# jh-jeong/ContraD

Hardware: AMD Instinct MI355X
Metric: discriminator-step images/sec (ContraD, SimCLR aug) (higher is better)
Workload: dtype f32; 1 GPU; SNDCGAN + ContraD D-step, CIFAR-10 32x32, global batch 512, simclr aug, nonsat loss, Adam(2e-4,(0.5,0.999)), random-init weights; global_batch=512, per_gpu_batch=512, parallelism=dp1, losses_finite=True, launch=hipGraph replay, rccl_ranks=1

## Files before the change

contrad_amd/_lib.py:

```python
import ctypes
import os
import re

_HERE = os.path.dirname(os.path.abspath(__file__))
LIB_PATH = os.environ.get('CONTRAD_HIP_LIB') or os.path.join(_HERE, 'csrc', 'libcontrad_hip.so')
HEADER_PATH = os.path.join(os.path.dirname(_HERE), 'include', 'contrad_hip.h')


class ConvDesc(ctypes.Structure):
    _fields_ = [(n, ctypes.c_int) for n in
                ('N', 'H', 'W', 'C', 'ldx', 'Ho', 'Wo', 'K', 'ldy', 'KH', 'KW', 'stride', 'pad', 'ldw')]


SN_MAX_LAYERS = 24
ADAM_MAX_TENSORS = 64
ADAM_CHUNK = 16384
AUG_NPARAM = 16


class SnLayer(ctypes.Structure):
    _fields_ = [('w', ctypes.c_void_p), ('u', ctypes.c_void_p), ('v', ctypes.c_void_p),
                ('u_snap', ctypes.c_void_p), ('v_snap', ctypes.c_void_p),
                ('wp', ctypes.c_void_p), ('gwp', ctypes.c_void_p), ('gw', ctypes.c_void_p),
                ('K', ctypes.c_int), ('C', ctypes.c_int), ('T', ctypes.c_int), ('ldw', ctypes.c_int),
                ('fixed_scale', ctypes.c_float)]


class SnBatch(ctypes.Structure):
    _fields_ = [('n', ctypes.c_int), ('layers', SnLayer * SN_MAX_LAYERS),
                ('scratch_off', ctypes.c_longlong * SN_MAX_LAYERS)]


class AdamTensor(ctypes.Structure):
    _fields_ = [('p', ctypes.c_void_p), ('g', ctypes.c_void_p), ('m', ctypes.c_void_p), ('v', ctypes.c_void_p),
                ('numel', ctypes.c_longlong)]


class AdamBatch(ctypes.Structure):
    _fields_ = [('n', ctypes.c_int), ('t', AdamTensor * ADAM_MAX_TENSORS),
                ('block_start', ctypes.c_int * (ADAM_MAX_TENSORS + 1))]


MODCONV_MAX_LAYERS = 32


class ModconvLayer(ctypes.Structure):
    _fields_ = [('w', ctypes.c_void_p), ('wp', ctypes.c_void_p), ('wsq', ctypes.c_void_p),
                ('Cout', ctypes.c_int), ('Cin', ctypes.c_int), ('T', ctypes.c_int), ('ldw', ctypes.c_int),
                ('transposed', ctypes.c_int), ('scale', ctypes.c_float)]


class ModconvBatch(ctypes.Structure):
    _fields_ = [('n', ctypes.c_int), ('layers', ModconvLayer * MODCONV_MAX_LAYERS)]


class DemodLayer(ctypes.Structure):
    _fields_ = [('style', ctypes.c_void_p), ('wsq', ctypes.c_void_p), ('out', ctypes.c_void_p),
                ('Cin', ctypes.c_int), ('K', ctypes.c_int)]


class DemodBatch(ctypes.Structure):
    _fields_ = [('n', ctypes.c_int), ('B', ctypes.c_int), ('layers', DemodLayer * MODCONV_MAX_LAYERS)]


_CTYPES = {
    'int': ctypes.c_int,
    'float': ctypes.c_float,
    'double': ctypes.c_double,
    'long long': ctypes.c_longlong,
    'contrad_stream_t': ctypes.c_void_p,
    'void': None,
}


def _map_type(t):
    t = t.strip()
    if t.endswith('*'):
        base = t[:-1].replace('const', '').strip()
        if base == 'contrad_conv_desc':
            return ctypes.POINTER(ConvDesc)
        if base == 'int':
            return ctypes.POINTER(ctypes.c_int)
        return ctypes.c_void_p
    t = t.replace('const', '').strip()
    return _CTYPES[t]


def parse_header(path=HEADER_PATH):
    src = open(path).read()
    src = re.sub(r'/\*.*?\*/', '', src, flags=re.S)
    protos = {}
    for m in re.finditer(r'\b(int|long long|void|double)\s+(contrad_\w+)\s*\(([^)]*)\)\s*;', src):
        ret, name, args = m.group(1), m.group(2), m.group(3).strip()
        argtypes = []
        if args and args != 'void':
            for a in args.split(','):
                a = a.strip()
                mm = re.match(r'(.*?)(\w+)$', a)
                argtypes.append(_map_type(mm.group(1)))
        protos[name] = (_CTYPES[ret], argtypes)
    return protos


class _Lib(object):
    def __init__(self):
        if not os.path.exists(LIB_PATH):
            raise RuntimeError(
                'contrad_amd: %s not found -- run `python -c "import __graft_entry__ as g; g.build()"` '
                '(or python contrad_amd/build.py).  There is no CPU / PyTorch fallback.' % LIB_PATH)
        self._dll = ctypes.CDLL(LIB_PATH)
        self.protos = parse_header()
        for name, (ret, argtypes) in self.protos.items():
            fn = getattr(self._dll, name)
            fn.restype = ret
            fn.argtypes = argtypes
            setattr(self, '_raw_' + name, fn)

    def call(self, name, *args):
        rc = getattr(self, '_raw_' + name)(*args)
        if rc != 0:
            raise RuntimeError('contrad_hip: %s failed with status %d' % (name, rc))

    def raw(self, name):
        return getattr(self, '_raw_' + name)


_lib = None


def lib():
    global _lib
    if _lib is None:
        _lib = _Lib()
    return _lib
```

contrad_amd/csrc/igemm.hip:

```cpp
#include "common.h"
#include <stdlib.h>
#include <string.h>
#include <algorithm>
#include <utility>
#include "../../include/contrad_hip.h"

namespace {

enum { MODE_FWD = 0, MODE_DGRAD = 1, MODE_WGRAD = 2 };
#ifndef IGEMM_BK
#define IGEMM_BK 16
#endif
constexpr int BK = IGEMM_BK;
#ifndef IGEMM_MIN_WAVES
#define IGEMM_MIN_WAVES 4
#endif
constexpr int NTHREADS = 256;

struct IgemmArgs {
  const float* A;
  const float* B;
  float* C;
  const float* bias;
  const float* addend;
// ... 713 lines not shown
  if (d->H < 4 || d->W < 4 || (d->H & (d->H - 1)) || (d->W & (d->W - 1))) return false;
  const int cin = mode == MODE_FWD ? d->C : d->K, cout = mode == MODE_FWD ? d->K : d->C;
  const int ldi = mode == MODE_FWD ? d->ldx : d->ldy, ldo = mode == MODE_FWD ? d->ldy : d->ldx;
  if ((cin & 15) || (cout & 63) || (ldi & 3) || (d->ldw & 3)) return false;
  const int th = std::min(8, d->H / 2), tw = std::min(8, d->W / 2);
  const long long nimg = 64 / (th * tw);
  if (nimg > 16) return false;
  const long long lim = 1ll << 31;
  if (nimg * d->H * d->W * std::max(ldi, ldo) * 4 >= lim) return false;
  if (16ll * cin * cout * 4 >= lim) return false;
  return true;
}

wino::Args wino_args(const contrad_conv_desc* d, int mode) {
  wino::Args a{};
  a.N = d->N; a.H = d->H; a.W = d->W;
  a.Cin = mode == MODE_FWD ? d->C : d->K;
  a.Cout = mode == MODE_FWD ? d->K : d->C;
  a.ldi = mode == MODE_FWD ? d->ldx : d->ldy;
  a.ldo = mode == MODE_FWD ? d->ldy : d->ldx;
  a.TH = std::min(8, d->H / 2); a.TW = std::min(8, d->W / 2);
  a.sh_tw = __builtin_ctz(a.TW); a.sh_thw = __builtin_ctz(a.TH * a.TW);
  a.NIMG = 64 / (a.TH * a.TW);
  a.PH = d->H / (2 * a.TH); a.PW = d->W / (2 * a.TW);
  a.NP = cdiv(d->N, a.NIMG) * a.PH * a.PW;
  a.NKB = a.Cout / 64;
  a.BH = a.PH > 1 ? 2 * a.TH + 2 : d->H; a.r_org = a.PH > 1 ? -1 : 0;
  a.BW = a.PW > 1 ? 2 * a.TW + 2 : d->W; a.c_org = a.PW > 1 ? -1 : 0;
  return a;
}

long long wino_items(const contrad_conv_desc* d, int mode) {
  const wino::Args a = wino_args(d, mode);
  return (long long)a.NP * a.NKB;
}

constexpr int WINO_CUS = 256;
bool wino44_planned(const contrad_conv_desc* d, int mode);

bool wino_planned(const contrad_conv_desc* d, int mode) {
  static const bool enabled = []() { const char* e = contrad_dev_env("CONTRAD_WINO"); return !(e && e[0] == '0'); }();
  if (!enabled || !wino_ok(d, mode)) return false;
  if (wino44_planned(d, mode)) return false;
  const long long items = wino_items(d, mode);
  const long long rounds = cdivll(items, WINO_CUS);
  static const long long min_items = []() { const char* e = contrad_dev_env("CONTRAD_WINO_MIN_ITEMS"); return e ? atoll(e) : 150ll; }();
  if (items < WINO_CUS) return items >= min_items;
  return rounds * WINO_CUS * 10 <= items * 14;
}

long long wino_workspace_bytes(const contrad_conv_desc* d) { return 16ll * d->C * d->K * (long long)sizeof(float); }

int wino_grid(const wino::Args& a) {
  const int l0 = cdiv(a.NP, 8) * a.NKB;
  return 8 * std::min(WINO_CUS / 8, l0);
}


bool wino44_ok(const contrad_conv_desc* d, int mode) {
  if (mode != MODE_FWD && mode != MODE_DGRAD) return false;
  if (d->KH != 3 || d->KW != 3 || d->stride != 1 || d->pad != 1) return false;
  if (d->H < 4 || d->W < 4 || (d->H & (d->H - 1)) || (d->W & (d->W - 1)) || (d->W < 32 ? d->H != d->W : d->H < 16)) return false;
  const int cin = mode == MODE_FWD ? d->C : d->K, cout = mode == MODE_FWD ? d->K : d->C;
  const int ldi = mode == MODE_FWD ? d->ldx : d->ldy, ldo = mode == MODE_FWD ? d->ldy : d->ldx;
  if ((cin & 31) || (cout & 31) || (ldi & 3) || (d->ldw & 3)) return false;
  const long long lim = 1ll << 31;
  const long long nimg = d->W >= 32 ? 1 : d->W == 16 ? 2 : d->W == 8 ? 8 : 32;
  if (nimg * d->H * d->W * std::max(ldi, ldo) * 4 >= lim) return false;
  if (36ll * cin * cout * 4 >= lim) return false;
  return true;
}

static inline bool wino44_round_ok(long long items) {
  static const long long min_items = []() { const char* e = contrad_dev_env("CONTRAD_WINO44_MIN_ITEMS"); return e ? atoll(e) : 230ll; }();
  if (items < WINO_CUS) return items >= min_items;
  return cdivll(items, WINO_CUS) * WINO_CUS * 10 <= items * 14;
}

static inline long long wino44_patches(const contrad_conv_desc* d) {
  const int TW = std::min(8, d->W / 4), TH = std::min(4, d->H / 4);
  return (long long)cdiv(d->N, 32 / (TH * TW)) * (d->H / (4 * TH)) * (d->W / (4 * TW));
}

static inline bool wino44_n32(const contrad_conv_desc* d, int mode) {
  static const bool all = []() { const char* e = contrad_dev_env("CONTRAD_WINO44N_ALL"); return e && e[0] == '1'; }();
  static const bool fill = []() { const char* e = contrad_dev_env("CONTRAD_WINO44N_FILL"); return !(e && e[0] == '0'); }();
  const int cout = mode == MODE_FWD ? d->K : d->C;
  if ((cout & 63) != 0 || d->W == 4 || all) return true;
  const long long items64 = wino44_patches(d) * (cout / 64);
  return fill && !wino44_round_ok(items64) && wino44_round_ok(2 * items64);
}

wino44::Args wino44_args(const contrad_conv_desc* d, int mode) {
  wino44::Args a{};
  a.N = d->N; a.H = d->H; a.W = d->W;
  a.Cin = mode == MODE_FWD ? d->C : d->K;
  a.Cout = mode == MODE_FWD ? d->K : d->C;
  a.ldi = mode == MODE_FWD ? d->ldx : d->ldy;
  a.ldo = mode == MODE_FWD ? d->ldy : d->ldx;
  a.TW = std::min(8, d->W / 4); a.TH = std::min(4, d->H / 4);
  a.sh_tw = __builtin_ctz(a.TW); a.sh_thw = __builtin_ctz(a.TH * a.TW);
  a.NIMG = 32 / (a.TH * a.TW);
  a.PH = d->H / (4 * a.TH); a.PW = d->W / (4 * a.TW);
  a.NP = cdiv(d->N, a.NIMG) * a.PH * a.PW;
  a.n32 = wino44_n32(d, mode) ? 1 : 0;
  a.NKB = a.n32 ? a.Cout / 32 : a.Cout / 64;
  a.BH = 4 * a.TH + 2; a.BW = 4 * a.TW + 2;
  return a;
}

long long wino44_items(const contrad_conv_desc* d, int mode) {
  const wino44::Args a = wino44_args(d, mode);
  return (long long)a.NP * a.NKB;
}

bool wino44_planned(const contrad_conv_desc* d, int mode) {
  static const bool enabled = []() { const char* e = contrad_dev_env("CONTRAD_WINO44"); return !(e && e[0] == '0'); }();
  static const bool enabled2 = []() { const char* e = contrad_dev_env("CONTRAD_WINO"); return !(e && e[0] == '0'); }();
  if (!enabled || !enabled2 || !wino44_ok(d, mode)) return false;
  static const bool enabled_n = []() { const char* e = contrad_dev_env("CONTRAD_WINO44N"); return !(e && e[0] == '0'); }();
  if (!enabled_n && wino44_n32(d, mode)) return false;
  return wino44_round_ok(wino44_items(d, mode));
}

long long wino44_workspace_bytes(const contrad_conv_desc* d) { return 36ll * d->C * d->K * (long long)sizeof(float); }

int wino44_grid(const wino44::Args& a) {
  const int l0 = cdiv(a.NP, 8) * a.NKB;
  return 8 * std::min(WINO_CUS / 8, l0);
}

template <int MODE, int BOXW>
int launch_wino44_inst(const wino44::Args& a, hipStream_t stream) {
  static const hipError_t attr = hipFuncSetAttribute((const void*)wino44::wino44_kernel<MODE, BOXW>, hipFuncAttributeMaxDynamicSharedMemorySize,
                                                     wino44::LDS_DWORDS * 4);
  if (attr != hipSuccess) return (int)attr;
  hipLaunchKernelGGL((wino44::wino44_kernel<MODE, BOXW>), dim3(wino44_grid(a)), dim3(512), wino44::LDS_DWORDS * 4, stream, a);
  CONTRAD_CHECK_LAUNCH();
  return 0;
}

template <int MODE, int BOXW>
int launch_wino44n_inst(const wino44::Args& a, hipStream_t stream) {
  static const hipError_t attr = hipFuncSetAttribute((const void*)wino44n::wino44n_kernel<MODE, BOXW>, hipFuncAttributeMaxDynamicSharedMemorySize,
                                                     wino44::LDS_DWORDS * 4);
  if (attr != hipSuccess) return (int)attr;
  hipLaunchKernelGGL((wino44n::wino44n_kernel<MODE, BOXW>), dim3(wino44_grid(a)), dim3(512), wino44::LDS_DWORDS * 4, stream, a);
  CONTRAD_CHECK_LAUNCH();
  return 0;
}

template <int MODE>
int launch_wino44(const contrad_conv_desc* d, const float* in, const float* wp, const float* bias, const float* ref,
                  float* out, float slope, float gain, float* U, hipStream_t stream) {
  wino44::Args a = wino44_args(d, MODE);
  a.x = in; a.U = U; a.y = out; a.bias = bias; a.ref = ref; a.slope = slope; a.gain = gain;
  const int quads = (a.Cin / 4) * a.Cout;
  hipLaunchKernelGGL(wino44::wino44_filter_kernel<MODE>, dim3(cdiv(quads, 256)), dim3(256), 0, stream, wp, U, d->C, d->K, d->ldw);
  CONTRAD_CHECK_LAUNCH();
  if (a.n32)
    return a.BW == 34 ? launch_wino44n_inst<MODE, 34>(a, stream) : a.BW == 18 ? launch_wino44n_inst<MODE, 18>(a, stream)
           : a.BW == 10 ? launch_wino44n_inst<MODE, 10>(a, stream) : launch_wino44n_inst<MODE, 6>(a, stream);
  return a.BW == 34 ? launch_wino44_inst<MODE, 34>(a, stream) : a.BW == 18 ? launch_wino44_inst<MODE, 18>(a, stream) : launch_wino44_inst<MODE, 10>(a, stream);
}

bool wino22_ok(const contrad_conv_desc* d, int mode) {
  if (mode != MODE_FWD && mode != MODE_DGRAD) return false;
  if (d->KH != 4 || d->KW != 4 || d->stride != 2 || d->pad != 1) return false;
  if ((d->H & 1) || (d->W & 1) || d->Ho * 2 != d->H || d->Wo * 2 != d->W) return false;
  auto grid_ok = [](int g) { return g == 4 || g == 8 || g == 16; };
  if (!grid_ok(d->Ho) || !grid_ok(d->Wo)) return false;
  const int cin = mode == MODE_FWD ? d->C : d->K, cout = mode == MODE_FWD ? d->K : d->C;
  const int ldi = mode == MODE_FWD ? d->ldx : d->ldy;
  if ((cin & (mode == MODE_FWD ? 7 : 15)) || (cout & 63) || (ldi & 3) || (d->ldw & 3)) return false;
  const long long nimg = wino22::TB / ((d->Ho / 2) * (d->Wo / 2));
  const long long lim = 1ll << 31;
  if (nimg * d->H * d->W * std::max(d->ldx, d->ldy) * 4 >= lim) return false;
  if (4ll * 9 * cin * cout * 4 >= lim) return false;
  return true;
}

wino22::Args wino22_args(const contrad_conv_desc* d, int mode) {
  wino22::Args a{};
  const bool dg = mode == MODE_DGRAD;
  a.N = d->N; a.dgrad = dg ? 1 : 0;
  a.Hi = dg ? d->Ho : d->H; a.Wi = dg ? d->Wo : d->W;
  a.Hout = dg ? d->H : d->Ho; a.Wout = dg ? d->W : d->Wo;
  a.Cin = dg ? d->K : d->C; a.Cout = dg ? d->C : d->K;
  a.ldi = dg ? d->ldy : d->ldx; a.ldo = dg ? d->ldx : d->ldy;
  a.GH = d->Ho; a.GW = d->Wo;
  const int tw = a.GW / 2, thw = (a.GH / 2) * tw;
  a.sh_tw = __builtin_ctz(tw); a.sh_thw = __builtin_ctz(thw);
  a.NIMG = wino22::TB / thw;
  a.NTB = cdiv(d->N, a.NIMG);
  a.NKB = a.Cout / 64;
  return a;
}

long long wino22_items(const contrad_conv_desc* d, int mode) {
  const wino22::Args a = wino22_args(d, mode);
  return (long long)a.NTB * a.NKB * (mode == MODE_DGRAD ? 4 : 1);
}

bool wino22_planned(const contrad_conv_desc* d, int mode) {
  static const bool enabled = []() { const char* e = contrad_dev_env("CONTRAD_WINO22"); return !(e && e[0] == '0'); }();
  if (!enabled || !wino22_ok(d, mode)) return false;
  const long long items = wino22_items(d, mode);
  const long long rounds = cdivll(items, WINO_CUS);
  static const long long min_items = []() { const char* e = contrad_dev_env("CONTRAD_WINO22_MIN_ITEMS"); return e ? atoll(e) : 150ll; }();
  if (items < WINO_CUS) return items >= min_items;
  return rounds * WINO_CUS * 100 <= items * 125;
}

long long wino22_workspace_bytes(const contrad_conv_desc* d) { return 4ll * 9 * d->C * d->K * (long long)sizeof(float); }

template <int MODE, int NRAW>
int launch_wino22_inst(const wino22::Args& a, int blocks, hipStream_t stream) {
  static const hipError_t attr = hipFuncSetAttribute((const void*)wino22::wino22_kernel<MODE, NRAW>, hipFuncAttributeMaxDynamicSharedMemorySize,
                                                     wino22::LDS_DWORDS * 4);
  if (attr != hipSuccess) return (int)attr;
  hipLaunchKernelGGL((wino22::wino22_kernel<MODE, NRAW>), dim3(blocks), dim3(512), wino22::LDS_DWORDS * 4, stream, a);
  CONTRAD_CHECK_LAUNCH();
  return 0;
}

template <int MODE>
int launch_wino22(const contrad_conv_desc* d, const float* in, const float* wp, const float* bias, const float* ref,
                  float* out, float slope, float gain, float* U, hipStream_t stream) {
  wino22::Args a = wino22_args(d, MODE);
  a.x = in; a.U = U; a.y = out; a.bias = bias; a.ref = ref; a.slope = slope; a.gain = gain;
  const int quads = 4 * (a.Cin / 4) * a.Cout;
  hipLaunchKernelGGL(wino22::wino22_filter_kernel<MODE>, dim3(cdiv(quads, 256)), dim3(256), 0, stream, wp, U, d->C, d->K, d->ldw);
  CONTRAD_CHECK_LAUNCH();
  const int l0 = cdiv(a.NTB, 8) * a.NKB * (MODE == MODE_DGRAD ? 4 : 1);
  const int blocks = 8 * std::min(WINO_CUS / 8, l0);
  const int items = 2 * a.NIMG * (a.GH + 1) * (a.GW + 1);
  const int nraw = cdiv(items, 256);
  if (nraw <= 5) return launch_wino22_inst<MODE, 5>(a, blocks, stream);
  if (nraw == 6) return launch_wino22_inst<MODE, 6>(a, blocks, stream);
  return launch_wino22_inst<MODE, 7>(a, blocks, stream);
}

bool wino23_ok(const contrad_conv_desc* d, int mode) {
  if (mode != MODE_FWD) return false;
  if (d->KH != 3 || d->KW != 3 || d->stride != 2 || d->pad != 0) return false;
  if (d->H != 2 * d->Ho + 1 || d->W != 2 * d->Wo + 1) return false;
  if (d->Ho < 4 || d->Wo < 4 || (d->Ho & (d->Ho - 1)) || (d->Wo & (d->Wo - 1))) return false;
  if (d->Wo >= 32 ? d->Ho < 16 : d->Ho != d->Wo) return false;
  if ((d->C & 15) || (d->K & 63) || (d->ldx & 3) || (d->ldw & 3)) return false;
  const long long nimg = d->Wo >= 32 ? 1 : 128 / ((d->Ho / 2) * (d->Wo / 2));
  const long long lim = 1ll << 31;
  if (nimg * d->H * d->W * std::max(d->ldx, d->ldy) * 4 >= lim) return false;
  if (4ll * 9 * d->C * d->K * 4 >= lim) return false;
  return true;
}

wino23::Args wino23_args(const contrad_conv_desc* d) {
  wino23::Args a{};
  a.N = d->N; a.Hi = d->H; a.Wi = d->W; a.GH = d->Ho; a.GW = d->Wo;
  a.Cin = d->C; a.Cout = d->K; a.ldi = d->ldx; a.ldo = d->ldy;
  a.TW = d->Wo >= 32 ? 16 : d->Wo / 2; a.TH = d->Wo >= 32 ? 8 : d->Ho / 2;
  a.sh_tw = __builtin_ctz(a.TW); a.sh_thw = __builtin_ctz(a.TH * a.TW);
  a.NIMG = wino23::TB / (a.TH * a.TW);
  a.PH = d->Ho / (2 * a.TH); a.PW = d->Wo / (2 * a.TW);
  a.NP = cdiv(d->N, a.NIMG) * a.PH * a.PW;
  a.NKB = a.Cout / 64;
  return a;
}

bool wino23_planned(const contrad_conv_desc* d, int mode) {
  static const bool enabled = []() { const char* e = contrad_dev_env("CONTRAD_WINO23"); return !(e && e[0] == '0'); }();
  if (!enabled || !wino23_ok(d, mode)) return false;
  const wino23::Args a = wino23_args(d);
  const long long items = (long long)a.NP * a.NKB;
  if (items < WINO_CUS) return items >= 230;
  return cdivll(items, WINO_CUS) * WINO_CUS * 10 <= items * 14;
}

long long wino23_workspace_bytes(const contrad_conv_desc* d) { return 4ll * 9 * d->C * d->K * (long long)sizeof(float); }

int wino23_grid(const wino23::Args& a) { return 8 * std::min(WINO_CUS / 8, cdiv(a.NP, 8) * a.NKB); }

template <int NRAW>
int launch_wino23_inst(const wino23::Args& a, hipStream_t stream) {
  static const hipError_t attr = hipFuncSetAttribute((const void*)wino23::wino23_kernel<NRAW>, hipFuncAttributeMaxDynamicSharedMemorySize,
                                                     wino23::LDS_DWORDS * 4);
  if (attr != hipSuccess) return (int)attr;
  hipLaunchKernelGGL((wino23::wino23_kernel<NRAW>), dim3(wino23_grid(a)), dim3(512), wino23::LDS_DWORDS * 4, stream, a);
  CONTRAD_CHECK_LAUNCH();
  return 0;
}

int launch_wino23(const contrad_conv_desc* d, const float* in, const float* wp, const float* bias, const float* ref,
                  float* out, float slope, float gain, float* U, hipStream_t stream) {
  wino23::Args a = wino23_args(d);
  a.x = in; a.U = U; a.y = out; a.bias = bias; a.ref = ref; a.slope = slope; a.gain = gain;
  const int quads = 4 * (a.Cin / 4) * a.Cout;
  hipLaunchKernelGGL(wino23::wino23_filter_kernel, dim3(cdiv(quads, 256)), dim3(256), 0, stream, wp, U, d->C, d->K, d->ldw);
  CONTRAD_CHECK_LAUNCH();
  const int nraw = cdiv(2 * a.NIMG * (2 * a.TH + 1) * (2 * a.TW + 1), 256);
  if (nraw <= 5) return launch_wino23_inst<5>(a, stream);
  if (nraw == 6) return launch_wino23_inst<6>(a, stream);
  return launch_wino23_inst<7>(a, stream);
}

bool wino22_wgrad_ok(const contrad_conv_desc* d) {
  if (d->KH != 4 || d->KW != 4 || d->stride != 2 || d->pad != 1) return false;
  if (d->Ho * 2 != d->H || d->Wo * 2 != d->W) return false;
  auto grid_ok = [](int g) { return g == 4 || g == 8 || g == 16; };
  if (!grid_ok(d->Ho) || !grid_ok(d->Wo)) return false;
  if ((d->C != 64 && (d->C & 127)) || (d->K & 63) || (d->ldx & 3) || (d->ldy & 3)) return false;
  if (2ll * d->H * d->W * std::max(d->ldx, d->ldy) * 4 >= (1ll << 31)) return false;
  return true;
}

wino22::WArgs wino22_wgrad_args(const contrad_conv_desc* d) {
  wino22::WArgs a{};
  a.N = d->N; a.H = d->H; a.W = d->W; a.C = d->C; a.K = d->K; a.ldx = d->ldx; a.ldy = d->ldy; a.GH = d->Ho; a.GW = d->Wo;
  a.CTW = std::min(4, a.GW / 2);
  a.CTH = std::min(8 / a.CTW, a.GH / 2);
  a.CNIMG = 8 / (a.CTH * a.CTW);
  a.sh_ctw = __builtin_ctz(a.CTW); a.sh_cthw = __builtin_ctz(a.CTH * a.CTW);
  a.QH = a.GH / (2 * a.CTH); a.QW = a.GW / (2 * a.CTW);
  a.Q = cdiv(d->N, a.CNIMG) * a.QH * a.QW;
  a.RBN = 4 * d->C / 128; a.KB = d->K / 64;
  a.CPB = std::min(d->C, 128); a.sh_cpb = __builtin_ctz(a.CPB);
  const int splits = std::max(1, std::min(a.Q, WINO_CUS / (a.RBN * a.KB)));
  a.qps = cdiv(a.Q, splits);
  return a;
}
int wino22_wgrad_splits(const wino22::WArgs& a) { return cdiv(a.Q, a.qps); }

bool wino22_wgrad_planned(const contrad_conv_desc* d) {
  static const bool enabled = []() { const char* e = contrad_dev_env("CONTRAD_WINO22_WGRAD"); return !(e && e[0] == '0'); }();
  static const bool enabled2 = []() { const char* e = contrad_dev_env("CONTRAD_WINO22"); return !(e && e[0] == '0'); }();
  if (!enabled || !enabled2 || !wino22_wgrad_ok(d)) return false;
  const wino22::WArgs a = wino22_wgrad_args(d);
  const long long blocks = (long long)a.RBN * a.KB * wino22_wgrad_splits(a);
  static const int min_qps = []() { const char* e = contrad_dev_env("CONTRAD_WINO_MIN_QPS"); return e ? atoi(e) : 16; }();
  return a.qps >= min_qps && blocks * 10 >= WINO_CUS * 7 && blocks <= WINO_CUS;
}

long long wino22_wgrad_workspace_bytes(const contrad_conv_desc* d) {
  const wino22::WArgs a = wino22_wgrad_args(d);
  return (long long)wino22_wgrad_splits(a) * (16ll * d->C + 1) * d->K * (long long)sizeof(float);
}

bool wino_wgrad_ok(const contrad_conv_desc* d) {
  if (d->KH != 3 || d->KW != 3 || d->stride != 1 || d->pad != 1) return false;
  if (d->H < 4 || d->W < 4 || (d->H & (d->H - 1)) || (d->W & (d->W - 1))) return false;
  if ((d->C & 63) || (d->K & 63) || (d->ldx & 3) || (d->ldy & 3)) return false;
  const long long lim = 1ll << 31;
  if (2ll * d->H * d->W * std::max(d->ldx, d->ldy) * 4 >= lim) return false;
  return true;
}

wino::WArgs wino_wgrad_args(const contrad_conv_desc* d) {
  wino::WArgs a{};
  a.N = d->N; a.H = d->H; a.W = d->W; a.C = d->C; a.K = d->K; a.ldx = d->ldx; a.ldy = d->ldy;
  a.CTW = std::min(4, d->W / 2);
  a.CTH = std::min(8 / a.CTW, d->H / 2);
  a.CNIMG = 8 / (a.CTH * a.CTW);
  a.sh_ctw = __builtin_ctz(a.CTW); a.sh_cthw = __builtin_ctz(a.CTH * a.CTW);
  a.QH = d->H / (2 * a.CTH); a.QW = d->W / (2 * a.CTW);
  a.Q = cdiv(d->N, a.CNIMG) * a.QH * a.QW;
  a.CB = d->C / 64; a.KB = d->K / 64;
  const int splits = std::max(1, std::min(a.Q, WINO_CUS / (a.CB * a.KB)));
  a.qps = cdiv(a.Q, splits);
  a.BH = a.QH > 1 ? 2 * a.CTH + 2 : d->H; a.r_org = a.QH > 1 ? -1 : 0;
  a.BW = a.QW > 1 ? 2 * a.CTW + 2 : d->W; a.c_org = a.QW > 1 ? -1 : 0;
  return a;
}
int wino_wgrad_splits(const wino::WArgs& a) { return cdiv(a.Q, a.qps); }

bool wino_wgrad_planned(const contrad_conv_desc* d) {
  static const bool enabled = []() { const char* e = contrad_dev_env("CONTRAD_WINO_WGRAD"); return !(e && e[0] == '0'); }();
  static const bool enabled2 = []() { const char* e = contrad_dev_env("CONTRAD_WINO"); return !(e && e[0] == '0'); }();
  if (!enabled || !enabled2 || !wino_wgrad_ok(d)) return false;
  const wino::WArgs a = wino_wgrad_args(d);
  const long long blocks = (long long)a.CB * a.KB * wino_wgrad_splits(a);
  static const int min_qps = []() { const char* e = contrad_dev_env("CONTRAD_WINO_MIN_QPS"); return e ? atoi(e) : 16; }();
  return a.qps >= min_qps && blocks * 10 >= WINO_CUS * 7 && blocks <= WINO_CUS;
}

long long wino_wgrad_workspace_bytes(const contrad_conv_desc* d) {
  const wino::WArgs a = wino_wgrad_args(d);
  return (long long)wino_wgrad_splits(a) * (9ll * d->C + 1) * d->K * (long long)sizeof(float);
}

template <int MODE>
int launch_wino(const contrad_conv_desc* d, const float* in, const float* wp, const float* bias, const float* ref,
                float* out, float slope, float gain, float* U, hipStream_t stream) {
  static const hipError_t attr = hipFuncSetAttribute((const void*)wino::wino_kernel<MODE>, hipFuncAttributeMaxDynamicSharedMemorySize,
                                                     wino::LDS_DWORDS * 4);
  if (attr != hipSuccess) return (int)attr;
  wino::Args a = wino_args(d, MODE);
  a.x = in; a.U = U; a.y = out; a.bias = bias; a.ref = ref; a.slope = slope; a.gain = gain;
  const int quads = (a.Cin / 4) * a.Cout;
  hipLaunchKernelGGL(wino::wino_filter_kernel<MODE>, dim3(cdiv(quads, 256)), dim3(256), 0, stream, wp, U, d->C, d->K, d->ldw);
  CONTRAD_CHECK_LAUNCH();
  hipLaunchKernelGGL(wino::wino_kernel<MODE>, dim3(wino_grid(a)), dim3(512), wino::LDS_DWORDS * 4, stream, a);
  CONTRAD_CHECK_LAUNCH();
  return 0;
}

template <int MODE, int BM, int BN, bool BAL>
int launch_lean_inst(const IgemmArgs& a, dim3 grid, hipStream_t stream) {
  static bool attr_set_dev[64] = {};
  constexpr size_t smem = lean_smem_bytes<MODE, BM, BN>();
  int dev_id = 0;
  (void)hipGetDevice(&dev_id);
  bool& attr_set = attr_set_dev[dev_id & 63];
  if (!attr_set) {
    hipError_t e = hipFuncSetAttribute(reinterpret_cast<const void*>(&igemm_lean_kernel<MODE, BM, BN, BAL>),
                                       hipFuncAttributeMaxDynamicSharedMemorySize, (int)smem);
    if (e != hipSuccess) return (int)e;
    attr_set = true;
  }
  IgemmArgs b = a;
  b.ny = (int)grid.y;
  hipLaunchKernelGGL((igemm_lean_kernel<MODE, BM, BN, BAL>), dim3(grid.x * grid.y), dim3(NTHREADS), smem, stream, b);
  CONTRAD_CHECK_LAUNCH();
  return 0;
}

template <int MODE, int BM, int BN>
int launch_lean(const IgemmArgs& a, dim3 grid, hipStream_t stream) {
  if constexpr (MODE == MODE_DGRAD) {
    if (a.cbal > 0) return launch_lean_inst<MODE, BM, BN, true>(a, grid, stream);
  }
  return launch_lean_inst<MODE, BM, BN, false>(a, grid, stream);
}

bool lean_ok(const contrad_conv_desc* d, int mode, long long pps) {
  static const bool enabled = []() { const char* e = contrad_dev_env("CONTRAD_IGEMM_LEAN"); return !(e && e[0] == '0'); }();
  if (!enabled || BK != 16) return false;
  const long long lim = 1ll << 31;
  if (d->KH * d->KW > 32) return false;
  if ((long long)d->KH * d->KW * d->C * d->ldw * 4 >= lim) return false;
  const long long img_x = (long long)d->H * d->W * d->ldx * 4, img_y = (long long)d->Ho * d->Wo * d->ldy * 4;
  if ((long long)d->ldy * 4 * 128 >= (1ll << 30) || (long long)d->K * 4 * 128 >= (1ll << 30)) return false;
  if (mode == MODE_FWD) {
    if ((d->C & 15) || (d->ldx & 3) || (d->K & 3)) return false;
    const long long imgs = 128 / ((long long)d->Ho * d->Wo) + 2;
    return imgs * img_x < lim;
  }
  if (mode == MODE_DGRAD) {
    if ((d->K & 15) || (d->ldy & 3)) return false;
    const long long imgs = 128 / ((long long)cdiv(d->H, d->stride) * cdiv(d->W, d->stride)) + 2;
    return imgs * img_y < lim && imgs * img_x < (1ll << 30);
  }
  if ((d->C & 3) || (d->ldx & 3) || (d->K & 3) || (d->ldy & 3)) return false;
  const long long P = (long long)d->N * d->Ho * d->Wo;
  if (P % 16) return false;
  const int gw = d->Wo < 16 ? d->Wo : 16;
  if (gw <= 0 || 16 % gw || d->Wo % gw) return false;
  const int gh = d->Ho < 16 / gw ? d->Ho : 16 / gw;
  if ((16 / gw) % gh || d->Ho % gh) return false;
  if (d->pad > gh * d->stride || d->pad > gw * d->stride) return false;
  const long long imgs = pps * 16 / ((long long)d->Ho * d->Wo) + 2;
  return imgs * img_x < lim && pps * 16 * d->ldy * 4 < lim;
}

bool vec_ok(const contrad_conv_desc* d, int mode) {
  const bool c4 = (d->C & 3) == 0 && (d->ldx & 3) == 0;
  const bool k4 = (d->K & 3) == 0 && (d->ldy & 3) == 0;
  if (mode == MODE_FWD) return c4 && (d->K & 3) == 0;
  if (mode == MODE_DGRAD) return k4;
  return c4 && k4;
}

struct PlanOverride { int bm, bn, splits; };
PlanOverride g_plan_override = {0, 0, 0};
#if defined(CONTRAD_DEV_SWITCHES)
}
extern "C" void contrad_dev_plan_override(int bm, int bn, int splits) { g_plan_override = PlanOverride{bm, bn, splits}; }
namespace {
#endif

void pick_tile(long long M, int Ncol, bool vec, bool lean, int mult4, int* bm, int* bn) {
  if (!vec) { *bm = 64; *bn = 64; return; }
  if (lean && Ncol <= 32) { *bm = 128; *bn = 32; return; }
  static const int forced = []() { const char* e = contrad_dev_env("CONTRAD_IGEMM_TILE"); return e ? atoi(e) : 0; }();
  if (forced) { *bm = forced / 1000; *bn = forced % 1000; return; }
  if (g_plan_override.bm > 0) { *bm = g_plan_override.bm; *bn = g_plan_override.bn; return; }
  static const int cand[4][2] = {{128, 128}, {64, 128}, {128, 64}, {64, 64}};
  for (int i = (Ncol > 64 ? 0 : 2); i < 4; ++i) {
    *bm = cand[i][0]; *bn = cand[i][1];
    if (cdivll(M, *bm) * cdivll(Ncol, *bn) * mult4 >= 768 * 4) return;
  }
}

template <int MODE>
int dispatch(const IgemmArgs& a, int bm, int bn, bool vec, dim3 grid, hipStream_t s) {
  if (vec && lean_ok(&a.d, MODE, a.ptiles_per_split)) {
    if (bn == 32) return launch_lean<MODE, 128, 32>(a, grid, s);
    if (bm == 128 && bn == 128) return launch_lean<MODE, 128, 128>(a, grid, s);
    if (bm == 128 && bn == 64) return launch_lean<MODE, 128, 64>(a, grid, s);
    if (bm == 64 && bn == 128) return launch_lean<MODE, 64, 128>(a, grid, s);
    return launch_lean<MODE, 64, 64>(a, grid, s);
  }
  if (!vec) return launch<MODE, 64, 64, false>(a, grid, s);
  if (bm == 128 && bn == 128) return launch<MODE, 128, 128, true>(a, grid, s);
  if (bm == 128 && bn == 64) return launch<MODE, 128, 64, true>(a, grid, s);
  if (bm == 64 && bn == 128) return launch<MODE, 64, 128, true>(a, grid, s);
  return launch<MODE, 64, 64, true>(a, grid, s);
}

bool aligned16(const void* a, const void* b, const void* c) {
  return (((uintptr_t)a | (uintptr_t)b | (uintptr_t)c) & 15) == 0;
}

int check_desc(const contrad_conv_desc* d) {
  CONTRAD_ARG(d != nullptr);
  CONTRAD_ARG(d->N > 0 && d->H > 0 && d->W > 0 && d->C > 0 && d->K > 0);
  CONTRAD_ARG(d->KH > 0 && d->KW > 0 && (d->stride == 1 || d->stride == 2) && d->pad >= 0);
  CONTRAD_ARG(d->Ho == (d->H + 2 * d->pad - d->KH) / d->stride + 1);
  CONTRAD_ARG(d->Wo == (d->W + 2 * d->pad - d->KW) / d->stride + 1);
  CONTRAD_ARG(d->ldx >= d->C && d->ldy >= d->K && d->ldw >= d->K);
  CONTRAD_ARG((d->ldw & 3) == 0);
  CONTRAD_ARG((long long)d->N * d->H * d->W * d->ldx < (1ll << 31));
  CONTRAD_ARG((long long)d->N * d->Ho * d->Wo * d->ldy < (1ll << 31));
  CONTRAD_ARG((long long)d->KH * d->KW * d->C * d->ldw < (1ll << 31));
  if ((d->C & 3) == 0) CONTRAD_ARG((d->ldx & 3) == 0);
  if ((d->K & 3) == 0) CONTRAD_ARG((d->ldy & 3) == 0);
  return 0;
}

int wgrad_plan(const contrad_conv_desc* d, int* bm, int* bn, int* tiles_m, int* tiles_n, int* splits,
               int* ptiles_per_split) {
  const int Kg = d->KH * d->KW * d->C;
  const long long P = (long long)d->N * d->Ho * d->Wo;
  *bn = (d->K > 64) ? 128 : 64;
  *bm = (Kg > 64) ? 128 : 64;
  static const int forced = []() { const char* e = contrad_dev_env("CONTRAD_WGRAD_TILE"); return e ? atoi(e) : 0; }();
  if (forced) { *bm = forced / 1000; *bn = forced % 1000; }
  if (g_plan_override.bm > 0) { *bm = g_plan_override.bm; *bn = g_plan_override.bn; }
  static const int target = []() { const char* e = contrad_dev_env("CONTRAD_WGRAD_BLOCKS"); return e ? atoi(e) : 1024; }();
  if (!vec_ok(d, MODE_WGRAD)) { *bm = 64; *bn = 64; }
  *tiles_m = cdiv(Kg, *bm);
  *tiles_n = cdiv(d->K, *bn);
  const long long ptiles = cdivll(P, BK);
  long long want = target / ((long long)(*tiles_m) * (*tiles_n));
  if (g_plan_override.splits > 0) want = g_plan_override.splits;
  if (want < 1) want = 1;
  long long pps = cdivll(ptiles, want);
  if (pps < 4) pps = 4;
  if (pps > ptiles) pps = ptiles;
  *ptiles_per_split = (int)pps;
  *splits = (int)cdivll(ptiles, pps);
  if (d->K <= 32 && *bm == 128 && vec_ok(d, MODE_WGRAD) && lean_ok(d, MODE_WGRAD, pps)) *bn = 32;
  return 0;
}
// ... 566 lines not shown
                       d->ldx, d->ldw, bias, slope, gain, y, d->ldy, addend);
    CONTRAD_CHECK_LAUNCH();
    return 0;
  }
  const bool vec = vec_ok(d, MODE_FWD);
  const FwdPlan p = fwd_plan(d);
  a.tiles_m = p.pixmajor == 1 ? cdiv(d->N, p.bm) * d->Ho * d->Wo : cdiv(a.M, p.bm);
  a.tiles_n = cdiv(a.Ncol, p.bn);
  a.pixmajor = p.pixmajor == 1;
  if (p.pixmajor == 2) fill_border_classes(d, MODE_FWD, p.bm, &a);
  if (p.pixmajor == 1) {
    int taps[256];
    for (int ho = 0; ho < d->Ho; ++ho)
      for (int wo = 0; wo < d->Wo; ++wo) {
        int vh = 0, vw = 0;
        for (int kh = 0; kh < d->KH; ++kh) vh += (unsigned)(ho * d->stride - d->pad + kh) < (unsigned)d->H;
        for (int kw = 0; kw < d->KW; ++kw) vw += (unsigned)(wo * d->stride - d->pad + kw) < (unsigned)d->W;
        taps[ho * d->Wo + wo] = vh * vw;
      }
    pixel_order(taps, d->Ho * d->Wo, a.px_order);
    unsigned char full[256];
    if (pixel_order_full(taps, d->Ho * d->Wo, cdiv(d->N, p.bm), a.tiles_n, full, 8)) {
      memcpy(a.px_order, full, sizeof(full));
      a.px_full = 1;
    }
  }
  a.ptiles_per_split = p.tps;
  if (p.splits > 1) {
    CONTRAD_ARG(workspace && workspace_bytes >= contrad_conv2d_fwd_workspace_bytes(d));
    a.C = workspace;
  }
  rc = dispatch<MODE_FWD>(a, p.bm, p.bn, vec, dim3(a.tiles_m * a.tiles_n, p.splits), (hipStream_t)stream);
  if (rc || p.splits <= 1) return rc;
  const long long total = M * d->K;
  int blocks = (int)((total + 255) / 256);
  if (blocks > 2048) blocks = 2048;
  hipLaunchKernelGGL(fwd_reduce_kernel, dim3(blocks), dim3(256), 0, (hipStream_t)stream, workspace, p.splits, M,
                     d->K, bias, slope, gain, y, d->ldy, addend);
  CONTRAD_CHECK_LAUNCH();
  return 0;
}

extern "C" int contrad_conv2d_fwd(const contrad_conv_desc* d, const float* x, const float* wp,
                                  const float* bias, float* y, float slope, float gain, float* workspace,
                                  long long workspace_bytes, contrad_stream_t stream) {
  return contrad_conv2d_fwd_add(d, x, wp, bias, nullptr, y, slope, gain, workspace, workspace_bytes, stream);
}

extern "C" long long contrad_conv2d_dgrad_workspace_bytes(const contrad_conv_desc* d) {
  if (check_desc(d)) return -22;
  if (wino44_planned(d, MODE_DGRAD)) return wino44_workspace_bytes(d);
  if (wino_planned(d, MODE_DGRAD)) return wino_workspace_bytes(d);
  if (wino22_planned(d, MODE_DGRAD)) return wino22_workspace_bytes(d);
  const FwdPlan p = dgrad_plan(d, true);
  if (p.splits <= 1) return 0;
  return (long long)p.splits * d->N * d->H * d->W * d->ldx * (long long)sizeof(float);
}

extern "C" int contrad_conv2d_dgrad_ws(const contrad_conv_desc* d, const float* gy, const float* wp,
                                       float* dx, const float* act_ref, float slope, float gain,
                                       float* workspace, long long workspace_bytes, contrad_stream_t stream) {
  int rc = check_desc(d);
  if (rc) return rc;
  CONTRAD_ARG(gy && wp && dx);
  if (vec_ok(d, MODE_DGRAD)) CONTRAD_ARG(aligned16(gy, wp, dx) && aligned16(act_ref, nullptr, nullptr));
  if (wino44_planned(d, MODE_DGRAD) && workspace && workspace_bytes >= wino44_workspace_bytes(d)) {
    CONTRAD_ARG(aligned16(gy, wp, workspace));
    return launch_wino44<MODE_DGRAD>(d, gy, wp, nullptr, act_ref, dx, slope, gain, workspace, (hipStream_t)stream);
  }
  if (wino_planned(d, MODE_DGRAD) && workspace && workspace_bytes >= wino_workspace_bytes(d)) {
    CONTRAD_ARG(aligned16(gy, wp, workspace));
    return launch_wino<MODE_DGRAD>(d, gy, wp, nullptr, act_ref, dx, slope, gain, workspace, (hipStream_t)stream);
  }
  if (wino22_planned(d, MODE_DGRAD) && workspace && workspace_bytes >= wino22_workspace_bytes(d)) {
    CONTRAD_ARG(aligned16(gy, wp, workspace));
    return launch_wino22<MODE_DGRAD>(d, gy, wp, nullptr, act_ref, dx, slope, gain, workspace, (hipStream_t)stream);
  }
  if (conv_c32_ok(d))
    return launch_conv_c32<MODE_DGRAD>(d, gy, wp, dx, nullptr, nullptr, act_ref, slope, gain, (hipStream_t)stream);
  IgemmArgs a{};
  a.A = gy; a.B = wp; a.C = dx; a.act_ref = act_ref; a.d = *d; a.slope = slope; a.gain = gain;
  a.st_nt = st_nt_for((long long)d->N * d->H * d->W, d->ldx);
  const int s = d->stride;
  const long long Mc = (long long)d->N * cdiv(d->H, s) * cdiv(d->W, s);
  CONTRAD_ARG(Mc < (1ll << 31));
  const bool vec = vec_ok(d, MODE_DGRAD);
  const FwdPlan pl = dgrad_plan(d, workspace != nullptr);
  const int bm = pl.bm, bn = pl.bn;
  a.pixmajor = pl.pixmajor == 1;
  a.px_pixels = cdiv(d->H, s) * cdiv(d->W, s);
  a.tiles_m = pl.pixmajor == 1 ? cdiv(d->N, bm) * a.px_pixels : cdiv((int)Mc, bm);
  if (pl.pixmajor == 2) fill_border_classes(d, MODE_DGRAD, bm, &a);
  if (pl.pixmajor == 1) {
    int taps[256];
    for (int i = 0; i < a.px_pixels; ++i) taps[i] = 1;
    if (s == 1)
      for (int h = 0; h < d->H; ++h)
        for (int w = 0; w < d->W; ++w) {
          int vh = 0, vw = 0;
          for (int kh = 0; kh < d->KH; ++kh) vh += (unsigned)(h + d->pad - kh) < (unsigned)d->Ho;
          for (int kw = 0; kw < d->KW; ++kw) vw += (unsigned)(w + d->pad - kw) < (unsigned)d->Wo;
          taps[h * d->W + w] = vh * vw;
        }
    pixel_order(taps, a.px_pixels, a.px_order);
    unsigned char full[256];
    if (s == 1 && pixel_order_full(taps, a.px_pixels, cdiv(d->N, bm), cdiv(d->C, bn), full, 8)) {
      memcpy(a.px_order, full, sizeof(full));
      a.px_full = 1;
    } else if (s == 2 && dgrad_strided_full_ok(d, bm, bn)) {
      int t0[256];
      const int npix = dgrad_strided_class0_taps(d, t0);
      pixel_order_full(t0, npix, cdiv(d->N, bm), cdiv(d->C, bn), full, 2);
      memcpy(a.px_order, full, sizeof(full));
      a.px_full = 2;
    }
  }
  a.tiles_n = cdiv(d->C, bn);
  if (pl.splits > 1) {
    CONTRAD_ARG(workspace_bytes >= contrad_conv2d_dgrad_workspace_bytes(d));
    a.dsplits = pl.splits;
    a.ptiles_per_split = pl.tps;
    a.slab_elems = (long long)d->N * d->H * d->W * d->ldx;
    CONTRAD_ARG(a.slab_elems * 4 < (1ll << 40));
    a.C = workspace; a.act_ref = nullptr;
    rc = dispatch<MODE_DGRAD>(a, bm, bn, vec, dim3(a.tiles_m * a.tiles_n, pl.splits), (hipStream_t)stream);
    if (rc) return rc;
    const long long rows = (long long)d->N * d->H * d->W;
    long long blocks = (rows * (d->C / 4) + 255) / 256;
    if (blocks > 4096) blocks = 4096;
    hipLaunchKernelGGL(dgrad_reduce_kernel, dim3((unsigned)blocks), dim3(256), 0, (hipStream_t)stream, workspace,
                       pl.splits, a.slab_elems, rows, d->C, d->ldx, act_ref, slope, gain, dx);
    CONTRAD_CHECK_LAUNCH();
    return 0;
  }
  a.cgroup = (s > 1) ? dgrad_cgroup(a.tiles_m, a.tiles_n) : 0;
  if (a.px_full == 2) a.cgroup = a.tiles_m;
  if (pl.balanced && vec && lean_ok(d, MODE_DGRAD, 0) && !a.pixmajor && a.nwin == 0) {
    const long long blocks = dgrad_balance(d, a.tiles_m, &a);
    if (blocks > 0) {
      a.cgroup = 0;
      return dispatch<MODE_DGRAD>(a, bm, bn, vec, dim3((unsigned)(blocks * a.tiles_n), 1), (hipStream_t)stream);
    }
  }
  const int tm_pad = a.cgroup > 0 ? cdiv(a.tiles_m, a.cgroup) * a.cgroup : a.tiles_m;
  return dispatch<MODE_DGRAD>(a, bm, bn, vec, dim3(tm_pad * a.tiles_n, s * s), (hipStream_t)stream);
}

extern "C" int contrad_conv2d_dgrad(const contrad_conv_desc* d, const float* gy, const float* wp,
                                    float* dx, const float* act_ref, float slope, float gain,
                                    contrad_stream_t stream) {
  return contrad_conv2d_dgrad_ws(d, gy, wp, dx, act_ref, slope, gain, nullptr, 0, stream);
}

extern "C" int contrad_conv2d_wino_ok(const contrad_conv_desc* d, int mode) {
  if (check_desc(d)) return -22;
  if (mode == MODE_WGRAD) return (wino_wgrad_ok(d) || wino22_wgrad_ok(d)) ? 1 : 0;
  return (wino_ok(d, mode) || wino22_ok(d, mode) || wino23_ok(d, mode)) ? 1 : 0;
}

extern "C" long long contrad_conv2d_wino_workspace_bytes(const contrad_conv_desc* d, int mode) {
  if (check_desc(d) || mode < 0 || mode > 2) return -22;
  if (mode == MODE_WGRAD) return wino_wgrad_ok(d) ? wino_wgrad_workspace_bytes(d) : wino22_wgrad_ok(d) ? wino22_wgrad_workspace_bytes(d) : -22;
  if (wino22_ok(d, mode)) return wino22_workspace_bytes(d);
  if (wino23_ok(d, mode)) return wino23_workspace_bytes(d);
  return wino_ok(d, mode) ? wino_workspace_bytes(d) : -22;
}

extern "C" int contrad_conv2d_wino_wgrad(const contrad_conv_desc* d, const float* x, const float* gy, float* dwp,
                                         float* dbias, float* workspace, long long workspace_bytes,
                                         contrad_stream_t stream) {
  int rc = check_desc(d);
  if (rc) return rc;
  CONTRAD_ARG(x && gy && dwp && workspace && aligned16(x, gy, workspace));
  if (wino22_wgrad_ok(d)) {
    CONTRAD_ARG(workspace_bytes >= wino22_wgrad_workspace_bytes(d));
    return launch_wino22_wgrad(d, x, gy, dwp, dbias, workspace, (hipStream_t)stream);
  }
  CONTRAD_ARG(wino_wgrad_ok(d) && workspace_bytes >= wino_wgrad_workspace_bytes(d));
  return launch_wino_wgrad(d, x, gy, dwp, dbias, workspace, (hipStream_t)stream);
}

extern "C" int contrad_conv2d_wino(const contrad_conv_desc* d, int mode, const float* in, const float* wp,
                                   const float* bias, const float* ref, float* out, float slope, float gain,
                                   float* workspace, long long workspace_bytes, contrad_stream_t stream) {
  int rc = check_desc(d);
  if (rc) return rc;
  CONTRAD_ARG(in && wp && out && workspace && (mode == MODE_FWD || mode == MODE_DGRAD));
  CONTRAD_ARG(aligned16(in, wp, workspace));
  if (wino22_ok(d, mode)) {
    CONTRAD_ARG(workspace_bytes >= wino22_workspace_bytes(d) && (mode == MODE_FWD || bias == nullptr));
    if (mode == MODE_FWD) return launch_wino22<MODE_FWD>(d, in, wp, bias, ref, out, slope, gain, workspace, (hipStream_t)stream);
    return launch_wino22<MODE_DGRAD>(d, in, wp, nullptr, ref, out, slope, gain, workspace, (hipStream_t)stream);
  }
  if (wino23_ok(d, mode)) {
    CONTRAD_ARG(workspace_bytes >= wino23_workspace_bytes(d));
    return launch_wino23(d, in, wp, bias, ref, out, slope, gain, workspace, (hipStream_t)stream);
  }
  CONTRAD_ARG(wino_ok(d, mode) && workspace_bytes >= wino_workspace_bytes(d));
  if (mode == MODE_FWD) return launch_wino<MODE_FWD>(d, in, wp, bias, ref, out, slope, gain, workspace, (hipStream_t)stream);
  CONTRAD_ARG(bias == nullptr);
  return launch_wino<MODE_DGRAD>(d, in, wp, nullptr, ref, out, slope, gain, workspace, (hipStream_t)stream);
}

extern "C" int contrad_conv2d_wino44_ok(const contrad_conv_desc* d, int mode) {
  if (check_desc(d)) return -22;
  return wino44_ok(d, mode) ? 1 : 0;
}

extern "C" long long contrad_conv2d_wino44_workspace_bytes(const contrad_conv_desc* d) {
  if (check_desc(d)) return -22;
  if (!wino44_ok(d, MODE_FWD) && !wino44_ok(d, MODE_DGRAD)) return -22;
  return wino44_workspace_bytes(d);
}

extern "C" int contrad_conv2d_wino44(const contrad_conv_desc* d, int mode, const float* in, const float* wp,
                                     const float* bias, const float* ref, float* out, float slope, float gain,
                                     float* workspace, long long workspace_bytes, contrad_stream_t stream) {
  int rc = check_desc(d);
  if (rc) return rc;
  CONTRAD_ARG(in && wp && out && workspace && (mode == MODE_FWD || mode == MODE_DGRAD));
  CONTRAD_ARG(aligned16(in, wp, workspace) && aligned16(ref, nullptr, nullptr));
  CONTRAD_ARG(wino44_ok(d, mode) && workspace_bytes >= wino44_workspace_bytes(d));
  if (mode == MODE_FWD) return launch_wino44<MODE_FWD>(d, in, wp, bias, ref, out, slope, gain, workspace, (hipStream_t)stream);
  CONTRAD_ARG(bias == nullptr);
  return launch_wino44<MODE_DGRAD>(d, in, wp, nullptr, ref, out, slope, gain, workspace, (hipStream_t)stream);
}

extern "C" int contrad_conv2d_tile(const contrad_conv_desc* d, int mode, int* bm, int* bn) {
  int rc = check_desc(d);
  if (rc) return rc;
  CONTRAD_ARG(bm && bn && mode >= 0 && mode <= 2);
  if (mode == MODE_FWD) {
    const FwdPlan p = fwd_plan(d);
    *bm = p.bm; *bn = p.bn;
  } else if (mode == MODE_DGRAD) {
    const FwdPlan p = dgrad_plan(d, true);
    *bm = p.bm; *bn = p.bn;
  } else {
    int tm, tn, sp, pps;
    wgrad_plan(d, bm, bn, &tm, &tn, &sp, &pps);
  }
  return 0;
}

extern "C" int contrad_conv2d_path(const contrad_conv_desc* d, int mode) {
  if (check_desc(d) || mode < 0 || mode > 2) return -22;
  if (mode == MODE_FWD && fwd_k1_ok(d)) return 5;
  if (mode != MODE_WGRAD && wino44_planned(d, mode)) return wino44_n32(d, mode) ? 11 : 9;
  if (mode != MODE_WGRAD && wino_planned(d, mode)) return 7;
  if (mode != MODE_WGRAD && wino22_planned(d, mode)) return 8;
  if (wino23_planned(d, mode)) return 10;
  if (mode == MODE_WGRAD && wino_wgrad_planned(d)) return 7;
  if (mode == MODE_WGRAD && wino22_wgrad_planned(d)) return 8;
  if (mode != MODE_WGRAD && conv_c32_ok(d)) return 6;
  if (!vec_ok(d, mode)) return 0;
  if (mode == MODE_WGRAD && wgrad_c32_ok(d)) return 4;
  long long pps = 0;
  if (mode == MODE_WGRAD) {
    int bm, bn, tm, tn, sp, p;
    wgrad_plan(d, &bm, &bn, &tm, &tn, &sp, &p);
    pps = p;
  }
  if (!lean_ok(d, mode, pps)) return 1;
  if (mode == MODE_FWD && fwd_plan(d).pixmajor) return 3;
  if (mode == MODE_DGRAD && dgrad_plan(d, true).pixmajor) return 3;
  if (mode == MODE_WGRAD) {
    int bm, bn, tm, tn, sp, p;
    wgrad_plan(d, &bm, &bn, &tm, &tn, &sp, &p);
    if (wgrad_pixmajor_ok(d, bm, p)) return 3;
  }
  return 2;
}

extern "C" double contrad_conv2d_executed_fraction(const contrad_conv_desc* d, int mode) {
  if (check_desc(d) || mode < 0 || mode > 2) return -22.0;
  if (contrad_conv2d_path(d, mode) == 9 || contrad_conv2d_path(d, mode) == 11) return 0.25;
  if (contrad_conv2d_path(d, mode) == 7) return 4.0 / 9.0;
  if (contrad_conv2d_path(d, mode) == 8) return 9.0 / 16.0;
  if (contrad_conv2d_path(d, mode) == 10) return 25.0 / 36.0;
  if (contrad_conv2d_path(d, mode) != 3) return 1.0;
  return mode == MODE_DGRAD ? dgrad_valid_tap_fraction(d) : fwd_valid_tap_fraction(d);
}

extern "C" long long contrad_conv2d_grid_blocks(const contrad_conv_desc* d, int mode, int with_workspace) {
  if (check_desc(d) || mode < 0 || mode > 2) return -22;
  if (mode != MODE_WGRAD && with_workspace && wino44_planned(d, mode)) return wino44_grid(wino44_args(d, mode));
  if (mode != MODE_WGRAD && with_workspace && wino_planned(d, mode)) return wino_grid(wino_args(d, mode));
  if (with_workspace && wino23_planned(d, mode)) return wino23_grid(wino23_args(d));
  if (mode != MODE_WGRAD && with_workspace && wino22_planned(d, mode)) {
    const wino22::Args a = wino22_args(d, mode);
    return 8 * std::min(WINO_CUS / 8, cdiv(a.NTB, 8) * a.NKB * (mode == MODE_DGRAD ? 4 : 1));
  }
  if (mode == MODE_FWD) {
    const FwdPlan p = fwd_plan(d);
    const long long M = (long long)d->N * d->Ho * d->Wo;
    if (fwd_k1_ok(d)) return cdivll(M, 4);
    if (conv_c32_ok(d)) return conv_c32_blocks(d);
    if (p.pixmajor == 1) return (long long)cdiv(d->N, p.bm) * d->Ho * d->Wo * cdiv(d->K, p.bn);
    if (p.pixmajor == 2) return (long long)border_class_tiles(d, MODE_FWD, p.bm) * cdiv(d->K, p.bn);
    return cdivll(M, p.bm) * cdiv(d->K, p.bn) * (with_workspace ? p.splits : 1);
  }
  if (mode == MODE_DGRAD) {
    if (conv_c32_ok(d)) return conv_c32_blocks(d);
    const int s = d->stride;
    const long long Mc = (long long)d->N * cdiv(d->H, s) * cdiv(d->W, s);
    const FwdPlan p = dgrad_plan(d, with_workspace != 0);
// ... 127 lines not shown
```

contrad_amd/csrc/wino.h:

```cpp
#pragma once

namespace wino {

constexpr int KQS = 264;
constexpr int PL = 528;
constexpr int V_SZ = 16 * PL;
constexpr int BUF = 2 * V_SZ;
constexpr int RAW_PX = 324;
constexpr int RAW_SZ = (RAW_PX + 1) * 8;
constexpr int RAW0 = 2 * BUF;
constexpr int LDS_DWORDS = 2 * BUF + 2 * RAW_SZ;
constexpr unsigned OOB = 0x80000000u;

struct Args {
  const float* x;
  const float* U;
  float* y;
  const float* bias;
  const float* ref;
  float slope, gain;
  int N, H, W, Cin, Cout, ldi, ldo;
  int TH, TW;
  int sh_tw, sh_thw;
  int NIMG;
// ... 181 lines not shown
    for (int i = 0; i < 4; ++i) row_stage_store(0, i);
  }
  __syncthreads();

#ifndef WINO_EARLY_BARRIER
#define WINO_EARLY_BARRIER 1
#endif
  float4 fa[2], fb[2];
  fa[0] = *reinterpret_cast<const float4*>(smem + rdA);
  fb[0] = *reinterpret_cast<const float4*>(smem + rdB);
  auto chunk = [&](auto par) {
    constexpr int P = decltype(par)::value;
    constexpr int cur = P * BUF, nxt = BUF - cur;
#if !WINO_EARLY_BARRIER
    fa[0] = *reinterpret_cast<const float4*>(smem + cur + rdA);
    fb[0] = *reinterpret_cast<const float4*>(smem + cur + rdB);
#endif
#pragma unroll
    for (int xi = 0; xi < 8; ++xi) {
      if (xi + 1 < 8) {
        fa[(xi + 1) & 1] = *reinterpret_cast<const float4*>(smem + cur + rdA + (xi + 1) * PL);
        fb[(xi + 1) & 1] = *reinterpret_cast<const float4*>(smem + cur + rdB + (xi + 1) * PL);
      }
      if constexpr (ROLE == 0) {
        if (xi == 0) read_raw(1 - P);
        if (xi == 1) { col_stage(0); col_stage(1); }
        if (xi == 2) { col_stage(2); col_stage(3); }
        if (xi >= 3 && xi < 7) row_stage_store(nxt, xi - 3);
      } else {
        if (xi == 0) { store_raw(P, 0); store_raw(P, 1); store_raw(P, 2); }
        if (xi == 1) load_raw3();
        if (xi >= 2 && xi < 6) { store_u(nxt, 2 * (xi - 2)); store_u(nxt, 2 * (xi - 2) + 1); }
        if (xi >= 3 && xi < 7) { load_u(2 * (xi - 3)); load_u(2 * (xi - 3) + 1); }
        if (xi == 6) step_u();
      }
#if WINO_EARLY_BARRIER
      if (xi == 7) {
        __syncthreads();
        fa[0] = *reinterpret_cast<const float4*>(smem + nxt + rdA);
        fb[0] = *reinterpret_cast<const float4*>(smem + nxt + rdB);
      }
#endif
      __builtin_amdgcn_sched_barrier(0);
      const float* a = (const float*)&fa[xi & 1];
      const float* b = (const float*)&fb[xi & 1];
#pragma unroll
      for (int j = 0; j < 4; ++j) acc[xi] = __builtin_amdgcn_mfma_f32_32x32x2f32(a[j], b[j], acc[xi], 0, 0, 0);
      __builtin_amdgcn_sched_barrier(0);
    }
#if !WINO_EARLY_BARRIER
    __syncthreads();
#endif
  };

  float4* xch = reinterpret_cast<float4*>(smem + BUF) + (wave * 16) * 64 + lane;
  const float g1 = p.gain, g0 = p.gain * p.slope;

  for (; w_cur < L; w_cur += nslots) {
    for (int t = 0; t < NCH; t += 2) {
      chunk(std::integral_constant<int, 0>{});
      chunk(std::integral_constant<int, 1>{});
    }
    auto part = [&](int r) -> float4 {
      float s0[2], s1[2];
#pragma unroll
      for (int a = 0; a < 2; ++a) {
        const float m0 = acc[a * 4 + 0][r], m1 = acc[a * 4 + 1][r], m2 = acc[a * 4 + 2][r], m3 = acc[a * 4 + 3][r];
        s0[a] = m0 + m1 + m2;
        s1[a] = m1 - m2 - m3;
      }
      return ROLE == 0 ? make_float4(s0[0] + s0[1], s1[0] + s1[1], s0[1], s1[1])
                       : make_float4(s0[0], s1[0], -s0[0] - s0[1], -s1[0] - s1[1]);
    };
    if constexpr (ROLE == 1) {
#pragma unroll
      for (int r = 0; r < 16; ++r) xch[r * 64] = part(r);
      __syncthreads();
    } else {
      const Item it = decode(w_cur);
      const int cout = it.kb * 64 + wn * 32 + l31;
      float* ybase = p.y + (size_t)it.n_first * p.H * p.W * p.ldo;
      const __amdgpu_buffer_rsrc_t rsY = rsrc(ybase, true);
      const __amdgpu_buffer_rsrc_t rsR = rsrc(p.ref ? p.ref + (size_t)it.n_first * p.H * p.W * p.ldo : ybase, p.ref != nullptr);
      const unsigned dcol = (unsigned)p.ldo * 4u, drow = (unsigned)(p.W * p.ldo) * 4u;
      auto bit_off = [&](int b) -> unsigned {
        return b < p.sh_tw ? (unsigned)((2 << b) * p.ldo * 4)
               : b < p.sh_thw ? (unsigned)((2 << (b - p.sh_tw)) * p.W * p.ldo * 4)
                              : (unsigned)((1 << (b - p.sh_thw)) * p.H * p.W * p.ldo * 4);
      };
      const unsigned lane_off = (lhi ? bit_off(2) : 0u) + (wm ? bit_off(5) : 0u) + (unsigned)((wn * 32 + l31) * 4);
      const int lane_img = (wm * 32 + 4 * lhi) >> p.sh_thw;
      const unsigned item_off = (unsigned)(((it.ph * 2 * p.TH * p.W + it.pw * 2 * p.TW) * p.ldo + it.kb * 64) * 4);
      const int img_lim = p.N - it.n_first - lane_img;
      const unsigned base_off = lane_off + item_off;
      auto row_off = [&](int r) -> unsigned {
        const int rbits = (r & 3) + 8 * (r >> 2);
        const unsigned u = ((r & 1) ? bit_off(0) : 0u) + ((r & 2) ? bit_off(1) : 0u) + ((r & 4) ? bit_off(3) : 0u) + ((r & 8) ? bit_off(4) : 0u);
        return ((rbits >> p.sh_thw) < img_lim) ? base_off + u : OOB;
      };
      float rv[16][4];
#ifndef WINO_NO_REF
      if (p.ref) {
#pragma unroll
        for (int r = 0; r < 16; ++r) {
          const unsigned o = row_off(r);
          rv[r][0] = __builtin_bit_cast(float, __builtin_amdgcn_raw_buffer_load_b32(rsR, (int)o, 0, 0));
          rv[r][1] = __builtin_bit_cast(float, __builtin_amdgcn_raw_buffer_load_b32(rsR, (int)(o + dcol), 0, 0));
          rv[r][2] = __builtin_bit_cast(float, __builtin_amdgcn_raw_buffer_load_b32(rsR, (int)(o + drow), 0, 0));
          rv[r][3] = __builtin_bit_cast(float, __builtin_amdgcn_raw_buffer_load_b32(rsR, (int)(o + drow + dcol), 0, 0));
        }
      }
#else
      for (int r = 0; r < 16; ++r) for (int e = 0; e < 4; ++e) rv[r][e] = 1.f;
#endif
      const float bj = (MODE == MODE_FWD && p.bias) ? p.bias[cout] : 0.f;
      __syncthreads();
#pragma unroll
      for (int r = 0; r < 16; ++r) {
        __builtin_amdgcn_sched_barrier(0);
        const float4 mine = part(r), oth = xch[r * 64];
        float v[4] = {mine.x + oth.x, mine.y + oth.y, mine.z + oth.z, mine.w + oth.w};
#pragma unroll
        for (int e = 0; e < 4; ++e) {
          if constexpr (MODE == MODE_DGRAD) {
            if (p.ref) v[e] *= (rv[r][e] > 0.f) ? g1 : g0;
          } else {
            v[e] += bj;
            v[e] *= (v[e] > 0.f) ? g1 : g0;
            if (p.ref) v[e] += rv[r][e];
          }
        }
        const unsigned o = row_off(r);
        __builtin_amdgcn_raw_buffer_store_b32(__builtin_bit_cast(unsigned, v[0]), rsY, (int)o, 0, 0);
        __builtin_amdgcn_raw_buffer_store_b32(__builtin_bit_cast(unsigned, v[1]), rsY, (int)(o + dcol), 0, 0);
        __builtin_amdgcn_raw_buffer_store_b32(__builtin_bit_cast(unsigned, v[2]), rsY, (int)(o + drow), 0, 0);
        __builtin_amdgcn_raw_buffer_store_b32(__builtin_bit_cast(unsigned, v[3]), rsY, (int)(o + drow + dcol), 0, 0);
      }
    }
#pragma unroll
    for (int i = 0; i < 8; ++i)
#pragma unroll
      for (int r = 0; r < 16; ++r) acc[i][r] = 0.f;
    __syncthreads();
  }
}

template <int MODE>
__global__ __launch_bounds__(512, 2) void wino_kernel(const Args p) {
  extern __shared__ __attribute__((aligned(16))) float smem[];
  if (threadIdx.x < 256) body<MODE, 0>(p, smem); else body<MODE, 1>(p, smem);
}

template <int MODE>
__global__ __launch_bounds__(256) void wino_filter_kernel(const float* __restrict__ wp, float* __restrict__ U, int C, int K, int ldw) {
  const int cin = (MODE == MODE_FWD) ? C : K, cout = (MODE == MODE_FWD) ? K : C;
  const int idx = blockIdx.x * 256 + threadIdx.x;
  if (idx >= (cin >> 2) * cout) return;
  const int o = idx % cout, q4 = idx / cout;
  float g[9][4];
  if constexpr (MODE == MODE_FWD) {
#pragma unroll
    for (int t = 0; t < 9; ++t)
#pragma unroll
      for (int j = 0; j < 4; ++j) g[t][j] = wp[(size_t)(t * C + 4 * q4 + j) * ldw + o];
  } else {
#pragma unroll
    for (int t = 0; t < 9; ++t) {
      const float4 v = *reinterpret_cast<const float4*>(wp + (size_t)((8 - t) * C + o) * ldw + 4 * q4);
      g[t][0] = v.x; g[t][1] = v.y; g[t][2] = v.z; g[t][3] = v.w;
    }
  }
  const int nch = cin >> 3;
  float4* Uo = reinterpret_cast<float4*>(U);
#pragma unroll
  for (int a = 0; a < 4; ++a) {
    float t[3][4];
#pragma unroll
    for (int j = 0; j < 3; ++j)
#pragma unroll
      for (int e = 0; e < 4; ++e) {
        const float g0 = g[0 * 3 + j][e], g1 = g[1 * 3 + j][e], g2 = g[2 * 3 + j][e];
        t[j][e] = a == 0 ? g0 : a == 1 ? 0.5f * (g0 + g1 + g2) : a == 2 ? 0.5f * (g0 - g1 + g2) : g2;
      }
#pragma unroll
    for (int b = 0; b < 4; ++b) {
      float u[4];
#pragma unroll
      for (int e = 0; e < 4; ++e) {
        const float v = b == 0 ? t[0][e] : b == 1 ? 0.5f * (t[0][e] + t[1][e] + t[2][e]) : b == 2 ? 0.5f * (t[0][e] - t[1][e] + t[2][e]) : -t[2][e];
        u[e] = v;
      }
      const int xi = a * 4 + b;
      Uo[((size_t)(xi * nch + (q4 >> 1)) * 2 + (q4 & 1)) * cout + o] = make_float4(u[0], u[1], u[2], u[3]);
    }
  }
}


constexpr int W_PLANE = 512;
constexpr int W_VSZ = 16 * W_PLANE;
constexpr int W_STAGE = 2 * W_VSZ;
constexpr int W_RAWPX = 60;
constexpr int W_RAWSZ = W_RAWPX * 64;
constexpr int W_RAW0 = 2 * W_STAGE;
constexpr int W_ZERO = W_RAW0 + 2 * W_RAWSZ;
constexpr int W_LDS_DWORDS = W_ZERO + 64;

struct WArgs {
  const float* x;
  const float* gy;
  float* ws;
  float* bias_ws;
  int N, H, W, C, K, ldx, ldy;
  int CTH, CTW, sh_ctw, sh_cthw, CNIMG;
  int QH, QW;
  int Q, qps;
  int BH, BW, r_org, c_org;
  int CB, KB;
};

template <int ROLE>
__device__ __forceinline__ void wbody(const WArgs& p, float* smem) {
  const int tid = threadIdx.x & 255, lane = tid & 63, wave = tid >> 6;
  const int l31 = lane & 31, lhi = lane >> 5;
  const int wm = wave >> 1, wn = wave & 1;
  const int per = p.CB * p.KB;
  const int lin = xcd_remap(blockIdx.x, gridDim.x);
  const int split = lin / per, rem = lin - split * per;
  const int cb = rem / p.KB, kb = rem - cb * p.KB;
  const int q_begin = split * p.qps, q_end = min(p.Q, q_begin + p.qps);
  const int T = max(0, q_end - q_begin);
  const int qpi = p.QH * p.QW;

  struct Stream { int q, ng, cy, cx; };
  auto stream_at = [&](int q) -> Stream {
    Stream s; s.q = q; s.ng = q / qpi;
    const int r = q - s.ng * qpi;
    s.cy = r / p.QW; s.cx = r - s.cy * p.QW;
    return s;
  };
  auto step = [&](Stream& s) { ++s.q; if (++s.cx == p.QW) { s.cx = 0; if (++s.cy == p.QH) { s.cy = 0; ++s.ng; } } };

  int xfix[4], xr[4], xc[4], ximg[4], wrRaw[4];
  const int npx = p.CNIMG * p.BH * p.BW;
  const int gq = tid & 15, hsel = (tid >> 4) & 1, gt = tid >> 5;
  int gfix = 0, gimg = 0;
  const int wrG = W_VSZ + (hsel * 8) * W_PLANE + gt * 64 + gq * 4;
  if constexpr (ROLE == 1) {
#pragma unroll
    for (int i = 0; i < 4; ++i) {
      const int item = (tid + 256 * i) % (npx * 16), px = item >> 4, cq = item & 15;
      const int bhw = p.BH * p.BW;
      ximg[i] = px / bhw;
      const int r2 = px - ximg[i] * bhw;
      xr[i] = r2 / p.BW + p.r_org; xc[i] = r2 - (r2 / p.BW) * p.BW + p.c_org;
      xfix[i] = ((ximg[i] * p.H + xr[i]) * p.W + xc[i]) * p.ldx * 4 + (cb * 64 + cq * 4) * 4;
      wrRaw[i] = px * 64 + ((cq ^ ((px & 1) * 8)) * 4);
    }
    gimg = gt >> p.sh_cthw;
    const int ty = (gt >> p.sh_ctw) & (p.CTH - 1), tx = gt & (p.CTW - 1);
    gfix = ((gimg * p.H + 2 * ty) * p.W + 2 * tx) * p.ldy * 4 + (kb * 64 + gq * 4) * 4;
  }
  Stream sx = stream_at(q_begin), sg = stream_at(q_begin);
  float4 rraw[4], rg[4];
  float4 colacc = make_float4(0.f, 0.f, 0.f, 0.f);
  const bool do_bias = p.bias_ws != nullptr && cb == 0;

  auto load_raw = [&]() {
    const bool on = sx.q < q_end;
    const float* base = p.x + (size_t)sx.ng * p.CNIMG * p.H * p.W * p.ldx;
    const __amdgpu_buffer_rsrc_t rs = rsrc(base, on);
    const int oy = sx.cy * 2 * p.CTH, ox = sx.cx * 2 * p.CTW;
    const int soff = (oy * p.W + ox) * p.ldx * 4;
    const int nleft = p.N - sx.ng * p.CNIMG;
#pragma unroll
    for (int i = 0; i < 4; ++i) {
      const bool ok = (unsigned)(oy + xr[i]) < (unsigned)p.H && (unsigned)(ox + xc[i]) < (unsigned)p.W && ximg[i] < nleft;
      rraw[i] = bload4(rs, ok ? (unsigned)(xfix[i] + soff) : OOB, 0);
    }
    step(sx);
  };
  auto store_raw = [&](int stage) {
#pragma unroll
    for (int i = 0; i < 4; ++i)
      *reinterpret_cast<float4*>(smem + W_RAW0 + stage * W_RAWSZ + wrRaw[i]) = rraw[i];
  };
  auto load_gy = [&]() {
    const bool on = sg.q < q_end && sg.ng * p.CNIMG + gimg < p.N;
    const float* base = p.gy + (size_t)sg.ng * p.CNIMG * p.H * p.W * p.ldy;
    const __amdgpu_buffer_rsrc_t rs = rsrc(base, sg.q < q_end);
    const unsigned v = on ? (unsigned)(gfix + ((sg.cy * 2 * p.CTH * p.W + sg.cx * 2 * p.CTW) * p.ldy) * 4) : OOB;
    const unsigned dc = (unsigned)p.ldy * 4u, dr = (unsigned)(p.W * p.ldy) * 4u;
    rg[0] = bload4(rs, v, 0); rg[1] = bload4(rs, v + dc, 0);
    rg[2] = bload4(rs, v + dr, 0); rg[3] = bload4(rs, v + dr + dc, 0);
    step(sg);
  };
  const float hs = hsel ? 1.f : 0.f;
  auto gy_stage_store = [&](int bufoff) {
    float u0[2][4], u1[2][4];
#pragma unroll
    for (int q = 0; q < 2; ++q)
#pragma unroll
      for (int e = 0; e < 4; ++e) {
        const float g0 = ((const float*)&rg[q])[e], g1 = ((const float*)&rg[2 + q])[e];
        u0[q][e] = __builtin_fmaf(-hs, g1, g0);
        u1[q][e] = __builtin_fmaf(1.f - hs, g0, g1);
      }
#pragma unroll
    for (int al = 0; al < 2; ++al) {
      const float (*u)[4] = al ? u1 : u0;
      float4 o0, o1, o2, o3;
#pragma unroll
      for (int e = 0; e < 4; ++e) {
        ((float*)&o0)[e] = u[0][e]; ((float*)&o1)[e] = u[0][e] + u[1][e];
        ((float*)&o2)[e] = u[0][e] - u[1][e]; ((float*)&o3)[e] = u[1][e];
      }
      float* dst = smem + bufoff + wrG + al * 4 * W_PLANE;
      *reinterpret_cast<float4*>(dst) = o0;
      *reinterpret_cast<float4*>(dst + W_PLANE) = o1;
      *reinterpret_cast<float4*>(dst + 2 * W_PLANE) = o2;
      *reinterpret_cast<float4*>(dst + 3 * W_PLANE) = o3;
      if (al == 1 && do_bias) {
        asm volatile("" ::: "memory");
        colacc.x += o1.x; colacc.y += o1.y; colacc.z += o1.z; colacc.w += o1.w;
      }
    }
  };

  const int half = tid & 1, cq = (tid >> 1) & 15, tile = tid >> 5;
  const float sgn = half ? -1.f : 1.f;
  const int wsw = (cq ^ (half ? 4 : 0)) * 4;
  const int wrV0 = (half ? 3 : 0) * W_PLANE + tile * 64 + wsw;
  const int wrV1 = (half ? 2 : 1) * W_PLANE + tile * 64 + wsw;
  int rdRawA[4], rdRawB[4];
  if constexpr (ROLE == 0) {
    const int img = tile >> p.sh_cthw, ty = (tile >> p.sh_ctw) & (p.CTH - 1), tx = tile & (p.CTW - 1);
    const int cA = 2 * tx - 1 + (half ? 2 : 1) - p.c_org, cB = 2 * tx - 1 + (half ? 3 : 0) - p.c_org;
#pragma unroll
    for (int i = 0; i < 4; ++i) {
      const int r = 2 * ty - 1 + i - p.r_org;
      const bool rok = (unsigned)r < (unsigned)p.BH;
      const int pa = (img * p.BH + r) * p.BW + cA, pb = (img * p.BH + r) * p.BW + cB;
      rdRawA[i] = (rok && (unsigned)cA < (unsigned)p.BW) ? pa * 64 + ((cq ^ ((pa & 1) * 8)) * 4) : -1;
      rdRawB[i] = (rok && (unsigned)cB < (unsigned)p.BW) ? pb * 64 + ((cq ^ ((pb & 1) * 8)) * 4) : -1;
    }
  }
  float4 rxA[4], rxB[4];
  float tA[4][4], tB[4][4];
// ... 163 lines not shown
```

contrad_amd/csrc/wino22.h:

```cpp
#pragma once

namespace wino22 {

constexpr int TB = 128;
constexpr int VKQ = TB * 4;
constexpr int VPL = 2 * VKQ;
constexpr int V_SZ = 9 * VPL;
constexpr int UKQ = 64 * 4, UPL = 2 * UKQ;
constexpr int U_SZ = 9 * UPL;
constexpr int BUF = V_SZ + U_SZ;
constexpr int RAW_PX = 800;
constexpr int RAW_SZ = RAW_PX * 8;
constexpr int RAW0 = 2 * BUF;
constexpr int LDS_DWORDS = 2 * BUF + 2 * RAW_SZ;
constexpr unsigned OOB = 0x80000000u;
constexpr int NU = 5;

struct Args {
  const float* x;
  const float* U;
  float* y;
  const float* bias;
  const float* ref;
  float slope, gain;
// ... 158 lines not shown
  for (int i = 0; i < 9; ++i)
#pragma unroll
    for (int r = 0; r < 16; ++r) acc[i][r] = 0.f;

  if constexpr (ROLE == 1) {
    w_raw = w_cur; raw_item(w_raw);
    load_raw();
    store_raw(0);
    load_raw();
  } else {
    w_u = w_cur; u_item(w_u);
    load_u();
    store_u(0);
    load_u();
  }
  __syncthreads();
  if constexpr (ROLE == 0) {
    read_raw(0);
    row_ops();
#pragma unroll
    for (int r = 0; r < 3; ++r) col_ops_store(0, r);
  } else {
    store_raw(1);
    load_raw();
  }
  __syncthreads();

  auto chunk = [&](auto par, auto last_c) {
    constexpr int P = decltype(par)::value;
    constexpr bool last = decltype(last_c)::value;
    constexpr int cur = P * BUF, nxt = BUF - cur;
    float4 fa[2], fb[2];
    fa[0] = *reinterpret_cast<const float4*>(smem + cur + rdA);
    fb[0] = *reinterpret_cast<const float4*>(smem + cur + rdB);
#pragma unroll
    for (int xi = 0; xi < 9; ++xi) {
      if (xi + 1 < 9) {
        fa[(xi + 1) & 1] = *reinterpret_cast<const float4*>(smem + cur + rdA + (xi + 1) * VPL);
        fb[(xi + 1) & 1] = *reinterpret_cast<const float4*>(smem + cur + rdB + (xi + 1) * UPL);
      }
      if constexpr (ROLE == 0) {
#ifndef W22_ABL_NO_TR
        if (xi == 0) read_raw(1 - P);
        if (xi == 2) row_ops();
        if (xi >= 3 && xi < 6) col_ops_store(nxt, xi - 3);
#endif
#ifndef W22_ABL_NO_U
        if (xi == 6) store_u(nxt);
        if (xi == 7 && !last) load_u();
#endif
      } else {
#ifndef W22_ABL_NO_RAW
        if (xi == 0) store_raw(P);
        if (xi == 1 && !last) load_raw();
#endif
      }
      __builtin_amdgcn_sched_barrier(0);
      const float* a = (const float*)&fa[xi & 1];
      const float* b = (const float*)&fb[xi & 1];
#pragma unroll
      for (int j = 0; j < 4; ++j) acc[xi] = __builtin_amdgcn_mfma_f32_32x32x2f32(a[j], b[j], acc[xi], 0, 0, 0);
      __builtin_amdgcn_sched_barrier(0);
    }
    __syncthreads();
  };

  const float g1 = p.gain, g0 = p.gain * p.slope;
  const int OS = DG ? 2 : 1;
  auto bit_off = [&](int b) -> unsigned {
    return b < p.sh_tw ? (unsigned)((2 << b) * OS * p.ldo * 4)
           : b < p.sh_thw ? (unsigned)((2 << (b - p.sh_tw)) * OS * p.Wout * p.ldo * 4)
                          : (unsigned)((1 << (b - p.sh_thw)) * p.Hout * p.Wout * p.ldo * 4);
  };

  for (; w_cur < L; w_cur += nslots) {
    for (int t = 0; t + 2 < NCH; t += 2) {
      chunk(std::integral_constant<int, 0>{}, std::false_type{});
      chunk(std::integral_constant<int, 1>{}, std::false_type{});
    }
    chunk(std::integral_constant<int, 0>{}, std::false_type{});
    chunk(std::integral_constant<int, 1>{}, std::true_type{});
    const Item it = decode(w_cur);
    const int cout = it.kb * 64 + wn * 32 + l31;
    float* ybase = p.y + (size_t)it.n_first * p.Hout * p.Wout * p.ldo;
    const __amdgpu_buffer_rsrc_t rsY = rsrc(ybase, true);
    const __amdgpu_buffer_rsrc_t rsR = rsrc(p.ref ? p.ref + (size_t)it.n_first * p.Hout * p.Wout * p.ldo : ybase, p.ref != nullptr);
    const float ga = p.ref ? g1 : 1.f, gb = p.ref ? g0 : 1.f;
    const unsigned dcol = (unsigned)(OS * p.ldo) * 4u, drow = (unsigned)(OS * p.Wout * p.ldo) * 4u;
    const unsigned ph_off = DG ? (unsigned)((((it.ph >> 1) * p.Wout) + (it.ph & 1)) * p.ldo * 4) : 0u;
    const unsigned lane_off = (lhi ? bit_off(2) : 0u) + (unsigned)((wn * 32 + l31) * 4);
    const unsigned wave_off = ((wm & 1) ? bit_off(5) : 0u) + ((wm & 2) ? bit_off(6) : 0u) + (unsigned)(it.kb * 64 * 4) + ph_off;
    const int lane_img = (wm * 32 + 4 * lhi) >> p.sh_thw;
    const int img_lim = p.N - it.n_first - lane_img;
    const float bj = (MODE == MODE_FWD && p.bias) ? p.bias[cout] : 0.f;
#ifdef W22_ABL_NO_EPI
    if (p.N < 0)
#endif
#pragma unroll
    for (int h = 0; h < 4; ++h) {
      float rv[4][4];
      unsigned vo[4], so[4];
#pragma unroll
      for (int q = 0; q < 4; ++q) {
        const int r = h * 4 + q, rbits = (r & 3) + 8 * (r >> 2);
        vo[q] = ((rbits >> p.sh_thw) < img_lim) ? lane_off : OOB;
        so[q] = wave_off + ((r & 1) ? bit_off(0) : 0u) + ((r & 2) ? bit_off(1) : 0u) + ((r & 4) ? bit_off(3) : 0u) + ((r & 8) ? bit_off(4) : 0u);
        rv[q][0] = __builtin_bit_cast(float, __builtin_amdgcn_raw_buffer_load_b32(rsR, (int)vo[q], (int)so[q], 0));
        rv[q][1] = __builtin_bit_cast(float, __builtin_amdgcn_raw_buffer_load_b32(rsR, (int)vo[q], (int)(so[q] + dcol), 0));
        rv[q][2] = __builtin_bit_cast(float, __builtin_amdgcn_raw_buffer_load_b32(rsR, (int)vo[q], (int)(so[q] + drow), 0));
        rv[q][3] = __builtin_bit_cast(float, __builtin_amdgcn_raw_buffer_load_b32(rsR, (int)vo[q], (int)(so[q] + drow + dcol), 0));
      }
#pragma unroll
      for (int q = 0; q < 4; ++q) {
        __builtin_amdgcn_sched_barrier(0);
        const int r = h * 4 + q;
        float s[3], s2[3];
#pragma unroll
        for (int a = 0; a < 3; ++a) {
          const float m0 = acc[a * 3 + 0][r], m1 = acc[a * 3 + 1][r], m2 = acc[a * 3 + 2][r];
          s[a] = m0 + m1; s2[a] = m1 + m2;
        }
        float v[4] = {s[0] + s[1], s2[0] + s2[1], s[1] + s[2], s2[1] + s2[2]};
#pragma unroll
        for (int e = 0; e < 4; ++e) {
          if constexpr (DG) {
            v[e] *= (rv[q][e] > 0.f) ? ga : gb;
          } else {
            v[e] += bj;
            v[e] = __builtin_fmaf(v[e], (v[e] > 0.f) ? g1 : g0, rv[q][e]);
          }
        }
        __builtin_amdgcn_raw_buffer_store_b32(__builtin_bit_cast(unsigned, v[0]), rsY, (int)vo[q], (int)so[q], 0);
        __builtin_amdgcn_raw_buffer_store_b32(__builtin_bit_cast(unsigned, v[1]), rsY, (int)vo[q], (int)(so[q] + dcol), 0);
        __builtin_amdgcn_raw_buffer_store_b32(__builtin_bit_cast(unsigned, v[2]), rsY, (int)vo[q], (int)(so[q] + drow), 0);
        __builtin_amdgcn_raw_buffer_store_b32(__builtin_bit_cast(unsigned, v[3]), rsY, (int)vo[q], (int)(so[q] + drow + dcol), 0);
      }
    }
#pragma unroll
    for (int i = 0; i < 9; ++i)
#pragma unroll
      for (int r = 0; r < 16; ++r) acc[i][r] = 0.f;
    __builtin_amdgcn_sched_barrier(0);
    if constexpr (ROLE == 1) load_raw(); else load_u();
  }
}

template <int MODE, int NRAW>
__global__ __launch_bounds__(512, 2) void wino22_kernel(const Args p) {
  extern __shared__ __attribute__((aligned(16))) float smem[];
  if (threadIdx.x < 256) body<MODE, 0, NRAW>(p, smem); else body<MODE, 1, NRAW>(p, smem);
}

template <int MODE>
__global__ __launch_bounds__(256) void wino22_filter_kernel(const float* __restrict__ wp, float* __restrict__ U, int C, int K, int ldw) {
  const int cin = (MODE == MODE_FWD) ? C : K, cout = (MODE == MODE_FWD) ? K : C;
  const int per = (cin >> 2) * cout;
  const int idx = blockIdx.x * 256 + threadIdx.x;
  if (idx >= 4 * per) return;
  const int ph = idx / per, rem = idx - ph * per;
  const int o = rem % cout, q4 = rem / cout;
  const int phh = ph >> 1, phw = ph & 1;
  float g[2][2][4];
#pragma unroll
  for (int a = 0; a < 2; ++a)
#pragma unroll
    for (int b = 0; b < 2; ++b) {
      const int kh = (MODE == MODE_FWD) ? (phh ? 2 * a : 1 + 2 * a) : (phh ? 2 - 2 * a : 3 - 2 * a);
      const int kw = (MODE == MODE_FWD) ? (phw ? 2 * b : 1 + 2 * b) : (phw ? 2 - 2 * b : 3 - 2 * b);
      if constexpr (MODE == MODE_FWD) {
#pragma unroll
        for (int j = 0; j < 4; ++j) g[a][b][j] = wp[(size_t)((kh * 4 + kw) * C + 4 * q4 + j) * ldw + o];
      } else {
        const float4 v = *reinterpret_cast<const float4*>(wp + (size_t)((kh * 4 + kw) * C + o) * ldw + 4 * q4);
        g[a][b][0] = v.x; g[a][b][1] = v.y; g[a][b][2] = v.z; g[a][b][3] = v.w;
      }
    }
  const int nch = cin >> 3;
  float4* Uo = reinterpret_cast<float4*>(U) + (size_t)ph * 9 * nch * 2 * cout;
#pragma unroll
  for (int i = 0; i < 3; ++i)
#pragma unroll
    for (int j = 0; j < 3; ++j) {
      float u[4];
#pragma unroll
      for (int e = 0; e < 4; ++e) {
        const float r0 = j == 0 ? g[0][0][e] : j == 1 ? g[0][0][e] + g[0][1][e] : g[0][1][e];
        const float r1 = j == 0 ? g[1][0][e] : j == 1 ? g[1][0][e] + g[1][1][e] : g[1][1][e];
        u[e] = i == 0 ? r0 : i == 1 ? r0 + r1 : r1;
      }
      Uo[((size_t)((i * 3 + j) * nch + (q4 >> 1)) * 2 + (q4 & 1)) * cout + o] = make_float4(u[0], u[1], u[2], u[3]);
    }
}


constexpr int WV_PL = 8 * 128, WG_PL = 8 * 64;
constexpr int WV_SZ = 9 * WV_PL, WG_SZ = 9 * WG_PL;
constexpr int W_STAGE = WV_SZ + WG_SZ;
constexpr int W_RAWPX = 50;
constexpr int W_RAWSZ = W_RAWPX * 128;
constexpr int W_RAW0 = 2 * W_STAGE;
constexpr int W_LDS_DWORDS = 2 * W_STAGE + 2 * W_RAWSZ;
constexpr int W_NRAW = 7;

struct WArgs {
  const float* x;
  const float* gy;
  float* ws;
  float* bias_ws;
  int N, H, W, C, K, ldx, ldy, GH, GW;
  int CTH, CTW, sh_ctw, sh_cthw, CNIMG;
  int QH, QW, Q, qps;
  int RBN, KB;
  int CPB, sh_cpb;
};

template <int ROLE>
__device__ __forceinline__ void wbody(const WArgs& p, float* smem) {
  const int tid = threadIdx.x & 255, lane = threadIdx.x & 63, w8 = threadIdx.x >> 6;
  const int l31 = lane & 31, lhi = lane >> 5;
  const int wr = w8 & 3, wc = w8 >> 2;
  const int per = p.RBN * p.KB;
  const int lin = xcd_remap(blockIdx.x, gridDim.x);
  const int split = lin / per, rem = lin - split * per;
  const int rb = rem / p.KB, kb = rem - rb * p.KB;
  const int q_begin = split * p.qps, q_end = min(p.Q, q_begin + p.qps);
  const int T = max(0, q_end - q_begin);
  const int qpi = p.QH * p.QW;
  const int BH = 2 * p.CTH + 1, BW = 2 * p.CTW + 1, BHW = BH * BW;
  const int NBOX = 128 >> p.sh_cpb;
  const int row0 = rb * 128;

  struct Stream { int q, ng, cy, cx; };
  auto stream_at = [&](int q) -> Stream {
    Stream s; s.q = q; s.ng = q / qpi;
    const int r = q - s.ng * qpi;
    s.cy = r / p.QW; s.cx = r - s.cy * p.QW;
    return s;
  };
  auto step = [&](Stream& s) { ++s.q; if (++s.cx == p.QW) { s.cx = 0; if (++s.cy == p.QH) { s.cy = 0; ++s.ng; } } };

  int xfix[W_NRAW], xpk[W_NRAW];
  const int qpb = p.CPB >> 2;
  const int nitems = NBOX * p.CNIMG * BHW * qpb;
  if constexpr (ROLE == 1) {
#pragma unroll
    for (int i = 0; i < W_NRAW; ++i) {
      const int item = tid + 256 * i;
      const int cq = item % qpb, t1 = item / qpb;
      const int px = t1 % BHW, t2 = t1 / BHW;
      const int im = t2 % p.CNIMG, box = t2 / p.CNIMG;
      const int r = px / BW, c = px - r * BW;
      const int row = row0 + box * p.CPB;
      const int ph = row / p.C, c0 = row - ph * p.C;
      const int pp = ph >> 1, pq = ph & 1;
      const int dr = 2 * r - pp, dc = 2 * c - pq;
      xpk[i] = (item < nitems) ? (im << 24 | (dr + 64) << 12 | (dc + 64)) : (127 << 24);
      xfix[i] = ((im * p.H + dr) * p.W + dc) * p.ldx * 4 + (c0 + cq * 4) * 4;
    }
  }
  const int gq = tid & 15, gt = (tid >> 4) & 7;
  const bool g_on = tid < 128;
  int gfix = 0, gimg = 0;
  if constexpr (ROLE == 0) {
    gimg = gt >> p.sh_cthw;
    const int ty = (gt >> p.sh_ctw) & (p.CTH - 1), tx = gt & (p.CTW - 1);
    gfix = ((gimg * p.GH + 2 * ty) * p.GW + 2 * tx) * p.ldy * 4 + (kb * 64 + gq * 4) * 4;
  }
  Stream sx = stream_at(q_begin), sg = stream_at(q_begin);
  float4 rraw[W_NRAW], rg[4];
  float4 colacc = make_float4(0.f, 0.f, 0.f, 0.f);
  const bool do_bias = p.bias_ws != nullptr && rb == 0;

  auto load_raw = [&]() {
    const bool on = sx.q < q_end;
    const float* base = p.x + (size_t)sx.ng * p.CNIMG * p.H * p.W * p.ldx;
    const __amdgpu_buffer_rsrc_t rs = rsrc(base, on);
    const int oy = sx.cy * 4 * p.CTH, ox = sx.cx * 4 * p.CTW;
    const int soff = (oy * p.W + ox) * p.ldx * 4;
    const int nleft = p.N - sx.ng * p.CNIMG;
#pragma unroll
    for (int i = 0; i < W_NRAW; ++i) {
      const int dr = ((xpk[i] >> 12) & 4095) - 64, dc = (xpk[i] & 4095) - 64;
      const bool ok = (unsigned)(oy + dr) < (unsigned)p.H && (unsigned)(ox + dc) < (unsigned)p.W && (xpk[i] >> 24) < nleft;
      rraw[i] = bload4(rs, ok ? (unsigned)(xfix[i] + soff) : OOB, 0);
    }
    step(sx);
  };
  auto store_raw = [&](int stage) {
#pragma unroll
    for (int i = 0; i < W_NRAW; ++i)
      if (tid + 256 * i < nitems) *reinterpret_cast<float4*>(smem + W_RAW0 + stage * W_RAWSZ + (tid + 256 * i) * 4) = rraw[i];
  };
  auto load_gy = [&]() {
    const bool on = g_on && sg.q < q_end && sg.ng * p.CNIMG + gimg < p.N;
    const float* base = p.gy + (size_t)sg.ng * p.CNIMG * p.GH * p.GW * p.ldy;
    const __amdgpu_buffer_rsrc_t rs = rsrc(base, sg.q < q_end);
    const unsigned v = on ? (unsigned)(gfix + ((sg.cy * 2 * p.CTH * p.GW + sg.cx * 2 * p.CTW) * p.ldy) * 4) : OOB;
    const unsigned dc = (unsigned)p.ldy * 4u, dr = (unsigned)(p.GW * p.ldy) * 4u;
    rg[0] = bload4(rs, v, 0); rg[1] = bload4(rs, v + dc, 0);
    rg[2] = bload4(rs, v + dr, 0); rg[3] = bload4(rs, v + dr + dc, 0);
    step(sg);
  };
  auto add4 = [](const float4& a, const float4& b) { return make_float4(a.x + b.x, a.y + b.y, a.z + b.z, a.w + b.w); };
  const int wrG = WV_SZ + gt * 64 + gq * 4;
  auto gy_stage_store = [&](int bufoff) {
    if (!g_on) return;
    const float4 m0 = add4(rg[0], rg[2]), m1 = add4(rg[1], rg[3]);
    float* dst = smem + bufoff + wrG;
    *reinterpret_cast<float4*>(dst + 0 * WG_PL) = rg[0];
    *reinterpret_cast<float4*>(dst + 1 * WG_PL) = add4(rg[0], rg[1]);
    *reinterpret_cast<float4*>(dst + 2 * WG_PL) = rg[1];
    *reinterpret_cast<float4*>(dst + 3 * WG_PL) = m0;
    const float4 mm = add4(m0, m1);
    *reinterpret_cast<float4*>(dst + 4 * WG_PL) = mm;
    *reinterpret_cast<float4*>(dst + 5 * WG_PL) = m1;
    *reinterpret_cast<float4*>(dst + 6 * WG_PL) = rg[2];
    *reinterpret_cast<float4*>(dst + 7 * WG_PL) = add4(rg[2], rg[3]);
    *reinterpret_cast<float4*>(dst + 8 * WG_PL) = rg[3];
    if (do_bias) {
      asm volatile("" ::: "memory");
      colacc = add4(colacc, mm);
    }
  };

  const int cq = tid & 31, tile = tid >> 5;
  int rd0 = 0;
  if constexpr (ROLE == 0) {
    const int img = tile >> p.sh_cthw, ty = (tile >> p.sh_ctw) & (p.CTH - 1), tx = tile & (p.CTW - 1);
    const int box = (cq * 4) >> p.sh_cpb, cql = cq - box * qpb;
    rd0 = (((box * p.CNIMG + img) * BHW + 2 * ty * BW + 2 * tx) * qpb + cql) * 4;
  }
  const int pxstep = qpb * 4, rowstep = BW * qpb * 4;
  const int wrV = tile * 128 + cq * 4;
  float4 d[3][3];
  auto read_raw = [&](int stage) {
#pragma unroll
    for (int r = 0; r < 3; ++r)
#pragma unroll
      for (int c = 0; c < 3; ++c) d[r][c] = *reinterpret_cast<const float4*>(smem + W_RAW0 + stage * W_RAWSZ + rd0 + r * rowstep + c * pxstep);
  };
  auto sub4 = [](const float4& a, const float4& b) { return make_float4(a.x - b.x, a.y - b.y, a.z - b.z, a.w - b.w); };
  auto row_ops = [&]() {
#pragma unroll
    for (int c = 0; c < 3; ++c) { d[0][c] = sub4(d[0][c], d[1][c]); d[2][c] = sub4(d[2][c], d[1][c]); }
// ... 124 lines not shown
```

contrad_amd/csrc/wino23.h:

```cpp
#pragma once

namespace wino23 {

constexpr int TB = 128;
constexpr int VKQ = TB * 4;
constexpr int VPL = 2 * VKQ;
constexpr int V_SZ = 9 * VPL;
constexpr int UKQ = 64 * 4, UPL = 2 * UKQ;
constexpr int U_SZ = 9 * UPL;
constexpr int BUF = V_SZ + U_SZ;
constexpr int RAW_PX = 800;
constexpr int RAW_SZ = RAW_PX * 8;
constexpr int RAW0 = 2 * BUF;
constexpr int LDS_DWORDS = 2 * BUF + 2 * RAW_SZ;
constexpr unsigned OOB = 0x80000000u;
constexpr int NU = 5;

struct Args {
  const float* x;
  const float* U;
  float* y;
  const float* bias;
  const float* ref;
  float slope, gain;
// ... 170 lines not shown
    w_raw = w_cur; raw_item(w_raw);
    load_raw();
    store_raw(0);
    load_raw();
  } else {
    w_u = w_cur; u_item(w_u);
    load_u();
    store_u(0);
    load_u();
  }
  __syncthreads();
  if constexpr (ROLE == 0) {
    read_raw(std::integral_constant<int, 0>{}, 0);
    row_ops(std::integral_constant<int, 0>{});
#pragma unroll
    for (int r = 0; r < 3; ++r) col_ops_store(std::integral_constant<int, 0>{}, 0, r);
  } else {
    store_raw(1);
    load_raw();
  }
  __syncthreads();

  auto chunk = [&](auto par, auto phc, auto nphc, auto last_c) {
    constexpr int P = decltype(par)::value, PH = decltype(phc)::value;
    constexpr bool last = decltype(last_c)::value;
    constexpr int NPH = decltype(nphc)::value;
    constexpr int cur = P * BUF, nxt = BUF - cur;
    constexpr int S = nactive(PH);
    constexpr int R0 = NPH >> 1;
    constexpr int first = (PH >> 1) * 3 + (PH & 1);
    float4 fa[2], fb[2];
    fa[0] = *reinterpret_cast<const float4*>(smem + cur + rdA + first * VPL);
    fb[0] = *reinterpret_cast<const float4*>(smem + cur + rdB + first * UPL);
    int s = 0;
#pragma unroll
    for (int xi = 0; xi < 9; ++xi) {
      if (!active(PH, xi)) continue;
      int nx = xi + 1;
      while (nx < 9 && !active(PH, nx)) ++nx;
      if (nx < 9) {
        fa[(s + 1) & 1] = *reinterpret_cast<const float4*>(smem + cur + rdA + nx * VPL);
        fb[(s + 1) & 1] = *reinterpret_cast<const float4*>(smem + cur + rdB + nx * UPL);
      }
      if constexpr (ROLE == 0) {
        if (s == 0) read_raw(std::integral_constant<int, NPH>{}, 1 - P);
        if (s == 1) row_ops(std::integral_constant<int, NPH>{});
        if (s == 1 && S == 4) col_ops_store(std::integral_constant<int, NPH>{}, nxt, R0);
        if (s == 2) { if (S == 4) { for (int r = R0 + 1; r < 3; ++r) col_ops_store(std::integral_constant<int, NPH>{}, nxt, r); }
                      else col_ops_store(std::integral_constant<int, NPH>{}, nxt, R0); }
        if (S > 4 && s == 3) col_ops_store(std::integral_constant<int, NPH>{}, nxt, R0 + 1);
        if (S > 4 && s == 4 && R0 == 0) col_ops_store(std::integral_constant<int, NPH>{}, nxt, 2);
        if (s == S - 2) store_u(nxt);
        if (s == S - 1 && !last) load_u();
      } else {
        if (s == 0) store_raw(P);
        if (s == 1 && !last) load_raw();
      }
      __builtin_amdgcn_sched_barrier(0);
      const float* a = (const float*)&fa[s & 1];
      const float* b = (const float*)&fb[s & 1];
#pragma unroll
      for (int j = 0; j < 4; ++j) acc[xi] = __builtin_amdgcn_mfma_f32_32x32x2f32(a[j], b[j], acc[xi], 0, 0, 0);
      __builtin_amdgcn_sched_barrier(0);
      ++s;
    }
    __syncthreads();
  };
  auto phase = [&](auto phc) {
    constexpr int PH = decltype(phc)::value;
    constexpr int NX = (PH + 1) & 3;
    for (int t = 0; t + 2 < NCHc; t += 2) {
      chunk(std::integral_constant<int, 0>{}, phc, phc, std::false_type{});
      chunk(std::integral_constant<int, 1>{}, phc, phc, std::false_type{});
    }
    chunk(std::integral_constant<int, 0>{}, phc, phc, std::false_type{});
    chunk(std::integral_constant<int, 1>{}, phc, std::integral_constant<int, NX>{}, std::integral_constant<bool, PH == 3>{});
  };

  const float g1 = p.gain, g0 = p.gain * p.slope;
  auto bit_off = [&](int b) -> unsigned {
    return b < p.sh_tw ? (unsigned)((2 << b) * p.ldo * 4)
           : b < p.sh_thw ? (unsigned)((2 << (b - p.sh_tw)) * p.GW * p.ldo * 4)
                          : (unsigned)((1 << (b - p.sh_thw)) * p.GH * p.GW * p.ldo * 4);
  };

  for (; w_cur < L; w_cur += nslots) {
    phase(std::integral_constant<int, 0>{});
    phase(std::integral_constant<int, 1>{});
    phase(std::integral_constant<int, 2>{});
    phase(std::integral_constant<int, 3>{});
    const Item it = decode(w_cur);
    const int cout = it.kb * 64 + wn * 32 + l31;
    float* ybase = p.y + (size_t)it.n_first * p.GH * p.GW * p.ldo;
    const __amdgpu_buffer_rsrc_t rsY = rsrc(ybase, true);
    const __amdgpu_buffer_rsrc_t rsR = rsrc(p.ref ? p.ref + (size_t)it.n_first * p.GH * p.GW * p.ldo : ybase, p.ref != nullptr);
    const unsigned dcol = (unsigned)p.ldo * 4u, drow = (unsigned)(p.GW * p.ldo) * 4u;
    const unsigned lane_off = (lhi ? bit_off(2) : 0u) + (unsigned)((wn * 32 + l31) * 4);
    const unsigned wave_off = ((wm & 1) ? bit_off(5) : 0u) + ((wm & 2) ? bit_off(6) : 0u) + (unsigned)(it.kb * 64 * 4) +
                              (unsigned)(((it.py * 2 * p.TH) * p.GW + it.px * 2 * p.TW) * p.ldo * 4);
    const int lane_img = (wm * 32 + 4 * lhi) >> p.sh_thw;
    const int img_lim = p.N - it.n_first - lane_img;
    const float bj = p.bias ? p.bias[cout] : 0.f;
#pragma unroll
    for (int h = 0; h < 4; ++h) {
      float rv[4][4];
      unsigned vo[4], so[4];
#pragma unroll
      for (int q = 0; q < 4; ++q) {
        const int r = h * 4 + q, rbits = (r & 3) + 8 * (r >> 2);
        vo[q] = ((rbits >> p.sh_thw) < img_lim) ? lane_off : OOB;
        so[q] = wave_off + ((r & 1) ? bit_off(0) : 0u) + ((r & 2) ? bit_off(1) : 0u) + ((r & 4) ? bit_off(3) : 0u) + ((r & 8) ? bit_off(4) : 0u);
        rv[q][0] = __builtin_bit_cast(float, __builtin_amdgcn_raw_buffer_load_b32(rsR, (int)vo[q], (int)so[q], 0));
        rv[q][1] = __builtin_bit_cast(float, __builtin_amdgcn_raw_buffer_load_b32(rsR, (int)vo[q], (int)(so[q] + dcol), 0));
        rv[q][2] = __builtin_bit_cast(float, __builtin_amdgcn_raw_buffer_load_b32(rsR, (int)vo[q], (int)(so[q] + drow), 0));
        rv[q][3] = __builtin_bit_cast(float, __builtin_amdgcn_raw_buffer_load_b32(rsR, (int)vo[q], (int)(so[q] + drow + dcol), 0));
      }
#pragma unroll
      for (int q = 0; q < 4; ++q) {
        __builtin_amdgcn_sched_barrier(0);
        const int r = h * 4 + q;
        float s[3], s2[3];
#pragma unroll
        for (int a = 0; a < 3; ++a) {
          const float m0 = acc[a * 3 + 0][r], m1 = acc[a * 3 + 1][r], m2 = acc[a * 3 + 2][r];
          s[a] = m0 + m1; s2[a] = m1 + m2;
        }
        float v[4] = {s[0] + s[1], s2[0] + s2[1], s[1] + s[2], s2[1] + s2[2]};
#pragma unroll
        for (int e = 0; e < 4; ++e) {
          v[e] += bj;
          v[e] = __builtin_fmaf(v[e], (v[e] > 0.f) ? g1 : g0, rv[q][e]);
        }
        __builtin_amdgcn_raw_buffer_store_b32(__builtin_bit_cast(unsigned, v[0]), rsY, (int)vo[q], (int)so[q], 0);
        __builtin_amdgcn_raw_buffer_store_b32(__builtin_bit_cast(unsigned, v[1]), rsY, (int)vo[q], (int)(so[q] + dcol), 0);
        __builtin_amdgcn_raw_buffer_store_b32(__builtin_bit_cast(unsigned, v[2]), rsY, (int)vo[q], (int)(so[q] + drow), 0);
        __builtin_amdgcn_raw_buffer_store_b32(__builtin_bit_cast(unsigned, v[3]), rsY, (int)vo[q], (int)(so[q] + drow + dcol), 0);
      }
    }
#pragma unroll
    for (int i = 0; i < 9; ++i)
#pragma unroll
      for (int r = 0; r < 16; ++r) acc[i][r] = 0.f;
    __builtin_amdgcn_sched_barrier(0);
    if constexpr (ROLE == 1) load_raw(); else load_u();
  }
}

template <int NRAW>
__global__ __launch_bounds__(512, 2) void wino23_kernel(const Args p) {
  extern __shared__ __attribute__((aligned(16))) float smem[];
  if (threadIdx.x < 256) body<0, NRAW>(p, smem); else body<1, NRAW>(p, smem);
}

__global__ __launch_bounds__(256) void wino23_filter_kernel(const float* __restrict__ wp, float* __restrict__ U, int C, int K, int ldw) {
  const int per = (C >> 2) * K;
  const int idx = blockIdx.x * 256 + threadIdx.x;
  if (idx >= 4 * per) return;
  const int ph = idx / per, rem = idx - ph * per;
  const int o = rem % K, q4 = rem / K;
  const int phh = ph >> 1, phw = ph & 1;
  float g[2][2][4];
#pragma unroll
  for (int a = 0; a < 2; ++a)
#pragma unroll
    for (int b = 0; b < 2; ++b) {
      const int kh = (phh ? 2 * a : 1 + 2 * a) - 1, kw = (phw ? 2 * b : 1 + 2 * b) - 1;
#pragma unroll
      for (int j = 0; j < 4; ++j) g[a][b][j] = (kh < 0 || kw < 0) ? 0.f : wp[(size_t)((kh * 3 + kw) * C + 4 * q4 + j) * ldw + o];
    }
  const int nch = C >> 3;
  float4* Uo = reinterpret_cast<float4*>(U) + (size_t)ph * 9 * nch * 2 * K;
#pragma unroll
  for (int i = 0; i < 3; ++i)
#pragma unroll
    for (int j = 0; j < 3; ++j) {
      float u[4];
#pragma unroll
      for (int e = 0; e < 4; ++e) {
        const float r0 = j == 0 ? g[0][0][e] : j == 1 ? g[0][0][e] + g[0][1][e] : g[0][1][e];
        const float r1 = j == 0 ? g[1][0][e] : j == 1 ? g[1][0][e] + g[1][1][e] : g[1][1][e];
        u[e] = i == 0 ? r0 : i == 1 ? r0 + r1 : r1;
      }
      Uo[((size_t)((i * 3 + j) * nch + (q4 >> 1)) * 2 + (q4 & 1)) * K + o] = make_float4(u[0], u[1], u[2], u[3]);
    }
}

}
```

contrad_amd/csrc/wino44.h:

```cpp
#pragma once

namespace wino44 {

constexpr int NT = 32;
constexpr int KQS = NT * 4;
constexpr int PL = 2 * KQS;
constexpr int V_SZ = 36 * PL;
constexpr int RPS = 10;
constexpr int RAW_SZ = 800 * RPS;
constexpr int RAW0 = 2 * V_SZ;
constexpr int LDS_DWORDS = 2 * V_SZ + 2 * RAW_SZ;
constexpr unsigned OOB = 0x80000000u;

struct Args {
  const float* x;
  const float* U;
  float* y;
  const float* bias;
  const float* ref;
  float slope, gain;
  int N, H, W, Cin, Cout, ldi, ldo;
  int TH, TW;
  int sh_tw, sh_thw;
  int NIMG;
// ... 159 lines not shown
    load_raw(0); store_raw(0);
    load_raw(1); store_raw(1);
    load_raw(2);
  }
  unsigned u_pair = u_base(w_cur);
#pragma unroll
  for (int i = 0; i < 6; ++i) load_u(i, u_pair + (unsigned)i * u_plane, true);

  const float g1 = p.gain, g0 = p.gain * p.slope;

  auto pair = [&](auto last_c, int t) {
    constexpr bool LAST = decltype(last_c)::value;
    float4 fa[2];
    fa[0] = *reinterpret_cast<const float4*>(smem + rdA);
#pragma unroll
    for (int s = 0; s < 18; ++s) {
      const int P = s / 9, xi = s - 9 * P;
      if (xi + 1 < 9) fa[(s + 1) & 1] = *reinterpret_cast<const float4*>(smem + P * V_SZ + rdA + (xi + 1) * PL);
      if constexpr (ROLE == 1) {
#ifndef W44_NO_RAW
        if (xi == 0) store_raw(P);
        if (xi == 1 && !(P == 1 && LAST)) load_raw(t + P + 3);
#endif
      } else if (!(P == 1 && LAST)) {
#ifndef W44_NO_TRANSFORM
        if (xi == 0) tr_read(1 - P);
        if (xi == 1) tr_cols(0);
        if (xi == 2) tr_cols(3);
        if (xi >= 3) tr_row(1 - P, xi - 3);
#endif
      }
      __builtin_amdgcn_sched_barrier(0);
      const float* a = (const float*)&fa[s & 1];
      const float* b = (const float*)&ru[s % 6];
#pragma unroll
      for (int j = 0; j < 4; ++j) acc[xi] = __builtin_amdgcn_mfma_f32_32x32x2f32(a[j], b[j], acc[xi], 0, 0, 0);
      __builtin_amdgcn_sched_barrier(0);
#ifndef W44_NO_ULOAD
      if (s + 6 < 18) load_u(s % 6, u_pair + (unsigned)((s + 6) / 9) * u_step + (unsigned)((s + 6) % 9) * u_plane, true);
      else if (!LAST) load_u(s % 6, u_pair + 2u * u_step + (unsigned)(s - 12) * u_plane, true);
#endif
      if (xi == 8) {
        __syncthreads();
        if (P == 0) fa[(s + 1) & 1] = *reinterpret_cast<const float4*>(smem + V_SZ + rdA);
      }
    }
    u_pair += 2u * u_step;
  };

  for (; w_cur < L; w_cur += nslots) {
    __syncthreads();
    if constexpr (ROLE == 0) {
      tr_read(0); tr_cols(0); tr_cols(3);
#pragma unroll
      for (int i = 0; i < 6; ++i) tr_row(0, i);
    }
    __syncthreads();

    for (int t = 0; t + 2 < NCH; t += 2) pair(std::false_type{}, t);
    pair(std::true_type{}, NCH - 2);

    const Item it = decode(w_cur);
    auto bit_off = [&](int bb) -> unsigned {
      return bb < SH_TW ? (unsigned)((4 << bb) * p.ldo * 4)
             : bb < SH_THW ? (unsigned)((4 << (bb - SH_TW)) * p.W * p.ldo * 4)
                           : (unsigned)((1 << (bb - SH_THW)) * p.H * p.W * p.ldo * 4);
    };
    const unsigned lane_off = (lhi ? bit_off(2) : 0u) + (unsigned)((wn * 32 + l31) * 4);
    const unsigned item_off = (unsigned)((((it.ph * TH * 4) * p.W + it.pw * TW * 4) * p.ldo + it.kb * 64) * 4)
                              + ((grp & 1) ? bit_off(0) : 0u) + ((grp & 2) ? bit_off(1) : 0u);
    float* ybase = p.y + (size_t)it.n_first * p.H * p.W * p.ldo;
    const float* rbase = p.ref ? p.ref + (size_t)it.n_first * p.H * p.W * p.ldo : ybase;
    const unsigned dcol = (unsigned)p.ldo * 4u, drow = (unsigned)(p.W * p.ldo) * 4u;
    const float bj = (MODE == MODE_FWD && p.bias) ? p.bias[it.kb * 64 + wn * 32 + l31] : 0.f;
    const float ga = p.ref ? g1 : 1.f, gb = p.ref ? g0 : 1.f;
    float* xw = smem + (w8 * 9) * 64 + lane;
    const float* xr = smem + (grp * 72 + wn * 9) * 64 + lane;
#ifdef W44_NO_EPILOGUE
    if (p.N < 0)
#endif
#pragma unroll
    for (int q = 0; q < 4; ++q) {
      const unsigned voff = (it.n_first + ((grp + 8 * q + 4 * lhi) >> SH_THW) < p.N) ? lane_off : OOB;
      const __amdgpu_buffer_rsrc_t rsY = rsrc(ybase, true);
      const __amdgpu_buffer_rsrc_t rsR = rsrc(rbase, p.ref != nullptr);
      const unsigned s0 = item_off + ((q & 1) ? bit_off(3) : 0u) + ((q & 2) ? bit_off(4) : 0u);
      float rv[4][4];
#pragma unroll
      for (int j = 0; j < 4; ++j)
#pragma unroll
        for (int i = 0; i < 4; ++i)
          rv[j][i] = __builtin_bit_cast(float, __builtin_amdgcn_raw_buffer_load_b32(rsR, (int)voff, (int)(s0 + (unsigned)i * drow + (unsigned)j * dcol), 0));
#pragma unroll
      for (int xi = 0; xi < 9; ++xi)
#pragma unroll
        for (int r = 0; r < 4; ++r) xw[(r * 72 + xi) * 64] = acc[xi][4 * q + r];
      __syncthreads();
      float S[6][4];
#pragma unroll
      for (int a = 0; a < 6; ++a) {
        if ((a & 1) == 0) __builtin_amdgcn_sched_barrier(0);
        float m[6];
#pragma unroll
        for (int b = 0; b < 6; ++b) {
          const int xi36 = a * 6 + b, gq = xi36 / 9, xq = xi36 - gq * 9;
          m[b] = xr[(((gq >> 1) * 4 + (gq & 1) * 2) * 9 + xq) * 64];
        }
        at6(m[0], m[1], m[2], m[3], m[4], m[5], S[a]);
      }
      __builtin_amdgcn_sched_barrier(0);
#pragma unroll
      for (int j = 0; j < 4; ++j) {
        float v[4];
        at6(S[0][j], S[1][j], S[2][j], S[3][j], S[4][j], S[5][j], v);
#pragma unroll
        for (int i = 0; i < 4; ++i) {
          if constexpr (MODE == MODE_DGRAD) {
            v[i] *= (rv[j][i] > 0.f) ? ga : gb;
          } else {
            v[i] += bj;
            v[i] = __builtin_fmaf(v[i], (v[i] > 0.f) ? g1 : g0, rv[j][i]);
          }
          __builtin_amdgcn_raw_buffer_store_b32(__builtin_bit_cast(unsigned, v[i]), rsY, (int)voff, (int)(s0 + (unsigned)i * drow + (unsigned)j * dcol), 0);
        }
      }
      if (q < 3) __syncthreads();
    }
#pragma unroll
    for (int i = 0; i < 9; ++i)
#pragma unroll
      for (int r = 0; r < 16; ++r) acc[i][r] = 0.f;
    __builtin_amdgcn_sched_barrier(0);
    const int w_next = w_cur + nslots;
    if constexpr (ROLE == 1) {
#pragma unroll
      for (int i = 0; i < NRAW; ++i) vraw_cur[i] = vraw_nxt[i];
      xb_cur = xb_nxt;
      load_raw(2);
    }
    u_pair = u_base(w_next);
#pragma unroll
    for (int i = 0; i < 6; ++i) load_u(i, u_pair + (unsigned)i * u_plane, w_next < L);
    if constexpr (ROLE == 1) raw_offsets(w_next + nslots, vraw_nxt, xb_nxt);
  }
}

template <int MODE, int BOXW>
__global__ __launch_bounds__(512, 2) void wino44_kernel(const Args p) {
  extern __shared__ __attribute__((aligned(16))) float smem[];
  if (threadIdx.x < 256) body<MODE, 0, BOXW>(p, smem); else body<MODE, 1, BOXW>(p, smem);
}

template <int MODE>
__global__ __launch_bounds__(256) void wino44_filter_kernel(const float* __restrict__ wp, float* __restrict__ U, int C, int K, int ldw) {
  const int cin = (MODE == MODE_FWD) ? C : K, cout = (MODE == MODE_FWD) ? K : C;
  const int idx = blockIdx.x * 256 + threadIdx.x;
  if (idx >= (cin >> 2) * cout) return;
  const int o = idx % cout, q4 = idx / cout;
  float g[9][4];
  if constexpr (MODE == MODE_FWD) {
#pragma unroll
    for (int t = 0; t < 9; ++t)
#pragma unroll
      for (int j = 0; j < 4; ++j) g[t][j] = wp[(size_t)(t * C + 4 * q4 + j) * ldw + o];
  } else {
#pragma unroll
    for (int t = 0; t < 9; ++t) {
      const float4 v = *reinterpret_cast<const float4*>(wp + (size_t)((8 - t) * C + o) * ldw + 4 * q4);
      g[t][0] = v.x; g[t][1] = v.y; g[t][2] = v.z; g[t][3] = v.w;
    }
  }
  const int nch = cin >> 3;
  float4* Uo = reinterpret_cast<float4*>(U);
  auto grow = [](int a, float g0, float g1, float g2) -> float {
    return a == 0 ? 0.25f * g0
         : a == 1 ? (-1.f / 6.f) * (g0 + g1 + g2)
         : a == 2 ? (-1.f / 6.f) * (g0 - g1 + g2)
         : a == 3 ? (1.f / 24.f) * g0 + (1.f / 12.f) * g1 + (1.f / 6.f) * g2
         : a == 4 ? (1.f / 24.f) * g0 - (1.f / 12.f) * g1 + (1.f / 6.f) * g2
                  : g2;
  };
#pragma unroll
  for (int a = 0; a < 6; ++a) {
    float t[3][4];
#pragma unroll
    for (int j = 0; j < 3; ++j)
#pragma unroll
      for (int e = 0; e < 4; ++e) t[j][e] = grow(a, g[0 * 3 + j][e], g[1 * 3 + j][e], g[2 * 3 + j][e]);
#pragma unroll
    for (int b = 0; b < 6; ++b) {
      float u[4];
#pragma unroll
      for (int e = 0; e < 4; ++e) u[e] = grow(b, t[0][e], t[1][e], t[2][e]);
      const int xi = a * 6 + b;
      Uo[((size_t)(xi * nch + (q4 >> 1)) * 2 + (q4 & 1)) * cout + o] = make_float4(u[0], u[1], u[2], u[3]);
    }
  }
}

}
```

contrad_amd/models/gan/sndcgan.py:

```python
import torch
import torch.nn as nn
import torch.distributed as dist

from ... import ops
from ...hostio import upload
from ... import autograd_ops as A
from .base import BaseDiscriminator, SNParams, TinyHead, _Act, make_projection

_D_CONVS = [(3, 64, 3, 1, 1), (64, 128, 4, 2, 1), (128, 128, 3, 1, 1), (128, 256, 4, 2, 1),
            (256, 256, 3, 1, 1), (256, 512, 4, 2, 1), (512, 512, 3, 1, 1)]
_SLOPE = 0.1


def _flat_views(total_sizes, device):
    offs, tot = [], 0
    for n in total_sizes:
        offs.append(tot)
        tot += ops.round_up(n, 4)
    buf = torch.empty(max(tot, 4), device=device, dtype=torch.float32)
    return buf, [buf[o:o + n] for o, n in zip(offs, total_sizes)]


class _DPlan(object):

    def __init__(self, D, device):
        self.hb = D.s_hb
        self.wb = D.s_wb
        dh, dp = D.d_hidden, D.d_project
        self.dh, self.dp = dh, dp
        convs = [D.main[2 * i] for i in range(7)]
        heads1 = [D._head().l1, D.projection[0], D.projection2[0]]
        heads2 = [D._head().l2, D.projection[2], D.projection2[2]]
        self.layers = convs + heads1 + heads2
        T_head = self.hb * self.wb
        self.specs = []
        for m in convs:
            self.specs.append(ops.SnSpec(m.weight_orig, m.weight_u, m.weight_v))
        for m in heads1:
            self.specs.append(ops.SnSpec(m.weight_orig, m.weight_u, m.weight_v, view_kct=(dh, 512, T_head)))
        for m in heads2:
            self.specs.append(ops.SnSpec(m.weight_orig, m.weight_u, m.weight_v))
        sizes = [s.T * s.C * s.K for s in self.specs[:7]]
        sizes.append(T_head * 512 * 3 * dh)
        sizes += [dh * 4, dh * dp, dh * dp]
        self.pack_sizes = sizes
        self.feat = T_head * 512

    def alloc_packed(self, device):
        buf, v = _flat_views(self.pack_sizes, device)
        dh, dp = self.dh, self.dp
        wps, ldws = [], []
        for i, s in enumerate(self.specs[:7]):
            wps.append(v[i].view(s.T * s.C, s.K)); ldws.append(s.K)
        merged = v[7].view(self.feat, 3 * dh)
        for j in range(3):
            wps.append(merged[:, j * dh:(j + 1) * dh]); ldws.append(3 * dh)
        wps.append(v[8].view(dh, 4)); ldws.append(4)
        wps.append(v[9].view(dh, dp)); ldws.append(dp)
        wps.append(v[10].view(dh, dp)); ldws.append(dp)
        return buf, wps, ldws, merged


class _DFunction(torch.autograd.Function):
    @staticmethod
    def forward(ctx, D, images, sg_linear, want_features, trunk_grad, *params):
        dev = images.device
        plan = _DPlan(D, dev)
        specs = plan.specs
        n = len(specs)
        training = D.training
        B = images.shape[0]
        dh, dp = plan.dh, plan.dp

        wbuf, wps, ldws, merged = plan.alloc_packed(dev)
        offs, scr_n = ops.sn_scratch_floats(specs)
        snap_sizes = []
        for s in specs:
            snap_sizes += [s.K, s.C * s.T]
        snapbuf, snaps = _flat_views(snap_sizes, dev)
        u_snaps, v_snaps = snaps[0::2], snaps[1::2]
        scratch = torch.empty(scr_n, device=dev, dtype=torch.float32)
        sigma = torch.empty(n, device=dev, dtype=torch.float32)
        if trunk_grad:
            ops.sn_weight_prep(specs, wps, ldws, training, scratch, offs, sigma, u_snaps, v_snaps)
        else:
            ops.sn_weight_prep(specs[:7], wps[:7], ldws[:7], False, scratch, offs[:7], sigma, u_snaps[:7], v_snaps[:7])
            ops.sn_weight_prep(specs[7:], wps[7:], ldws[7:], training, scratch, offs[7:], sigma[7:], u_snaps[7:],
                               v_snaps[7:])

        biases = [m.bias for m in plan.layers]
        acts = []
        x = ops.rgb_conv_fwd(images, wps[0], biases[0], 64, 3, 2.0, -1.0, _SLOPE, 1.0)
        acts.append(x)
        for i in range(1, 7):
            ci, co, k, s, p = _D_CONVS[i]
            x = ops.conv2d_fwd(x, wps[i], biases[i], co, k, k, s, p, _SLOPE, 1.0)
            acts.append(x)
        bias_cat = torch.cat([biases[7], biases[8], biases[9]])
        hidden = ops.conv2d_fwd(x.view(B, 1, 1, plan.feat), merged, bias_cat, 3 * dh, 1, 1, 1, 0, _SLOPE, 1.0)
        logits = ops.conv2d_fwd(hidden[..., 0:dh], wps[10], biases[10], 1, 1, 1, 1, 0).view(B, 1)
        proj = ops.conv2d_fwd(hidden[..., dh:2 * dh], wps[11], biases[11], dp, 1, 1, 1, 0).view(B, dp)
        proj2 = ops.conv2d_fwd(hidden[..., 2 * dh:3 * dh], wps[12], biases[12], dp, 1, 1, 1, 0).view(B, dp)

        if getattr(D, '_record_activations', False):
            D._last_activations = (acts, hidden)
        ctx.plan, ctx.D = plan, D
        ctx.images, ctx.acts, ctx.hidden = images, acts, hidden
        ctx.wps, ctx.ldws, ctx.merged, ctx.wbuf = wps, ldws, merged, wbuf
        ctx.sigma, ctx.u_snaps, ctx.v_snaps, ctx.snapbuf = sigma, u_snaps, v_snaps, snapbuf
        ctx.sg_linear, ctx.trunk_grad = sg_linear, trunk_grad
        ctx.param_shapes = [tuple(p.shape) for p in params]
        if want_features:
            feats = x.permute(0, 3, 1, 2).reshape(B, -1)
        else:
            feats = logits.new_empty(0)
            ctx.mark_non_differentiable(feats)
        return logits, proj, proj2, feats

    @staticmethod
    def backward(ctx, g_logits, g_proj, g_proj2, g_feats):
        plan, D = ctx.plan, ctx.D
        specs, wps, ldws = plan.specs, ctx.wps, ctx.ldws
        acts, hidden, images = ctx.acts, ctx.hidden, ctx.images
        dev = images.device
        B = images.shape[0]
        dh, dp = plan.dh, plan.dp
        n = len(specs)
        need_params = any(ctx.needs_input_grad[5:])
        need_images = ctx.needs_input_grad[1]
        a6 = acts[6]
        comm = getattr(D, '_grad_comm', None)

        def exchange(t):
            if comm is not None:
                comm.reduce_async(t)

        def _c(g, shape):
            if g is None:
                return torch.zeros(shape, device=dev, dtype=torch.float32)
            return g.contiguous()

        g_logits = _c(g_logits, (B, 1)).view(B, 1, 1, 1)
        g_proj = _c(g_proj, (B, dp)).view(B, 1, 1, dp)
        g_proj2 = _c(g_proj2, (B, dp)).view(B, 1, 1, dp)

        if need_params:
            gbuf, gv = _flat_views(plan.pack_sizes, dev)
            gwps = []
            for i, s in enumerate(specs[:7]):
                gwps.append(gv[i].view(s.T * s.C, s.K))
            gmerged = gv[7].view(plan.feat, 3 * dh)
            for j in range(3):
                gwps.append(gmerged[:, j * dh:(j + 1) * dh])
            gwps += [gv[8].view(dh, 4), gv[9].view(dh, dp), gv[10].view(dh, dp)]
            bsizes = [m.bias.numel() for m in plan.layers]
            bbuf, gbias = _flat_views(bsizes, dev)

        g_hidden = torch.empty((B, 1, 1, 3 * dh), device=dev, dtype=torch.float32)
        outs = [(g_logits, 10, 0), (g_proj, 11, 1), (g_proj2, 12, 2)]
        for g, li, j in outs:
            hs = hidden[..., j * dh:(j + 1) * dh]
            ops.conv2d_dgrad(g, wps[li], (B, 1, 1, dh), 1, 1, 1, 0, act_ref=hs, slope=_SLOPE, gain=1.0,
                             out=g_hidden[..., j * dh:(j + 1) * dh])
            if need_params:
                if g.shape[3] % 4 == 0:
                    ops.conv2d_wgrad(hs, g, 1, 1, 1, 0, out=gwps[li], dbias=gbias[li])
                else:
                    ops.conv2d_wgrad(hs, g, 1, 1, 1, 0, out=gwps[li])
                    ops.colstats(ops.as_rows(g), out=gbias[li].view(1, -1))
                exchange(gwps[li])
        if need_params:
            gb_hidden = torch.empty(3 * dh, device=dev, dtype=torch.float32)
            ops.conv2d_wgrad(a6.view(B, 1, 1, plan.feat), g_hidden, 1, 1, 1, 0, out=gmerged, dbias=gb_hidden)
            exchange(gmerged)
            for j in range(3):
                gbias[7 + j].copy_(gb_hidden[j * dh:(j + 1) * dh])
        g = None
        if ctx.trunk_grad:
            lo = dh if ctx.sg_linear else 0
            fused = g_feats is None or g_feats.numel() == 0
            g = ops.conv2d_dgrad(g_hidden[..., lo:], ctx.merged[:, lo:], (B, 1, 1, plan.feat), 1, 1, 1, 0,
                                 act_ref=a6.view(B, 1, 1, plan.feat) if fused else None, slope=_SLOPE,
                                 gain=1.0).view(a6.shape)
            if not fused:
                g = g + g_feats.reshape(B, 512, plan.hb, plan.wb).permute(0, 2, 3, 1)
                g = (g * torch.where(a6 > 0, 1.0, _SLOPE)).contiguous()
            for i in range(6, 0, -1):
                ci, co, k, s, p = _D_CONVS[i]
                if need_params:
                    ops.conv2d_wgrad(acts[i - 1], g, k, k, s, p, out=gwps[i], dbias=gbias[i])
                    exchange(gwps[i])
                g = ops.conv2d_dgrad(g, wps[i], tuple(acts[i - 1].shape), k, k, s, p, act_ref=acts[i - 1],
                                     slope=_SLOPE, gain=1.0)
            if need_params:
                ops.rgb_conv_wgrad(images, g, 3, 2.0, -1.0, gwps[0], gbias[0])
                exchange(gwps[0])
        d_images = None
        if need_images and g is not None:
            d_images = ops.rgb_conv_dgrad(g, wps[0], None, 3, 3, act=0, out_scale=2.0, out_shift=0.0)

        grads = [None] * (2 * n)
        if need_params:
            if g is None:
                for i in range(7):
                    gwps[i].zero_(); gbias[i].zero_()
                    exchange(gwps[i])
            if comm is not None:
                exchange(bbuf)
                comm.wait()
            wsizes = [s.K * s.C * s.T for s in specs]
            gwbuf, gws = _flat_views(wsizes, dev)
            offs, scr_n = ops.sn_scratch_floats(specs)
            scratch = torch.empty(scr_n, device=dev, dtype=torch.float32)
            ops.sn_weight_grad(specs, wps, ldws, gwps, gws, scratch, offs, ctx.sigma, ctx.u_snaps, ctx.v_snaps)
            for i in range(n):
                grads[2 * i] = gws[i].view(ctx.param_shapes[2 * i])
                grads[2 * i + 1] = gbias[i]
        return (None, d_images, None, None, None) + tuple(grads)


class D_SNDCGAN(BaseDiscriminator):

    def __init__(self, image_size, ndf=64, n_classes=1, normalize=False, disable_sn=False, mlp_linear=True,
                 d_hidden=512, d_project=128):
        super().__init__()
        if ndf != 64 or n_classes != 1 or normalize or disable_sn or not mlp_linear:
            raise NotImplementedError('only the configuration built by get_architecture("sndcgan") is implemented')
        s_h, s_w, nc = image_size
        if nc != 3 or s_h % 8 or s_w % 8:
            raise NotImplementedError('RGB images with sides divisible by 8')
        self.image_size = image_size
        self.s_hb, self.s_wb = s_h // 8, s_w // 8
        self.n_features = 512 * self.s_hb * self.s_wb
        self.d_penul = self.n_features
        self.n_classes, self.d_hidden, self.d_project = n_classes, d_hidden, d_project

        self.linear = TinyHead(self.n_features, d_hidden, spectral=True)
        self.projection = make_projection(self.n_features, d_hidden, d_project, spectral=True)
        self.projection2 = make_projection(self.n_features, d_hidden, d_project, spectral=True)
        layers = []
        for (ci, co, k, s, p) in _D_CONVS:
            layers += [SNParams((co, ci, k, k)), _Act(_SLOPE)]
        self.main = nn.Sequential(*layers)

    def enable_grad_overlap(self, comm):
        self._grad_comm = comm

    def _ordered_params(self):
        out = []
        for m in ([self.main[2 * i] for i in range(7)] +
                  [self._head().l1, self.projection[0], self.projection2[0],
                   self._head().l2, self.projection[2], self.projection2[2]]):
            out += [m.weight_orig, m.bias]
        return out

    def _run(self, inputs, sg_linear, finetuning, want_features):
        if not inputs.is_cuda:
            raise RuntimeError('contrad_amd.D_SNDCGAN runs on the MI355X HIP path only (no CPU fallback)')
        if finetuning:
            inputs = inputs.detach()
        images = inputs.contiguous().float()
        logits, proj, proj2, feats = _DFunction.apply(self, images, bool(sg_linear), bool(want_features),
                                                      not finetuning, *self._ordered_params())
        return logits, proj, proj2, (feats if want_features else None)

    def penultimate(self, inputs):
        return self._run(inputs, False, False, True)[3]


class BNParams(nn.Module):

    def __init__(self, c, eps=1e-5, momentum=0.1):
        super().__init__()
        self.eps, self.momentum = eps, momentum
        self.weight = nn.Parameter(torch.ones(c))
        self.bias = nn.Parameter(torch.zeros(c))
        self.register_buffer('running_mean', torch.zeros(c))
        self.register_buffer('running_var', torch.ones(c))
        self.register_buffer('num_batches_tracked', torch.tensor(0, dtype=torch.long))


def _sync_on(flag):
    from ...engine import dist_on
    return flag and dist_on()


class _BNReLUFn(torch.autograd.Function):

    @staticmethod
    def forward(ctx, x2d, gamma, beta, bn, conv_bias, sync):
        x2d = x2d.contiguous()
        stats = ops.colstats(x2d, with_sq=True)
        count = float(x2d.shape[0])
        if _sync_on(sync):
            dist.all_reduce(stats)
            count *= dist.get_world_size()
        if bn.training:
            ops.bn_running_update(stats, count, conv_bias, bn.momentum, bn.running_mean, bn.running_var,
                                  bn.num_batches_tracked)
        y = torch.empty_like(x2d)
        ops.bn_relu_apply(x2d, y, stats, count, gamma, beta, bn.eps)
        ctx.save_for_backward(x2d, stats, gamma, beta)
        ctx.cfg = (count, bn.eps, sync)
        ctx.cb_shape = tuple(conv_bias.shape) if (conv_bias is not None and conv_bias.requires_grad) else None
        return y

    @staticmethod
    def backward(ctx, dy):
        x2d, stats, gamma, beta = ctx.saved_tensors
        count, eps, sync = ctx.cfg
        red = (lambda t: dist.all_reduce(t)) if _sync_on(sync) else None
        dx, dgamma, dbeta = ops.bn_relu_bwd(dy.contiguous(), x2d, stats, count, gamma, beta, eps, red)
        dcb = torch.zeros(ctx.cb_shape, device=dy.device, dtype=dy.dtype) if ctx.cb_shape is not None else None
        return dx, dgamma, dbeta, None, dcb, None


class _WB(nn.Module):
    def __init__(self, wshape, nbias):
        super().__init__()
        self.weight = nn.Parameter(torch.empty(*wshape).normal_(0.0, 0.02))
        self.bias = nn.Parameter(torch.zeros(nbias))


class G_SNDCGAN(nn.Module):

    _CONVT = [(512, 256, 4, 2, 1), (256, 128, 4, 2, 1), (128, 64, 4, 2, 1), (64, 3, 3, 1, 1)]

    def __init__(self, image_size, ngf=64, nz=128):
        super().__init__()
        if ngf != 64:
            raise NotImplementedError('ngf = 64')
        s_h, s_w, nc = image_size
        self.image_size, self.ngf, self.nz = image_size, ngf, nz
        self.s_hb, self.s_wb = s_h // 8, s_w // 8
        f = ngf * 8 * self.s_hb * self.s_wb
        self.linear = _WB((f, nz), f)
        self.norm_init = BNParams(f)
        layers = []
        for j, (ci, co, k, s, p) in enumerate(self._CONVT):
            layers.append(_WB((ci, co, k, k), co))
            if j < 3:
                layers += [BNParams(co), _Act(0.0)]
            else:
                layers.append(_Act(1.0))
        self.main = nn.Sequential(*layers)
        self.sync_bn = True
        self._packed = None
        self._packed_key = None

    def sample_latent(self, n_samples):
        _device = next(self.parameters()).device
        return upload(torch.empty(n_samples, self.nz).uniform_(-1, 1), _device)

    def invalidate_cache(self):
        self._packed, self._packed_key = None, None

    def _weights(self):
        ws = [self.linear.weight] + [self.main[3 * j].weight for j in range(4)]
        key = tuple((w.data_ptr(), w._version) for w in ws)
        if self._packed_key != key:
            dev = ws[0].device
            specs = [ops.SnSpec(w, fixed_scale=1.0) for w in ws]
            sizes = [s.K * s.C * s.T for s in specs]
            buf, v = _flat_views(sizes, dev)
            wps = [v[i].view(s.T * s.C, s.K) for i, s in enumerate(specs)]
            ldws = [s.K for s in specs]
            offs, scr_n = ops.sn_scratch_floats(specs)
            scratch = torch.empty(scr_n, device=dev, dtype=torch.float32)
            sigma = torch.empty(len(specs), device=dev, dtype=torch.float32)
            ops.sn_weight_prep(specs, wps, ldws, False, scratch, offs, sigma)
            self._packed, self._packed_key, self._packed_buf = wps, key, buf
        return self._packed

    def _bn(self, x2d, bn, conv_bias, out2d, perm_hw=1):
        if not self.training:
            mean = bn.running_mean if conv_bias is None else bn.running_mean - conv_bias
            stats = torch.stack([mean, bn.running_var + mean * mean]).contiguous()
            ops.bn_relu_apply(x2d, out2d, stats, 1.0, bn.weight, bn.bias, bn.eps, perm_hw)
            return
        stats = ops.colstats(x2d, with_sq=True)
        count = float(x2d.shape[0])
        if _sync_on(self.sync_bn):
            dist.all_reduce(stats)
            count *= dist.get_world_size()
        if self.training:
            ops.bn_running_update(stats, count, conv_bias, bn.momentum, bn.running_mean, bn.running_var,
                                  bn.num_batches_tracked)
        ops.bn_relu_apply(x2d, out2d, stats, count, bn.weight, bn.bias, bn.eps, perm_hw)

    def _forward_with_grad(self, z):
        N = z.shape[0]
        hb, wb = self.s_hb, self.s_wb
        f = 512 * hb * wb
        entries = [(f, self.nz, 1, 1.0, 0, 0)]
        groups = [(self.nz, f)]
        ws = [self.linear.weight]
        for j, (ci, co, k, s, p) in enumerate(self._CONVT):
            groups.append((k * k * co, ci))
            entries.append((ci, co, k * k, 1.0, j + 1, 0))
            ws.append(self.main[3 * j].weight)
        wp = A.PackWeightsFn.apply(A.PackMeta(entries, groups), *ws)
        z = z.contiguous().float()
        h0 = A.ConvBiasActFn.apply(z.view(N, 1, 1, self.nz), wp[0], self.linear.bias, (f, 1, 1, 1, 0), 1.0, 1.0)
        y0 = _BNReLUFn.apply(h0.view(N, f), self.norm_init.weight, self.norm_init.bias, self.norm_init, None,
                             self.sync_bn)
        x = y0.view(N, 512, hb, wb).permute(0, 2, 3, 1).contiguous()
        for j in range(3):
            ci, co, k, s, p = self._CONVT[j]
            H, W = x.shape[1], x.shape[2]
            y = A.ConvDgradFn.apply(x, wp[1 + j], (N, 2 * H, 2 * W, co), (ci, k, k, s, p))
            bn = self.main[3 * j + 1]
            y2 = _BNReLUFn.apply(y.view(-1, co), bn.weight, bn.bias, bn, self.main[3 * j].bias, self.sync_bn)
            x = y2.view(N, 2 * H, 2 * W, co)
        lin = A.RgbDgradFn.apply(x, wp[4], 3, (3, 1.0))
        return 0.5 * torch.tanh(lin + self.main[9].bias.view(1, 3, 1, 1)) + 0.5

    def forward(self, z):
        if not z.is_cuda:
            raise RuntimeError('contrad_amd.G_SNDCGAN runs on the MI355X HIP path only (no CPU fallback)')
        if torch.is_grad_enabled() and any(p.requires_grad for p in self.parameters()):
            if not self.training:
                raise NotImplementedError('eval-mode BatchNorm (running statistics) is not on the training path')
            return self._forward_with_grad(z)
        wps = self._weights()
        N = z.shape[0]
        hb, wb = self.s_hb, self.s_wb
        f = 512 * hb * wb
        z = z.contiguous().float()
        h0 = ops.conv2d_fwd(z.view(N, 1, 1, self.nz), wps[0], self.linear.bias, f, 1, 1, 1, 0).view(N, f)
        x = torch.empty((N, hb, wb, 512), device=z.device, dtype=torch.float32)
        self._bn(h0, self.norm_init, None, x.view(N, f), perm_hw=hb * wb)
        for j in range(3):
            ci, co, k, s, p = self._CONVT[j]
            H, W = x.shape[1], x.shape[2]
            y = ops.conv2d_dgrad(x, wps[1 + j], (N, 2 * H, 2 * W, co), k, k, s, p)
            y2 = ops.as_rows(y)
            self._bn(y2, self.main[3 * j + 1], self.main[3 * j].bias, y2)
            x = y
        return ops.rgb_conv_dgrad(x, wps[4], self.main[9].bias, 3, 3, act=1, out_scale=0.5, out_shift=0.5)
```

contrad_amd/ops.py:

```python
import ctypes

import torch

from ._lib import ConvDesc, lib


def _p(t):
    return ctypes.c_void_p(t.data_ptr()) if t is not None else ctypes.c_void_p(0)


_raw_stream = getattr(torch._C, '_cuda_getCurrentRawStream', None)


def _stream_handle():
    if _raw_stream is not None:
        return _raw_stream(torch.cuda.current_device())
    return torch.cuda.current_stream().cuda_stream


def _stream():
    return ctypes.c_void_p(_stream_handle())


def _chk(t, name):
    if t is None:
        return
    if not t.is_cuda or t.dtype != torch.float32:
        raise RuntimeError('contrad_hip: %s must be a CUDA float32 tensor (got %s, %s)' % (name, t.device, t.dtype))
    if t.dim() > 0 and t.numel() > 0 and t.stride(-1) != 1:
        raise RuntimeError('contrad_hip: %s must be contiguous in its last dimension' % name)


def _ld(t):
    if t.dim() == 4:
        N, H, W, C = t.shape
        ld = t.stride(2) if W > 1 else (t.stride(1) if H > 1 else (t.stride(0) if N > 1 else C))
        if (W > 1 and t.stride(1) != W * ld) or (H * W > 1 and N > 1 and t.stride(0) != H * W * ld):
            raise RuntimeError('contrad_hip: NHWC view must be dense over (N,H,W)')
        return ld
    if t.dim() == 2:
        return t.stride(0) if t.size(0) > 1 else max(t.size(1), t.stride(0))
    raise RuntimeError('contrad_hip: expected a 2-D or 4-D tensor')


def round_up(x, m):
    return (x + m - 1) // m * m


def out_size(h, k, stride, pad):
    return (h + 2 * pad - k) // stride + 1


PROFILE = None
PROFILE_ONLY = None
SEQUENCE = None


def conv_kernel_name(mode, d):
    bm, bn = ctypes.c_int(0), ctypes.c_int(0)
    lib().call('contrad_conv2d_tile', ctypes.byref(d), mode, ctypes.byref(bm), ctypes.byref(bn))
    path = lib().raw('contrad_conv2d_path')(ctypes.byref(d), mode)
    if path == 4:
        return 'wgrad_c32_kernel'
    if path == 5:
        return 'fwd_k1_kernel'
    if path == 6:
        return 'conv_c32_kernel<%d>' % mode
    if path == 7:
        return 'wino_wgrad_kernel' if mode == 2 else 'wino_kernel<%d>' % mode
    if path == 8:
        return 'wino22_wgrad_kernel' if mode == 2 else 'wino22_kernel<%d>' % mode
    if path == 9:
        return 'wino44_kernel<%d>' % mode
    if path == 11:
        return 'wino44n_kernel<%d>' % mode
    if path == 10:
        return 'wino23_kernel'
    if path in (2, 3):
        return 'igemm_lean_kernel<%d, %d, %d>' % (mode, bm.value, bn.value)
    return 'igemm_kernel<%d, %d, %d, %s>' % (mode, bm.value, bn.value, 'true' if path == 1 else 'false')


def _conv_call(mode, d, name, *args):
    if SEQUENCE is not None:
        SEQUENCE.append([conv_kernel_name(mode, d), [d.N, d.H, d.W, d.C, d.K, d.KH, d.KW, d.stride, d.pad],
                         int(lib().raw('contrad_conv2d_grid_blocks')(ctypes.byref(d), mode, 1)),
                         round(2.0 * d.N * d.Ho * d.Wo * d.K * d.C * d.KH * d.KW / 1e9, 4),
                         round(float(lib().raw('contrad_conv2d_executed_fraction')(ctypes.byref(d), mode)), 4)])
    if PROFILE is None:
        lib().call(name, *args)
        return
    kname = conv_kernel_name(mode, d)
    if PROFILE_ONLY is not None and kname != PROFILE_ONLY:
        lib().call(name, *args)
        return
    e0, e1 = torch.cuda.Event(enable_timing=True), torch.cuda.Event(enable_timing=True)
    st = torch.cuda.current_stream()
    e0.record(st)
    lib().call(name, *args)
    e1.record(st)
    flops = 2.0 * d.N * d.Ho * d.Wo * d.K * d.C * d.KH * d.KW
    shape = (d.N, d.H, d.W, d.C, d.K, d.KH, d.KW, d.stride, d.pad)
    blocks = lib().raw('contrad_conv2d_grid_blocks')(ctypes.byref(d), mode, 1)
    executed = float(lib().raw('contrad_conv2d_executed_fraction')(ctypes.byref(d), mode))
    PROFILE.append((kname, flops, e0, e1, shape, int(blocks), executed))


def make_desc(N, H, W, C, K, KH, KW, stride, pad, ldx, ldy, ldw):
    return ConvDesc(N, H, W, C, ldx, out_size(H, KH, stride, pad), out_size(W, KW, stride, pad), K, ldy,
                    KH, KW, stride, pad, ldw)


def pack_weight(w):
    K, C, KH, KW = w.shape
    ldw = round_up(K, 4)
    wp = w.new_zeros(KH * KW * C, ldw)
    wp[:, :K] = w.permute(2, 3, 1, 0).reshape(KH * KW * C, K)
    return wp


def unpack_weight(wp, K, C, KH, KW):
    return wp[:, :K].reshape(KH, KW, C, K).permute(3, 2, 0, 1).contiguous()


def conv2d_fwd(x, wp, bias, K, KH, KW, stride, pad, slope=1.0, gain=1.0, out=None, addend=None):
    _chk(x, 'x'); _chk(wp, 'wp'); _chk(bias, 'bias'); _chk(addend, 'addend')
    N, H, W, C = x.shape
    Ho, Wo = out_size(H, KH, stride, pad), out_size(W, KW, stride, pad)
    if out is None:
        out = torch.empty((N, Ho, Wo, K), device=x.device, dtype=torch.float32)
    _chk(out, 'out')
    d = make_desc(N, H, W, C, K, KH, KW, stride, pad, _ld(x), _ld(out), wp.stride(0))
    nbytes = lib().raw('contrad_conv2d_fwd_workspace_bytes')(ctypes.byref(d))
    ws = _workspace(nbytes, x.device) if nbytes > 0 else None
    if addend is not None and (tuple(addend.shape) != tuple(out.shape) or _ld(addend) != _ld(out)):
        raise RuntimeError('contrad_hip: addend must match y in shape and leading dimension')
    _conv_call(0, d, 'contrad_conv2d_fwd_add', ctypes.byref(d), _p(x), _p(wp), _p(bias), _p(addend), _p(out),
               float(slope), float(gain), _p(ws), nbytes, _stream())
    return out


def conv2d_dgrad(gy, wp, x_shape, KH, KW, stride, pad, act_ref=None, slope=1.0, gain=1.0, out=None):
    _chk(gy, 'gy'); _chk(wp, 'wp'); _chk(act_ref, 'act_ref')
    N, H, W, C = x_shape
    K = gy.shape[3]
    if out is None:
        out = torch.empty((N, H, W, C), device=gy.device, dtype=torch.float32)
    _chk(out, 'out')
    if act_ref is not None and (tuple(act_ref.shape) != tuple(out.shape) or _ld(act_ref) != _ld(out)):
        raise RuntimeError('contrad_hip: act_ref must match dx in shape and leading dimension')
    d = make_desc(N, H, W, C, K, KH, KW, stride, pad, _ld(out), _ld(gy), wp.stride(0))
    if (d.Ho, d.Wo) != (gy.shape[1], gy.shape[2]):
        raise RuntimeError('contrad_hip: gy spatial size does not match the conv geometry')
    nbytes = lib().raw('contrad_conv2d_dgrad_workspace_bytes')(ctypes.byref(d))
    ws = _workspace(nbytes, gy.device) if nbytes > 0 else None
    _conv_call(1, d, 'contrad_conv2d_dgrad_ws', ctypes.byref(d), _p(gy), _p(wp), _p(out), _p(act_ref),
               float(slope), float(gain), _p(ws), nbytes, _stream())
    return out


def conv2d_wino(mode, inp, wp, C, K, bias=None, ref=None, slope=1.0, gain=1.0, out=None, k4s2=False, f44=False, k3s2=False):
    _chk(inp, 'inp'); _chk(wp, 'wp'); _chk(bias, 'bias'); _chk(ref, 'ref')
    N, Hi, Wi, _ = inp.shape
    co = K if mode == 0 else C
    if k3s2:
        if mode != 0:
            raise RuntimeError('contrad_hip: the 3x3 stride-2 Winograd kernel is forward only')
        H, W = Hi, Wi
        oshape = (N, (H - 1) // 2, (W - 1) // 2, co)
        geo = (3, 3, 2, 0)
    elif k4s2:
        H, W = (Hi, Wi) if mode == 0 else (2 * Hi, 2 * Wi)
        oshape = (N, H // 2, W // 2, co) if mode == 0 else (N, H, W, co)
        geo = (4, 4, 2, 1)
    else:
        H, W = Hi, Wi
        oshape = (N, H, W, co)
        geo = (3, 3, 1, 1)
    if out is None:
        out = torch.empty(oshape, device=inp.device, dtype=torch.float32)
    _chk(out, 'out')
    if ref is not None and (tuple(ref.shape) != tuple(out.shape) or _ld(ref) != _ld(out)):
        raise RuntimeError('contrad_hip: ref must match the output in shape and leading dimension')
    d = make_desc(N, H, W, C, K, geo[0], geo[1], geo[2], geo[3], _ld(inp) if mode == 0 else _ld(out),
                  _ld(out) if mode == 0 else _ld(inp), wp.stride(0))
    if f44:
        if k4s2 or lib().raw('contrad_conv2d_wino44_ok')(ctypes.byref(d), mode) != 1:
            raise RuntimeError('contrad_hip: shape not supported by the F(4x4, 3x3) Winograd kernel')
        nbytes = lib().raw('contrad_conv2d_wino44_workspace_bytes')(ctypes.byref(d))
    else:
        if lib().raw('contrad_conv2d_wino_ok')(ctypes.byref(d), mode) != 1:
            raise RuntimeError('contrad_hip: shape not supported by the Winograd kernels')
        nbytes = lib().raw('contrad_conv2d_wino_workspace_bytes')(ctypes.byref(d), mode)
    if nbytes < 0:
        raise RuntimeError('contrad_hip: the Winograd workspace query rejected the shape (%d)' % nbytes)
    ws = _workspace(nbytes, inp.device)
    lib().call('contrad_conv2d_wino44' if f44 else 'contrad_conv2d_wino', ctypes.byref(d), mode, _p(inp), _p(wp), _p(bias), _p(ref), _p(out),
               float(slope), float(gain), _p(ws), ctypes.c_longlong(nbytes), _stream())
    return out


def conv2d_wino_wgrad(x, gy, ldw=None, out=None, dbias=None):
    _chk(x, 'x'); _chk(gy, 'gy')
    N, H, W, C = x.shape
    K = gy.shape[3]
    k, st = (3, 1) if gy.shape[1] == H else (4, 2)
    if out is None:
        out = torch.zeros((k * k * C, ldw or round_up(K, 4)), device=x.device, dtype=torch.float32)
    _chk(out, 'out')
    d = make_desc(N, H, W, C, K, k, k, st, 1, _ld(x), _ld(gy), out.stride(0))
    if lib().raw('contrad_conv2d_wino_ok')(ctypes.byref(d), 2) != 1:
        raise RuntimeError('contrad_hip: shape not supported by the Winograd weight-gradient kernel')
    nbytes = lib().raw('contrad_conv2d_wino_workspace_bytes')(ctypes.byref(d), 2)
    if nbytes < 0:
        raise RuntimeError('contrad_hip: the Winograd workspace query rejected the shape (%d)' % nbytes)
    ws = _workspace(nbytes, x.device)
    lib().call('contrad_conv2d_wino_wgrad', ctypes.byref(d), _p(x), _p(gy), _p(out), _p(dbias), _p(ws),
               ctypes.c_longlong(ws.numel() * 4), _stream())
    return out


_ws_cache = {}


class private_workspace(object):

    def __init__(self, owner_dict):
        self.mine = owner_dict

    def __enter__(self):
        global _ws_cache
        self.saved, _ws_cache = _ws_cache, self.mine
        return self

    def __exit__(self, *exc):
        global _ws_cache
        _ws_cache = self.saved
        return False


def _workspace(nbytes, device):
    key = (device.index, _stream_handle())
    buf = _ws_cache.get(key)
    if buf is None or buf.numel() * 4 < nbytes:
        buf = torch.empty((max(nbytes, 1) + 3) // 4, device=device, dtype=torch.float32)
        _ws_cache[key] = buf
    return buf


def conv2d_wgrad(x, gy, KH, KW, stride, pad, ldw=None, out=None, dbias=None):
    _chk(x, 'x'); _chk(gy, 'gy')
    N, H, W, C = x.shape
    K = gy.shape[3]
    if out is None:
        ldw = ldw or round_up(K, 4)
        out = torch.zeros((KH * KW * C, ldw), device=x.device, dtype=torch.float32)
    _chk(out, 'out')
    d = make_desc(N, H, W, C, K, KH, KW, stride, pad, _ld(x), _ld(gy), out.stride(0))
    nbytes = lib().raw('contrad_conv2d_wgrad_workspace_bytes')(ctypes.byref(d))
    if nbytes < 0:
        raise RuntimeError('contrad_hip: bad conv descriptor (%d)' % nbytes)
    ws = _workspace(nbytes, x.device)
    _conv_call(2, d, 'contrad_conv2d_wgrad', ctypes.byref(d), _p(x), _p(gy), _p(out), _p(dbias), _p(ws),
               ctypes.c_longlong(ws.numel() * 4), _stream())
    return out


def l2norm_fwd(u):
    _chk(u, 'u')
    R, D = u.shape
    z = torch.empty((R, D), device=u.device, dtype=torch.float32)
    inv = torch.empty((R,), device=u.device, dtype=torch.float32)
    lib().call('contrad_l2norm_fwd', _p(u), _ld(u), _p(z), _p(inv), R, D, 1e-12, _stream())
    return z, inv


def l2norm_bwd(dz, z, inv, out=None, accumulate=False):
    R, D = z.shape
    if out is None:
        out = torch.empty((R, D), device=z.device, dtype=torch.float32)
    lib().call('contrad_l2norm_bwd', _p(dz), _p(z), _p(inv), _p(out), _ld(out), R, D, int(accumulate), _stream())
    return out


def contrast_fwd(z, N, mode, temperature):
    _chk(z, 'z')
    if not z.is_contiguous():
        raise RuntimeError('contrad_hip: z must be contiguous')
    R, D = z.shape
    lse = torch.empty((R,), device=z.device, dtype=torch.float32)
    rowloss = torch.empty((R,), device=z.device, dtype=torch.float32)
    loss = torch.empty((1,), device=z.device, dtype=torch.float32)
    nbytes = lib().raw('contrad_contrast_workspace_bytes')(R, D)
    ws = _workspace(nbytes, z.device)
    lib().call('contrad_contrast_fwd', _p(z), R, D, N, mode, 1.0 / temperature, _p(lse), _p(rowloss), _p(loss),
               _p(ws), nbytes, _stream())
    return loss, lse


def contrast_bwd(z, lse, N, mode, temperature, grad_scale=None):
    R, D = z.shape
    dz = torch.empty((R, D), device=z.device, dtype=torch.float32)
    nbytes = lib().raw('contrad_contrast_workspace_bytes')(R, D)
    ws = _workspace(nbytes, z.device)
    lib().call('contrad_contrast_bwd', _p(z), _p(lse), R, D, N, mode, 1.0 / temperature, _p(grad_scale), _p(dz),
               _p(ws), nbytes, _stream())
    return dz


from ._lib import SnBatch, SnLayer, AdamBatch, SN_MAX_LAYERS, ADAM_MAX_TENSORS, AUG_NPARAM


class SnSpec(object):
    __slots__ = ('w', 'u', 'v', 'K', 'C', 'T', 'fixed_scale')

    def __init__(self, w, u=None, v=None, fixed_scale=0.0, view_kct=None):
        self.w, self.u, self.v = w, u, v
        if view_kct is not None:
            self.K, self.C, self.T = view_kct
        elif w.dim() == 4:
            self.K, self.C, self.T = w.shape[0], w.shape[1], w.shape[2] * w.shape[3]
        else:
            self.K, self.C, self.T = w.shape[0], w.shape[1], 1
        assert self.K * self.C * self.T == w.numel()
        self.fixed_scale = float(fixed_scale)


def sn_scratch_floats(specs):
    offs, tot = [], 0
    for s in specs:
        offs.append(tot)
        tot += int(lib().raw('contrad_sn_scratch_floats')(s.K, s.C, s.T))
        tot = round_up(tot, 4)
    return offs, tot


def _sn_batches(specs, wps, ldws, offs, u_snaps=None, v_snaps=None, gwps=None, gws=None):
    for start in range(0, len(specs), SN_MAX_LAYERS):
        b = SnBatch()
        chunk = specs[start:start + SN_MAX_LAYERS]
        b.n = len(chunk)
        for j, s in enumerate(chunk):
            i = start + j
            L = b.layers[j]
            L.w = s.w.data_ptr()
            L.u = s.u.data_ptr() if s.u is not None else None
            L.v = s.v.data_ptr() if s.v is not None else None
            L.u_snap = u_snaps[i].data_ptr() if (u_snaps is not None and u_snaps[i] is not None) else None
            L.v_snap = v_snaps[i].data_ptr() if (v_snaps is not None and v_snaps[i] is not None) else None
            L.wp = wps[i].data_ptr()
            L.gwp = gwps[i].data_ptr() if gwps is not None else None
            L.gw = gws[i].data_ptr() if gws is not None else None
            L.K, L.C, L.T, L.ldw = s.K, s.C, s.T, ldws[i]
            L.fixed_scale = s.fixed_scale
            b.scratch_off[j] = offs[i]
        yield b, start


def sn_weight_prep(specs, wps, ldws, training, scratch, offs, sigma, u_snaps=None, v_snaps=None, eps=1e-12):
    for b, start in _sn_batches(specs, wps, ldws, offs, u_snaps, v_snaps):
        lib().call('contrad_sn_weight_prep', ctypes.byref(b), int(bool(training)), float(eps), _p(scratch),
                   ctypes.c_void_p(sigma.data_ptr() + 4 * start), _stream())


def sn_weight_grad(specs, wps, ldws, gwps, gws, scratch, offs, sigma, u_snaps=None, v_snaps=None):
    for b, start in _sn_batches(specs, wps, ldws, offs, u_snaps, v_snaps, gwps, gws):
        lib().call('contrad_sn_weight_grad', ctypes.byref(b), _p(scratch),
                   ctypes.c_void_p(sigma.data_ptr() + 4 * start), _stream())


def rgb_conv_fwd(img, wp, bias, K, k, in_scale, in_shift, slope, gain, out=None):
    _chk(img, 'img'); _chk(wp, 'wp'); _chk(bias, 'bias')
    if not img.is_contiguous():
        raise RuntimeError('contrad_hip: image batch must be contiguous NCHW')
    N, Cin, H, W = img.shape
    if out is None:
        out = torch.empty((N, H, W, K), device=img.device, dtype=torch.float32)
    lib().call('contrad_rgb_conv_fwd', _p(img), _p(wp), _p(bias), _p(out), N, Cin, H, W, K, k, _ld(out),
               wp.stride(0), float(in_scale), float(in_shift), float(slope), float(gain), _stream())
    return out


def rgb_conv_wgrad(img, gy, k, in_scale, in_shift, dwp, dbias=None):
    _chk(img, 'img'); _chk(gy, 'gy'); _chk(dwp, 'dwp')
    N, Cin, H, W = img.shape
    K = gy.shape[3]
    nbytes = lib().raw('contrad_rgb_conv_wgrad_workspace_bytes')(N, Cin, H, W, K, k)
    ws = _workspace(nbytes, img.device)
    lib().call('contrad_rgb_conv_wgrad', _p(img), _p(gy), _p(dwp), _p(dbias), N, Cin, H, W, K, k, _ld(gy),
               dwp.stride(0), float(in_scale), float(in_shift), _p(ws), ctypes.c_longlong(ws.numel() * 4), _stream())
    return dwp


def rgb_conv_dgrad(gy, wp, bias, C, k, act=0, out_scale=1.0, out_shift=0.0, out=None, mod=None, residual=None):
    _chk(gy, 'gy'); _chk(wp, 'wp'); _chk(bias, 'bias'); _chk(mod, 'mod'); _chk(residual, 'residual')
    N, H, W, K = gy.shape
    if out is None:
        out = torch.empty((N, C, H, W), device=gy.device, dtype=torch.float32)
    if mod is not None and (tuple(mod.shape) != (N, K) or not mod.is_contiguous()):
        raise RuntimeError('contrad_hip: mod must be a contiguous (N, K) tensor')
    if residual is not None and (tuple(residual.shape) != (N, C, H, W) or not residual.is_contiguous()):
        raise RuntimeError('contrad_hip: residual must be a contiguous (N, C, H, W) tensor')
    lib().call('contrad_rgb_conv_dgrad', _p(gy), _p(wp), _p(bias), _p(mod), _p(residual), _p(out), N, C, H, W, K, k,
               _ld(gy), wp.stride(0), int(act), float(out_scale), float(out_shift), _stream())
    return out


def colstats(x2d, with_sq=False, out=None, accumulate=False):
    _chk(x2d, 'x')
    M, K = x2d.shape
    ld = _ld(x2d)
    if out is None:
        out = torch.empty((2 if with_sq else 1, K), device=x2d.device, dtype=torch.float32)
    nbytes = lib().raw('contrad_colstats_workspace_bytes')(ctypes.c_longlong(M), K, int(with_sq))
    ws = _workspace(nbytes, x2d.device)
    lib().call('contrad_colstats', _p(x2d), ctypes.c_longlong(M), K, ld, int(with_sq), _p(out), int(accumulate),
               _p(ws), ctypes.c_longlong(ws.numel() * 4), _stream())
    return out


def as_rows(t):
    N, H, W, C = t.shape
    return t.as_strided((N * H * W, C), (_ld(t), 1), t.storage_offset())


def bn_relu_apply(x2d, y2d, stats, count, gamma, beta, eps=1e-5, perm_hw=1):
    M, K = x2d.shape
    lib().call('contrad_bn_relu_apply', _p(x2d), _p(y2d), ctypes.c_longlong(M), K, _ld(x2d), _ld(y2d), _p(stats),
               float(count), _p(gamma), _p(beta), float(eps), int(perm_hw), _stream())
    return y2d


def bn_running_update(stats, count, conv_bias, momentum, running_mean, running_var, num_batches_tracked=None):
    K = running_mean.numel()
    if num_batches_tracked is not None and (num_batches_tracked.dtype != torch.int64 or not num_batches_tracked.is_cuda):
        raise RuntimeError('contrad_hip: num_batches_tracked must be an int64 tensor on the device')
    lib().call('contrad_bn_running_update', _p(stats), float(count), K, _p(conv_bias), float(momentum),
               _p(running_mean), _p(running_var), _p(num_batches_tracked), _stream())


GAN_LOSS_KINDS = {'nonsat': 0, 'wgan': 1, 'hinge': 2, 'lsgan': 3}


def gan_d_loss(logits, N, kind):
    _chk(logits, 'logits')
    out = torch.empty(3, device=logits.device, dtype=torch.float32)
    grad = torch.empty((3 * N, 1), device=logits.device, dtype=torch.float32)
    lib().call('contrad_gan_d_loss', _p(logits), logits.stride(0), N, GAN_LOSS_KINDS[kind], _p(out), _p(grad), _stream())
    return out, grad


def gan_g_loss(logits, kind):
    _chk(logits, 'logits')
    N = logits.shape[0]
    out = torch.empty(1, device=logits.device, dtype=torch.float32)
    grad = torch.empty((N, 1), device=logits.device, dtype=torch.float32)
    lib().call('contrad_gan_g_loss', _p(logits), logits.stride(0), N, GAN_LOSS_KINDS.get(kind, 1), _p(out), _p(grad),
               _stream())
    return out, grad


def adam_step(params, grads, exp_avgs, exp_avg_sqs, step, lr, beta1, beta2, eps=1e-8, grad_scale=1.0):
    n = len(params)
    for start in range(0, n, ADAM_MAX_TENSORS):
        b = AdamBatch()
        m = min(ADAM_MAX_TENSORS, n - start)
        b.n = m
        for j in range(m):
            p, g = params[start + j], grads[start + j]
            if not (p.is_contiguous() and g.is_contiguous()):
                raise RuntimeError('contrad_hip: Adam needs contiguous parameters and gradients')
            t = b.t[j]
            t.p, t.g = p.data_ptr(), g.data_ptr()
            t.m, t.v = exp_avgs[start + j].data_ptr(), exp_avg_sqs[start + j].data_ptr()
            t.numel = p.numel()
        lib().call('contrad_adam_step', ctypes.byref(b), int(step), float(lr), float(beta1), float(beta2),
                   float(eps), float(grad_scale), _stream())


def adam_step_dev(params, grads, exp_avgs, exp_avg_sqs, hyper, beta1, beta2, eps=1e-8):
    n = len(params)
    for start in range(0, n, ADAM_MAX_TENSORS):
        b = AdamBatch()
        m = min(ADAM_MAX_TENSORS, n - start)
        b.n = m
        for j in range(m):
            p, g = params[start + j], grads[start + j]
            if not (p.is_contiguous() and g.is_contiguous()):
                raise RuntimeError('contrad_hip: Adam needs contiguous parameters and gradients')
            t = b.t[j]
            t.p, t.g = p.data_ptr(), g.data_ptr()
            t.m, t.v = exp_avgs[start + j].data_ptr(), exp_avg_sqs[start + j].data_ptr()
            t.numel = p.numel()
        lib().call('contrad_adam_step_dev', ctypes.byref(b), _p(hyper), float(beta1), float(beta2), float(eps), _stream())


def axpby_(y, x, a, b):
    lib().call('contrad_axpby', _p(y), _p(x), ctypes.c_longlong(y.numel()), float(a), float(b), _stream())
    torch.autograd.graph.increment_version(y)
    return y


def _chk_out(out, like, name):
    _chk(out, 'out')
    if tuple(out.shape) != tuple(like.shape) or not out.is_contiguous() or out.device != like.device:
        raise RuntimeError('contrad_hip: %s: out must be a contiguous tensor of shape %s on %s' % (name, tuple(like.shape), like.device))


def simclr_augment(x, params, contrast_first, has_contrast, out=None):
    _chk(x, 'x'); _chk(params, 'params')
    if not x.is_contiguous() or tuple(params.shape) != (x.shape[0], AUG_NPARAM) or not params.is_contiguous():
        raise RuntimeError('contrad_hip: simclr_augment needs contiguous NCHW input and (B,%d) params' % AUG_NPARAM)
    B, C, H, W = x.shape
    if C != 3:
        raise RuntimeError('contrad_hip: simclr_augment is defined for RGB images')
# ... 342 lines not shown
```

include/contrad_hip.h:

```cpp
#ifndef CONTRAD_HIP_H
#define CONTRAD_HIP_H

#ifdef __cplusplus
extern "C" {
#endif

typedef void* contrad_stream_t;

int contrad_abi_version(void);

typedef struct {
  int N, H, W, C;
  int ldx;
  int Ho, Wo, K;
  int ldy;
  int KH, KW;
  int stride, pad;
  int ldw;
} contrad_conv_desc;

int contrad_conv2d_fwd(const contrad_conv_desc* d, const float* x, const float* wp, const float* bias,
                       float* y, float slope, float gain, float* workspace, long long workspace_bytes,
                       contrad_stream_t stream);
int contrad_conv2d_fwd_add(const contrad_conv_desc* d, const float* x, const float* wp, const float* bias,
                           const float* addend, float* y, float slope, float gain, float* workspace,
                           long long workspace_bytes, contrad_stream_t stream);
long long contrad_conv2d_fwd_workspace_bytes(const contrad_conv_desc* d);

int contrad_conv2d_dgrad(const contrad_conv_desc* d, const float* gy, const float* wp, float* dx,
                         const float* act_ref, float slope, float gain, contrad_stream_t stream);
long long contrad_conv2d_dgrad_workspace_bytes(const contrad_conv_desc* d);
int contrad_conv2d_dgrad_ws(const contrad_conv_desc* d, const float* gy, const float* wp, float* dx,
                            const float* act_ref, float slope, float gain, float* workspace,
                            long long workspace_bytes, contrad_stream_t stream);

int contrad_conv2d_wino_ok(const contrad_conv_desc* d, int mode);
long long contrad_conv2d_wino_workspace_bytes(const contrad_conv_desc* d, int mode);
int contrad_conv2d_wino_wgrad(const contrad_conv_desc* d, const float* x, const float* gy, float* dwp, float* dbias,
                              float* workspace, long long workspace_bytes, contrad_stream_t stream);
int contrad_conv2d_wino(const contrad_conv_desc* d, int mode, const float* in, const float* wp, const float* bias,
                        const float* ref, float* out, float slope, float gain, float* workspace,
                        long long workspace_bytes, contrad_stream_t stream);

int contrad_conv2d_wino44_ok(const contrad_conv_desc* d, int mode);
long long contrad_conv2d_wino44_workspace_bytes(const contrad_conv_desc* d);
int contrad_conv2d_wino44(const contrad_conv_desc* d, int mode, const float* in, const float* wp, const float* bias,
                          const float* ref, float* out, float slope, float gain, float* workspace,
                          long long workspace_bytes, contrad_stream_t stream);

long long contrad_conv2d_wgrad_workspace_bytes(const contrad_conv_desc* d);
int contrad_conv2d_tile(const contrad_conv_desc* d, int mode, int* bm, int* bn);
int contrad_conv2d_path(const contrad_conv_desc* d, int mode);
double contrad_conv2d_executed_fraction(const contrad_conv_desc* d, int mode);
long long contrad_conv2d_grid_blocks(const contrad_conv_desc* d, int mode, int with_workspace);
int contrad_conv2d_tile_order(const contrad_conv_desc* d, int mode, unsigned char* out, int capacity);
int contrad_conv2d_wgrad(const contrad_conv_desc* d, const float* x, const float* gy, float* dwp,
                         float* dbias, float* workspace, long long workspace_bytes, contrad_stream_t stream);

long long contrad_contrast_workspace_bytes(int R, int D);
int contrad_contrast_fwd(const float* z, int R, int D, int N, int mode, float inv_temp, float* lse,
                         float* rowloss, float* loss, float* workspace, long long workspace_bytes,
                         contrad_stream_t stream);
int contrad_contrast_bwd(const float* z, const float* lse, int R, int D, int N, int mode, float inv_temp,
                         const float* grad_scale, float* dz, float* workspace, long long workspace_bytes,
                         contrad_stream_t stream);
int contrad_l2norm_fwd(const float* u, int ldu, float* z, float* inv_norm, int R, int D, float eps,
                       contrad_stream_t stream);
int contrad_l2norm_bwd(const float* dz, const float* z, const float* inv_norm, float* du, int ldu, int R,
                       int D, int accumulate, contrad_stream_t stream);

#define CONTRAD_SN_MAX_LAYERS 24
#define CONTRAD_SN_MAX_PARTIALS 256
typedef struct {
  const float* w;
  float* u;
  float* v;
  float* u_snap;
  float* v_snap;
  float* wp;
  const float* gwp;
  float* gw;
  int K, C, T, ldw;
  float fixed_scale;
} contrad_sn_layer;
typedef struct {
  int n;
  contrad_sn_layer layers[CONTRAD_SN_MAX_LAYERS];
  long long scratch_off[CONTRAD_SN_MAX_LAYERS];
} contrad_sn_batch;

long long contrad_sn_scratch_floats(int K, int C, int T);
int contrad_sn_weight_prep(const contrad_sn_batch* b, int training, float eps, float* scratch,
                           float* sigma_out, contrad_stream_t stream);
int contrad_sn_weight_grad(const contrad_sn_batch* b, float* scratch, const float* sigma,
                           contrad_stream_t stream);

int contrad_rgb_conv_fwd(const float* img, const float* wp, const float* bias, float* y, int N, int Cin,
                         int H, int W, int K, int k, int ldy, int ldw, float in_scale, float in_shift,
                         float slope, float gain, contrad_stream_t stream);
long long contrad_rgb_conv_wgrad_workspace_bytes(int N, int Cin, int H, int W, int K, int k);
int contrad_rgb_conv_wgrad(const float* img, const float* gy, float* dwp, float* dbias, int N, int Cin,
                           int H, int W, int K, int k, int ldy, int ldw, float in_scale, float in_shift,
                           float* workspace, long long workspace_bytes, contrad_stream_t stream);
int contrad_rgb_conv_dgrad(const float* gy, const float* wp, const float* bias, const float* mod,
                           const float* residual, float* out, int N, int C, int H, int W, int K, int k,
                           int ldy, int ldw, int act, float out_scale, float out_shift,
                           contrad_stream_t stream);

long long contrad_colstats_workspace_bytes(long long M, int K, int with_sq);
int contrad_colstats(const float* x, long long M, int K, int ld, int with_sq, float* out, int accumulate,
                     float* workspace, long long workspace_bytes, contrad_stream_t stream);
int contrad_bn_relu_apply(const float* x, float* y, long long M, int K, int ldx, int ldy, const float* stats,
                          float count, const float* gamma, const float* beta, float eps, int perm_hw,
                          contrad_stream_t stream);
int contrad_bn_relu_bwd_stats(const float* dy, const float* x, long long M, int K, int ld, const float* stats,
                              float count, const float* gamma, const float* beta, float eps, float* out2k,
                              float* workspace, long long workspace_bytes, contrad_stream_t stream);
int contrad_bn_relu_bwd_apply(const float* dy, const float* x, float* dx, long long M, int K, int ld,
                              const float* stats, float count, const float* gamma, const float* beta, float eps,
                              const float* bstats, contrad_stream_t stream);
int contrad_bn_running_update(const float* stats, float count, int K, const float* conv_bias, float momentum,
                              float* running_mean, float* running_var, long long* num_batches_tracked,
                              contrad_stream_t stream);
int contrad_gan_d_loss(const float* logits, int ld, int N, int kind, float* out3, float* grad,
                       contrad_stream_t stream);
int contrad_gan_g_loss(const float* logits, int ld, int N, int kind, float* out1, float* grad,
                       contrad_stream_t stream);

#define CONTRAD_ADAM_MAX_TENSORS 64
#define CONTRAD_ADAM_CHUNK 16384
typedef struct {
  float* p;
  const float* g;
  float* m;
  float* v;
  long long numel;
} contrad_adam_tensor;
typedef struct {
  int n;
  contrad_adam_tensor t[CONTRAD_ADAM_MAX_TENSORS];
  int block_start[CONTRAD_ADAM_MAX_TENSORS + 1];
} contrad_adam_batch;
int contrad_adam_step(const contrad_adam_batch* b, int step, float lr, float beta1, float beta2, float eps,
                      float grad_scale, contrad_stream_t stream);
int contrad_adam_step_dev(const contrad_adam_batch* b, const float* hyper_dev, float beta1, float beta2, float eps,
                          contrad_stream_t stream);
int contrad_axpby(float* y, const float* x, long long n, float a, float b, contrad_stream_t stream);
int contrad_pull_host(const float* host_pinned, float* dst, long long n, contrad_stream_t stream);

#define CONTRAD_AUG_NPARAM 16
long long contrad_simclr_workspace_bytes(int B, int H, int W);
int contrad_simclr_augment(const float* x, float* y, const float* params, int B, int H, int W,
                           int contrast_first, int has_contrast, float* workspace,
                           long long workspace_bytes, contrad_stream_t stream);
long long contrad_simclr_augment_bwd_workspace_bytes(int B, int H, int W);
int contrad_simclr_augment_bwd(const float* x, const float* params, const float* grad_out, float* grad_in,
                               int B, int H, int W, int contrast_first, int has_contrast, float* workspace,
                               long long workspace_bytes, contrad_stream_t stream);
int contrad_gaussian_blur_masked(const float* x, float* tmp, float* y, const float* params,
                                 const float* kernel1d, int B, int H, int W, int radius,
                                 contrad_stream_t stream);
int contrad_cutout_masked(float* y, const float* params, int B, int H, int W, int length, contrad_stream_t stream);
int contrad_gaussian_blur_masked_bwd(const float* grad_out, float* tmp, float* grad_in, const float* params,
                                     const float* kernel1d, int B, int H, int W, int radius,
                                     contrad_stream_t stream);

int contrad_upfirdn2d(const float* input, const float* kernel, float* out, int major, int in_h, int in_w,
                      int minor, int kh, int kw, int up_x, int up_y, int down_x, int down_y, int pad_x0,
                      int pad_x1, int pad_y0, int pad_y1, contrad_stream_t stream);
int contrad_upfirdn2d_fused(const float* input, const float* kernel, float* out, int major, int in_h, int in_w,
                            int minor, int kh, int kw, int up_x, int up_y, int down_x, int down_y, int pad_x0,
                            int pad_x1, int pad_y0, int pad_y1, const float* addend, const float* act_ref, float slope,
                            float gain, float* out2, contrad_stream_t stream);
int contrad_fused_bias_act(const float* x, const float* bias, const float* ref, float* y, long long n,
                           int step_b, int size_b, int act, int grad, float alpha, float scale,
                           contrad_stream_t stream);
int contrad_lincomb(const float* x, const float* z, float* y, long long n, float a, float b,
                    contrad_stream_t stream);

int contrad_minibatch_stddev(int mode, const float* x, const float* gy, const float* h, float* out, float* out2,
                             int B, int P, int C, int Cp, contrad_stream_t stream);
long long contrad_sumsq_workspace_bytes(long long n);
int contrad_sumsq(const float* x, long long n, float scale, float* out, float* workspace, long long workspace_bytes,
                  contrad_stream_t stream);
int contrad_scale_dev(const float* x, const float* s, float c, float* y, long long n, contrad_stream_t stream);

#define CONTRAD_MODCONV_MAX_LAYERS 32
typedef struct {
  const float* w;
  float* wp;
  float* wsq;
  int Cout, Cin, T, ldw;
  int transposed;
  float scale;
} contrad_modconv_layer;
typedef struct {
  int n;
  contrad_modconv_layer layers[CONTRAD_MODCONV_MAX_LAYERS];
} contrad_modconv_batch;
int contrad_modconv_tables(const contrad_modconv_batch* b, contrad_stream_t stream);
typedef struct {
// ... 38 lines not shown
```

Baseline: 47020 images/sec.

## Batch Winograd filter transforms into one launch after spectral-norm weight prep

Result: no change. 47110 images/sec (median of 2 runs) (+0.2%).

```diff
diff --git a/contrad_amd/_lib.py b/contrad_amd/_lib.py
--- a/contrad_amd/_lib.py
+++ b/contrad_amd/_lib.py
@@ -29,6 +29,18 @@
 class SnBatch(ctypes.Structure):
     _fields_ = [('n', ctypes.c_int), ('layers', SnLayer * SN_MAX_LAYERS),
                 ('scratch_off', ctypes.c_longlong * SN_MAX_LAYERS)]
+
+
+FILTER_MAX_ITEMS = 48
+
+
+class FilterItem(ctypes.Structure):
+    _fields_ = [('wp', ctypes.c_void_p), ('U', ctypes.c_void_p),
+                ('C', ctypes.c_int), ('K', ctypes.c_int), ('ldw', ctypes.c_int), ('variant', ctypes.c_int)]
+
+
+class FilterBatch(ctypes.Structure):
+    _fields_ = [('n', ctypes.c_int), ('items', FilterItem * FILTER_MAX_ITEMS)]
 
 
 class AdamTensor(ctypes.Structure):
diff --git a/contrad_amd/csrc/igemm.hip b/contrad_amd/csrc/igemm.hip
--- a/contrad_amd/csrc/igemm.hip
+++ b/contrad_amd/csrc/igemm.hip
@@ -889,12 +889,14 @@
 
 template <int MODE>
 int launch_wino44(const contrad_conv_desc* d, const float* in, const float* wp, const float* bias, const float* ref,
-                  float* out, float slope, float gain, float* U, hipStream_t stream) {
+                  float* out, float slope, float gain, float* U, hipStream_t stream, bool prepared = false) {
   wino44::Args a = wino44_args(d, MODE);
   a.x = in; a.U = U; a.y = out; a.bias = bias; a.ref = ref; a.slope = slope; a.gain = gain;
   const int quads = (a.Cin / 4) * a.Cout;
-  hipLaunchKernelGGL(wino44::wino44_filter_kernel<MODE>, dim3(cdiv(quads, 256)), dim3(256), 0, stream, wp, U, d->C, d->K, d->ldw);
-  CONTRAD_CHECK_LAUNCH();
+  if (!prepared) {
+    hipLaunchKernelGGL(wino44::wino44_filter_kernel<MODE>, dim3(cdiv(quads, 256)), dim3(256), 0, stream, wp, U, d->C, d->K, d->ldw);
+    CONTRAD_CHECK_LAUNCH();
+  }
   if (a.n32)
     return a.BW == 34 ? launch_wino44n_inst<MODE, 34>(a, stream) : a.BW == 18 ? launch_wino44n_inst<MODE, 18>(a, stream)
            : a.BW == 10 ? launch_wino44n_inst<MODE, 10>(a, stream) : launch_wino44n_inst<MODE, 6>(a, stream);
@@ -963,12 +965,14 @@
 
 template <int MODE>
 int launch_wino22(const contrad_conv_desc* d, const float* in, const float* wp, const float* bias, const float* ref,
-                  float* out, float slope, float gain, float* U, hipStream_t stream) {
+                  float* out, float slope, float gain, float* U, hipStream_t stream, bool prepared = false) {
   wino22::Args a = wino22_args(d, MODE);
   a.x = in; a.U = U; a.y = out; a.bias = bias; a.ref = ref; a.slope = slope; a.gain = gain;
   const int quads = 4 * (a.Cin / 4) * a.Cout;
-  hipLaunchKernelGGL(wino22::wino22_filter_kernel<MODE>, dim3(cdiv(quads, 256)), dim3(256), 0, stream, wp, U, d->C, d->K, d->ldw);
-  CONTRAD_CHECK_LAUNCH();
+  if (!prepared) {
+    hipLaunchKernelGGL(wino22::wino22_filter_kernel<MODE>, dim3(cdiv(quads, 256)), dim3(256), 0, stream, wp, U, d->C, d->K, d->ldw);
+    CONTRAD_CHECK_LAUNCH();
+  }
   const int l0 = cdiv(a.NTB, 8) * a.NKB * (MODE == MODE_DGRAD ? 4 : 1);
   const int blocks = 8 * std::min(WINO_CUS / 8, l0);
   const int items = 2 * a.NIMG * (a.GH + 1) * (a.GW + 1);
@@ -1029,12 +1033,14 @@
 }
 
 int launch_wino23(const contrad_conv_desc* d, const float* in, const float* wp, const float* bias, const float* ref,
-                  float* out, float slope, float gain, float* U, hipStream_t stream) {
+                  float* out, float slope, float gain, float* U, hipStream_t stream, bool prepared = false) {
   wino23::Args a = wino23_args(d);
   a.x = in; a.U = U; a.y = out; a.bias = bias; a.ref = ref; a.slope = slope; a.gain = gain;
   const int quads = 4 * (a.Cin / 4) * a.Cout;
-  hipLaunchKernelGGL(wino23::wino23_filter_kernel, dim3(cdiv(quads, 256)), dim3(256), 0, stream, wp, U, d->C, d->K, d->ldw);
-  CONTRAD_CHECK_LAUNCH();
+  if (!prepared) {
+    hipLaunchKernelGGL(wino23::wino23_filter_kernel, dim3(cdiv(quads, 256)), dim3(256), 0, stream, wp, U, d->C, d->K, d->ldw);
+    CONTRAD_CHECK_LAUNCH();
+  }
   const int nraw = cdiv(2 * a.NIMG * (2 * a.TH + 1) * (2 * a.TW + 1), 256);
   if (nraw <= 5) return launch_wino23_inst<5>(a, stream);
   if (nraw == 6) return launch_wino23_inst<6>(a, stream);
@@ -1127,15 +1133,17 @@
 
 template <int MODE>
 int launch_wino(const contrad_conv_desc* d, const float* in, const float* wp, const float* bias, const float* ref,
-                float* out, float slope, float gain, float* U, hipStream_t stream) {
+                float* out, float slope, float gain, float* U, hipStream_t stream, bool prepared = false) {
   static const hipError_t attr = hipFuncSetAttribute((const void*)wino::wino_kernel<MODE>, hipFuncAttributeMaxDynamicSharedMemorySize,
                                                      wino::LDS_DWORDS * 4);
   if (attr != hipSuccess) return (int)attr;
   wino::Args a = wino_args(d, MODE);
   a.x = in; a.U = U; a.y = out; a.bias = bias; a.ref = ref; a.slope = slope; a.gain = gain;
   const int quads = (a.Cin / 4) * a.Cout;
-  hipLaunchKernelGGL(wino::wino_filter_kernel<MODE>, dim3(cdiv(quads, 256)), dim3(256), 0, stream, wp, U, d->C, d->K, d->ldw);
-  CONTRAD_CHECK_LAUNCH();
+  if (!prepared) {
+    hipLaunchKernelGGL(wino::wino_filter_kernel<MODE>, dim3(cdiv(quads, 256)), dim3(256), 0, stream, wp, U, d->C, d->K, d->ldw);
+    CONTRAD_CHECK_LAUNCH();
+  }
   hipLaunchKernelGGL(wino::wino_kernel<MODE>, dim3(wino_grid(a)), dim3(512), wino::LDS_DWORDS * 4, stream, a);
   CONTRAD_CHECK_LAUNCH();
   return 0;
@@ -2008,6 +2016,128 @@
   return contrad_conv2d_dgrad_ws(d, gy, wp, dx, act_ref, slope, gain, nullptr, 0, stream);
 }
 
+namespace {
+
+struct FilterMap { int start[CONTRAD_FILTER_MAX_ITEMS + 1]; };
+
+__global__ __launch_bounds__(256) void wino_filter_batch_kernel(const contrad_filter_batch b, const FilterMap map) {
+  int l = 0;
+  while (l + 1 < b.n && (int)blockIdx.x >= map.start[l + 1]) ++l;
+  const contrad_filter_item& it = b.items[l];
+  const int idx = ((int)blockIdx.x - map.start[l]) * 256 + (int)threadIdx.x;
+  switch (it.variant) {
+    case CONTRAD_FILTER_F44_FWD: wino44::wino44_filter_item<MODE_FWD>(it.wp, it.U, it.C, it.K, it.ldw, idx); break;
+    case CONTRAD_FILTER_F44_DGRAD: wino44::wino44_filter_item<MODE_DGRAD>(it.wp, it.U, it.C, it.K, it.ldw, idx); break;
+    case CONTRAD_FILTER_F22_FWD: wino::wino_filter_item<MODE_FWD>(it.wp, it.U, it.C, it.K, it.ldw, idx); break;
+    case CONTRAD_FILTER_F22_DGRAD: wino::wino_filter_item<MODE_DGRAD>(it.wp, it.U, it.C, it.K, it.ldw, idx); break;
+    case CONTRAD_FILTER_K4S2_FWD: wino22::wino22_filter_item<MODE_FWD>(it.wp, it.U, it.C, it.K, it.ldw, idx); break;
+    case CONTRAD_FILTER_K4S2_DGRAD: wino22::wino22_filter_item<MODE_DGRAD>(it.wp, it.U, it.C, it.K, it.ldw, idx); break;
+    case CONTRAD_FILTER_K3S2_FWD: wino23::wino23_filter_item(it.wp, it.U, it.C, it.K, it.ldw, idx); break;
+    default: break;
+  }
+}
+
+int filter_variant(const contrad_conv_desc* d, int mode) {
+  if (mode == MODE_FWD) {
+    if (wino44_planned(d, mode)) return CONTRAD_FILTER_F44_FWD;
+    if (wino_planned(d, mode)) return CONTRAD_FILTER_F22_FWD;
+    if (wino22_planned(d, mode)) return CONTRAD_FILTER_K4S2_FWD;
+    if (wino23_planned(d, mode)) return CONTRAD_FILTER_K3S2_FWD;
+  } else if (mode == MODE_DGRAD) {
+    if (wino44_planned(d, mode)) return CONTRAD_FILTER_F44_DGRAD;
+    if (wino_planned(d, mode)) return CONTRAD_FILTER_F22_DGRAD;
+    if (wino22_planned(d, mode)) return CONTRAD_FILTER_K4S2_DGRAD;
+  }
+  return CONTRAD_FILTER_NONE;
+}
+
+bool filter_is_dgrad(int variant) {
+  return variant == CONTRAD_FILTER_F44_DGRAD || variant == CONTRAD_FILTER_F22_DGRAD || variant == CONTRAD_FILTER_K4S2_DGRAD;
+}
+
+int filter_planes(int variant) {
+  switch (variant) {
+    case CONTRAD_FILTER_F44_FWD: case CONTRAD_FILTER_F44_DGRAD: return 36;
+    case CONTRAD_FILTER_F22_FWD: case CONTRAD_FILTER_F22_DGRAD: return 16;
+    case CONTRAD_FILTER_K4S2_FWD: case CONTRAD_FILTER_K4S2_DGRAD: case CONTRAD_FILTER_K3S2_FWD: return 36;
+    default: return 0;
+  }
+}
+
+long long filter_threads(int variant, int C, int K) {
+  const long long quads = (long long)((filter_is_dgrad(variant) ? K : C) / 4) * (filter_is_dgrad(variant) ? C : K);
+  const bool phased = variant == CONTRAD_FILTER_K4S2_FWD || variant == CONTRAD_FILTER_K4S2_DGRAD || variant == CONTRAD_FILTER_K3S2_FWD;
+  return phased ? 4 * quads : quads;
+}
+
+}
+
+extern "C" int contrad_conv2d_filter_variant(const contrad_conv_desc* d, int mode) {
+  if (check_desc(d) || mode < 0 || mode > 2) return -22;
+  return filter_variant(d, mode);
+}
+
+extern "C" long long contrad_conv2d_filter_bytes(int variant, int C, int K) {
+  if (filter_planes(variant) == 0 || C <= 0 || K <= 0) return -22;
+  return (long long)filter_planes(variant) * C * K * (long long)sizeof(float);
+}
+
+extern "C" int contrad_conv2d_filter_prep(const contrad_filter_batch* b, contrad_stream_t stream) {
+  CONTRAD_ARG(b && b->n > 0 && b->n <= CONTRAD_FILTER_MAX_ITEMS);
+  FilterMap map{};
+  for (int l = 0; l < b->n; ++l) {
+    const contrad_filter_item& it = b->items[l];
+    CONTRAD_ARG(filter_planes(it.variant) != 0 && it.wp && it.U && it.C > 0 && it.K > 0);
+    const int cin = filter_is_dgrad(it.variant) ? it.K : it.C;
+    CONTRAD_ARG((cin & 7) == 0 && it.ldw >= it.K && (it.ldw & 3) == 0 && aligned16(it.wp, it.U, nullptr));
+    CONTRAD_ARG(36ll * it.C * it.K * 4 < (1ll << 31));
+    const long long blocks = cdivll(filter_threads(it.variant, it.C, it.K), 256);
+    CONTRAD_ARG(map.start[l] + blocks < (1ll << 24));
+    map.start[l + 1] = map.start[l] + (int)blocks;
+  }
+  hipLaunchKernelGGL(wino_filter_batch_kernel, dim3(map.start[b->n]), dim3(256), 0, (hipStream_t)stream, *b, map);
+  CONTRAD_CHECK_LAUNCH();
+  return 0;
+}
+
+extern "C" int contrad_conv2d_fwd_add_pf(const contrad_conv_desc* d, const float* x, const float* bias, const float* addend,
+                                         float* y, float slope, float gain, const float* U, long long U_bytes, int variant,
+                                         contrad_stream_t stream) {
+  int rc = check_desc(d);
+  if (rc) return rc;
+  CONTRAD_ARG(x && y && U);
+  CONTRAD_ARG((long long)d->N * d->Ho * d->Wo < (1ll << 31));
+  CONTRAD_ARG(variant != CONTRAD_FILTER_NONE && variant == filter_variant(d, MODE_FWD));
+  CONTRAD_ARG(U_bytes >= contrad_conv2d_filter_bytes(variant, d->C, d->K));
+  CONTRAD_ARG(aligned16(x, U, y) && aligned16(addend, nullptr, nullptr));
+  float* Uw = const_cast<float*>(U);
+  hipStream_t s = (hipStream_t)stream;
+  switch (variant) {
+    case CONTRAD_FILTER_F44_FWD: return launch_wino44<MODE_FWD>(d, x, nullptr, bias, addend, y, slope, gain, Uw, s, true);
+    case CONTRAD_FILTER_F22_FWD: return launch_wino<MODE_FWD>(d, x, nullptr, bias, addend, y, slope, gain, Uw, s, true);
+    case CONTRAD_FILTER_K4S2_FWD: return launch_wino22<MODE_FWD>(d, x, nullptr, bias, addend, y, slope, gain, Uw, s, true);
+    default: return launch_wino23(d, x, nullptr, bias, addend, y, slope, gain, Uw, s, true);
+  }
+}
+
+extern "C" int contrad_conv2d_dgrad_pf(const contrad_conv_desc* d, const float* gy, float* dx, const float* act_ref,
+                                       float slope, float gain, const float* U, long long U_bytes, int variant,
+                                       contrad_stream_t stream) {
+  int rc = check_desc(d);
+  if (rc) return rc;
+  CONTRAD_ARG(gy && dx && U);
+  CONTRAD_ARG(variant != CONTRAD_FILTER_NONE && variant == filter_variant(d, MODE_DGRAD));
+  CONTRAD_ARG(U_bytes >= contrad_conv2d_filter_bytes(variant, d->C, d->K));
+  CONTRAD_ARG(aligned16(gy, U, dx) && aligned16(act_ref, nullptr, nullptr));
+  float* Uw = const_cast<float*>(U);
+  hipStream_t s = (hipStream_t)stream;
+  switch (variant) {
+    case CONTRAD_FILTER_F44_DGRAD: return launch_wino44<MODE_DGRAD>(d, gy, nullptr, nullptr, act_ref, dx, slope, gain, Uw, s, true);
+    case CONTRAD_FILTER_F22_DGRAD: return launch_wino<MODE_DGRAD>(d, gy, nullptr, nullptr, act_ref, dx, slope, gain, Uw, s, true);
+    default: return launch_wino22<MODE_DGRAD>(d, gy, nullptr, nullptr, act_ref, dx, slope, gain, Uw, s, true);
+  }
+}
+
 extern "C" int contrad_conv2d_wino_ok(const contrad_conv_desc* d, int mode) {
   if (check_desc(d)) return -22;
   if (mode == MODE_WGRAD) return (wino_wgrad_ok(d) || wino22_wgrad_ok(d)) ? 1 : 0;
diff --git a/contrad_amd/csrc/wino.h b/contrad_amd/csrc/wino.h
--- a/contrad_amd/csrc/wino.h
+++ b/contrad_amd/csrc/wino.h
@@ -357,9 +357,8 @@
 }
 
 template <int MODE>
-__global__ __launch_bounds__(256) void wino_filter_kernel(const float* __restrict__ wp, float* __restrict__ U, int C, int K, int ldw) {
+__device__ __forceinline__ void wino_filter_item(const float* __restrict__ wp, float* __restrict__ U, int C, int K, int ldw, int idx) {
   const int cin = (MODE == MODE_FWD) ? C : K, cout = (MODE == MODE_FWD) ? K : C;
-  const int idx = blockIdx.x * 256 + threadIdx.x;
   if (idx >= (cin >> 2) * cout) return;
   const int o = idx % cout, q4 = idx / cout;
   float g[9][4];
@@ -399,6 +398,11 @@
       Uo[((size_t)(xi * nch + (q4 >> 1)) * 2 + (q4 & 1)) * cout + o] = make_float4(u[0], u[1], u[2], u[3]);
     }
   }
+}
+
+template <int MODE>
+__global__ __launch_bounds__(256) void wino_filter_kernel(const float* __restrict__ wp, float* __restrict__ U, int C, int K, int ldw) {
+  wino_filter_item<MODE>(wp, U, C, K, ldw, blockIdx.x * 256 + threadIdx.x);
 }
 
 
diff --git a/contrad_amd/csrc/wino22.h b/contrad_amd/csrc/wino22.h
--- a/contrad_amd/csrc/wino22.h
+++ b/contrad_amd/csrc/wino22.h
@@ -334,10 +334,9 @@
 }
 
 template <int MODE>
-__global__ __launch_bounds__(256) void wino22_filter_kernel(const float* __restrict__ wp, float* __restrict__ U, int C, int K, int ldw) {
+__device__ __forceinline__ void wino22_filter_item(const float* __restrict__ wp, float* __restrict__ U, int C, int K, int ldw, int idx) {
   const int cin = (MODE == MODE_FWD) ? C : K, cout = (MODE == MODE_FWD) ? K : C;
   const int per = (cin >> 2) * cout;
-  const int idx = blockIdx.x * 256 + threadIdx.x;
   if (idx >= 4 * per) return;
   const int ph = idx / per, rem = idx - ph * per;
   const int o = rem % cout, q4 = rem / cout;
@@ -372,6 +371,11 @@
       }
       Uo[((size_t)((i * 3 + j) * nch + (q4 >> 1)) * 2 + (q4 & 1)) * cout + o] = make_float4(u[0], u[1], u[2], u[3]);
     }
+}
+
+template <int MODE>
+__global__ __launch_bounds__(256) void wino22_filter_kernel(const float* __restrict__ wp, float* __restrict__ U, int C, int K, int ldw) {
+  wino22_filter_item<MODE>(wp, U, C, K, ldw, blockIdx.x * 256 + threadIdx.x);
 }
 
 
diff --git a/contrad_amd/csrc/wino23.h b/contrad_amd/csrc/wino23.h
--- a/contrad_amd/csrc/wino23.h
+++ b/contrad_amd/csrc/wino23.h
@@ -346,9 +346,8 @@
   if (threadIdx.x < 256) body<0, NRAW>(p, smem); else body<1, NRAW>(p, smem);
 }
 
-__global__ __launch_bounds__(256) void wino23_filter_kernel(const float* __restrict__ wp, float* __restrict__ U, int C, int K, int ldw) {
+__device__ __forceinline__ void wino23_filter_item(const float* __restrict__ wp, float* __restrict__ U, int C, int K, int ldw, int idx) {
   const int per = (C >> 2) * K;
-  const int idx = blockIdx.x * 256 + threadIdx.x;
   if (idx >= 4 * per) return;
   const int ph = idx / per, rem = idx - ph * per;
   const int o = rem % K, q4 = rem / K;
@@ -379,4 +378,8 @@
     }
 }
 
-}
+__global__ __launch_bounds__(256) void wino23_filter_kernel(const float* __restrict__ wp, float* __restrict__ U, int C, int K, int ldw) {
+  wino23_filter_item(wp, U, C, K, ldw, blockIdx.x * 256 + threadIdx.x);
+}
+
+}
diff --git a/contrad_amd/csrc/wino44.h b/contrad_amd/csrc/wino44.h
--- a/contrad_amd/csrc/wino44.h
+++ b/contrad_amd/csrc/wino44.h
@@ -335,9 +335,8 @@
 }
 
 template <int MODE>
-__global__ __launch_bounds__(256) void wino44_filter_kernel(const float* __restrict__ wp, float* __restrict__ U, int C, int K, int ldw) {
+__device__ __forceinline__ void wino44_filter_item(const float* __restrict__ wp, float* __restrict__ U, int C, int K, int ldw, int idx) {
   const int cin = (MODE == MODE_FWD) ? C : K, cout = (MODE == MODE_FWD) ? K : C;
-  const int idx = blockIdx.x * 256 + threadIdx.x;
   if (idx >= (cin >> 2) * cout) return;
   const int o = idx % cout, q4 = idx / cout;
   float g[9][4];
@@ -355,30 +354,57 @@
   }
   const int nch = cin >> 3;
   float4* Uo = reinterpret_cast<float4*>(U);
-  auto grow = [](int a, float g0, float g1, float g2) -> float {
-    return a == 0 ? 0.25f * g0
-         : a == 1 ? (-1.f / 6.f) * (g0 + g1 + g2)
-         : a == 2 ? (-1.f / 6.f) * (g0 - g1 + g2)
-         : a == 3 ? (1.f / 24.f) * g0 + (1.f / 12.f) * g1 + (1.f / 6.f) * g2
-         : a == 4 ? (1.f / 24.f) * g0 - (1.f / 12.f) * g1 + (1.f / 6.f) * g2
-                  : g2;
+  constexpr float Q = 0.25f, M6 = -1.f / 6.f, C24 = 1.f / 24.f, C12 = 1.f / 12.f, C6 = 1.f / 6.f;
+  auto lin_p = [](bool lead1, float x0, float x1, float x2) -> float {
+    return lead1 ? __builtin_fmaf(x2, C6, __builtin_fmaf(x1, C12, x0 * C24)) : __builtin_fmaf(x2, C6, __builtin_fmaf(x0, C24, x1 * C12));
+  };
+  auto lin_m = [](float x0, float x1, float x2) -> float {
+    return __builtin_fmaf(x2, C6, __builtin_fmaf(x0, C24, -(x1 * C12)));
   };
 #pragma unroll
   for (int a = 0; a < 6; ++a) {
-    float t[3][4];
-#pragma unroll
-    for (int j = 0; j < 3; ++j)
-#pragma unroll
-      for (int e = 0; e < 4; ++e) t[j][e] = grow(a, g[0 * 3 + j][e], g[1 * 3 + j][e], g[2 * 3 + j][e]);
+    float u[6][4];
+#pragma unroll
+    for (int e = 0; e < 4; ++e) {
+      const bool lead1 = (MODE == MODE_FWD) && (e & 1) == 0;
+      if (a < 3) {
+        const float c = a == 0 ? Q : M6;
+        float X[3], t[3];
+#pragma unroll
+        for (int j = 0; j < 3; ++j) {
+          X[j] = a == 0 ? g[j][e] : a == 1 ? (g[j][e] + g[3 + j][e]) + g[6 + j][e] : (g[j][e] - g[3 + j][e]) + g[6 + j][e];
+          t[j] = X[j] * c;
+        }
+        u[0][e] = t[0] * Q;
+        u[1][e] = M6 * __builtin_fmaf(X[2], c, __builtin_fmaf(X[1], c, t[0]));
+        u[2][e] = M6 * __builtin_fmaf(X[2], c, __builtin_fmaf(-X[1], c, t[0]));
+        u[3][e] = lin_p(false, t[0], t[1], t[2]);
+        u[4][e] = lin_m(t[0], t[1], t[2]);
+        u[5][e] = t[2];
+      } else {
+        float t[3];
+#pragma unroll
+        for (int j = 0; j < 3; ++j)
+          t[j] = a == 3 ? lin_p(lead1, g[j][e], g[3 + j][e], g[6 + j][e]) : a == 4 ? lin_m(g[j][e], g[3 + j][e], g[6 + j][e]) : g[6 + j][e];
+        u[0][e] = t[0] * Q;
+        u[1][e] = M6 * ((t[0] + t[1]) + t[2]);
+        u[2][e] = M6 * ((t[0] - t[1]) + t[2]);
+        u[3][e] = lin_p(a == 5 && lead1, t[0], t[1], t[2]);
+        u[4][e] = lin_m(t[0], t[1], t[2]);
+        u[5][e] = t[2];
+      }
+    }
 #pragma unroll
     for (int b = 0; b < 6; ++b) {
-      float u[4];
-#pragma unroll
-      for (int e = 0; e < 4; ++e) u[e] = grow(b, t[0][e], t[1][e], t[2][e]);
       const int xi = a * 6 + b;
-      Uo[((size_t)(xi * nch + (q4 >> 1)) * 2 + (q4 & 1)) * cout + o] = make_float4(u[0], u[1], u[2], u[3]);
-    }
-  }
-}
-
-}
+      Uo[((size_t)(xi * nch + (q4 >> 1)) * 2 + (q4 & 1)) * cout + o] = make_float4(u[b][0], u[b][1], u[b][2], u[b][3]);
+    }
+  }
+}
+
+template <int MODE>
+__global__ __launch_bounds__(256) void wino44_filter_kernel(const float* __restrict__ wp, float* __restrict__ U, int C, int K, int ldw) {
+  wino44_filter_item<MODE>(wp, U, C, K, ldw, blockIdx.x * 256 + threadIdx.x);
+}
+
+}
diff --git a/contrad_amd/models/gan/sndcgan.py b/contrad_amd/models/gan/sndcgan.py
--- a/contrad_amd/models/gan/sndcgan.py
+++ b/contrad_amd/models/gan/sndcgan.py
@@ -81,10 +81,21 @@
         u_snaps, v_snaps = snaps[0::2], snaps[1::2]
         scratch = torch.empty(scr_n, device=dev, dtype=torch.float32)
         sigma = torch.empty(n, device=dev, dtype=torch.float32)
+        want_bwd = trunk_grad and any(ctx.needs_input_grad)
+        ff, fb = [None] * 7, [None] * 7
+        h, w = images.shape[2], images.shape[3]
+        for i in range(1, 7):
+            ci, co, k, s, p = _D_CONVS[i]
+            ff[i] = ops.plan_filter(0, B, h, w, ci, co, k, k, s, p, dev)
+            if want_bwd:
+                fb[i] = ops.plan_filter(1, B, h, w, ci, co, k, k, s, p, dev)
+            h, w = ops.out_size(h, k, s, p), ops.out_size(w, k, s, p)
+        filters = [(i, f) for i in range(1, 7) for f in (ff[i], fb[i]) if f is not None]
         if trunk_grad:
-            ops.sn_weight_prep(specs, wps, ldws, training, scratch, offs, sigma, u_snaps, v_snaps)
+            ops.sn_weight_prep(specs, wps, ldws, training, scratch, offs, sigma, u_snaps, v_snaps, filters=filters)
         else:
-            ops.sn_weight_prep(specs[:7], wps[:7], ldws[:7], False, scratch, offs[:7], sigma, u_snaps[:7], v_snaps[:7])
+            ops.sn_weight_prep(specs[:7], wps[:7], ldws[:7], False, scratch, offs[:7], sigma, u_snaps[:7], v_snaps[:7],
+                               filters=filters)
             ops.sn_weight_prep(specs[7:], wps[7:], ldws[7:], training, scratch, offs[7:], sigma[7:], u_snaps[7:],
                                v_snaps[7:])
 
@@ -94,7 +105,7 @@
         acts.append(x)
         for i in range(1, 7):
             ci, co, k, s, p = _D_CONVS[i]
-            x = ops.conv2d_fwd(x, wps[i], biases[i], co, k, k, s, p, _SLOPE, 1.0)
+            x = ops.conv2d_fwd(x, wps[i], biases[i], co, k, k, s, p, _SLOPE, 1.0, filt=ff[i])
             acts.append(x)
         bias_cat = torch.cat([biases[7], biases[8], biases[9]])
         hidden = ops.conv2d_fwd(x.view(B, 1, 1, plan.feat), merged, bias_cat, 3 * dh, 1, 1, 1, 0, _SLOPE, 1.0)
@@ -107,6 +118,7 @@
         ctx.plan, ctx.D = plan, D
         ctx.images, ctx.acts, ctx.hidden = images, acts, hidden
         ctx.wps, ctx.ldws, ctx.merged, ctx.wbuf = wps, ldws, merged, wbuf
+        ctx.dgrad_filters = fb
         ctx.sigma, ctx.u_snaps, ctx.v_snaps, ctx.snapbuf = sigma, u_snaps, v_snaps, snapbuf
         ctx.sg_linear, ctx.trunk_grad = sg_linear, trunk_grad
         ctx.param_shapes = [tuple(p.shape) for p in params]
@@ -191,7 +203,7 @@
                     ops.conv2d_wgrad(acts[i - 1], g, k, k, s, p, out=gwps[i], dbias=gbias[i])
                     exchange(gwps[i])
                 g = ops.conv2d_dgrad(g, wps[i], tuple(acts[i - 1].shape), k, k, s, p, act_ref=acts[i - 1],
-                                     slope=_SLOPE, gain=1.0)
+                                     slope=_SLOPE, gain=1.0, filt=ctx.dgrad_filters[i])
             if need_params:
                 ops.rgb_conv_wgrad(images, g, 3, 2.0, -1.0, gwps[0], gbias[0])
                 exchange(gwps[0])
@@ -355,9 +367,9 @@
     def invalidate_cache(self):
         self._packed, self._packed_key = None, None
 
-    def _weights(self):
+    def _weights(self, N):
         ws = [self.linear.weight] + [self.main[3 * j].weight for j in range(4)]
-        key = tuple((w.data_ptr(), w._version) for w in ws)
+        key = tuple((w.data_ptr(), w._version) for w in ws) + (N,)
         if self._packed_key != key:
             dev = ws[0].device
             specs = [ops.SnSpec(w, fixed_scale=1.0) for w in ws]
@@ -368,9 +380,16 @@
             offs, scr_n = ops.sn_scratch_floats(specs)
             scratch = torch.empty(scr_n, device=dev, dtype=torch.float32)
             sigma = torch.empty(len(specs), device=dev, dtype=torch.float32)
-            ops.sn_weight_prep(specs, wps, ldws, False, scratch, offs, sigma)
-            self._packed, self._packed_key, self._packed_buf = wps, key, buf
-        return self._packed
+            filts = []
+            h, w = self.s_hb, self.s_wb
+            for j in range(3):
+                ci, co, k, s, p = self._CONVT[j]
+                filts.append(ops.plan_filter(1, N, 2 * h, 2 * w, co, ci, k, k, s, p, dev))
+                h, w = 2 * h, 2 * w
+            ops.sn_weight_prep(specs, wps, ldws, False, scratch, offs, sigma,
+                               filters=[(1 + j, f) for j, f in enumerate(filts) if f is not None])
+            self._packed, self._packed_key, self._packed_buf, self._packed_filters = wps, key, buf, filts
+        return self._packed, self._packed_filters
 
     def _bn(self, x2d, bn, conv_bias, out2d, perm_hw=1):
         if not self.training:
@@ -422,8 +441,8 @@
             if not self.training:
                 raise NotImplementedError('eval-mode BatchNorm (running statistics) is not on the training path')
             return self._forward_with_grad(z)
-        wps = self._weights()
         N = z.shape[0]
+        wps, filts = self._weights(N)
         hb, wb = self.s_hb, self.s_wb
         f = 512 * hb * wb
         z = z.contiguous().float()
@@ -433,7 +452,7 @@
         for j in range(3):
             ci, co, k, s, p = self._CONVT[j]
             H, W = x.shape[1], x.shape[2]
-            y = ops.conv2d_dgrad(x, wps[1 + j], (N, 2 * H, 2 * W, co), k, k, s, p)
+            y = ops.conv2d_dgrad(x, wps[1 + j], (N, 2 * H, 2 * W, co), k, k, s, p, filt=filts[j])
             y2 = ops.as_rows(y)
             self._bn(y2, self.main[3 * j + 1], self.main[3 * j].bias, y2)
             x = y
diff --git a/contrad_amd/ops.py b/contrad_amd/ops.py
--- a/contrad_amd/ops.py
+++ b/contrad_amd/ops.py
@@ -123,7 +123,47 @@
     return wp[:, :K].reshape(KH, KW, C, K).permute(3, 2, 0, 1).contiguous()
 
 
-def conv2d_fwd(x, wp, bias, K, KH, KW, stride, pad, slope=1.0, gain=1.0, out=None, addend=None):
+class PreparedFilter(object):
+    __slots__ = ('U', 'variant', 'C', 'K')
+
+    def __init__(self, U, variant, C, K):
+        self.U, self.variant, self.C, self.K = U, variant, C, K
+
+
+FILTER_NONE, FILTER_F44_FWD, FILTER_F44_DGRAD, FILTER_F22_FWD, FILTER_F22_DGRAD = 0, 1, 2, 3, 4
+FILTER_K4S2_FWD, FILTER_K4S2_DGRAD, FILTER_K3S2_FWD = 5, 6, 7
+_filter_variants = {}
+
+
+def plan_filter(mode, N, H, W, C, K, KH, KW, stride, pad, device, ldx=None, ldy=None, ldw=None):
+    key = (mode, N, H, W, C, K, KH, KW, stride, pad, ldx, ldy, ldw)
+    variant = _filter_variants.get(key)
+    if variant is None:
+        d = make_desc(N, H, W, C, K, KH, KW, stride, pad, ldx or C, ldy or K, ldw or round_up(K, 4))
+        variant = int(lib().raw('contrad_conv2d_filter_variant')(ctypes.byref(d), mode))
+        if variant < 0:
+            raise RuntimeError('contrad_hip: bad conv descriptor (%d)' % variant)
+        _filter_variants[key] = variant
+    if variant == 0:
+        return None
+    nbytes = int(lib().raw('contrad_conv2d_filter_bytes')(variant, C, K))
+    return PreparedFilter(torch.empty(nbytes // 4, device=device, dtype=torch.float32), variant, C, K)
+
+
+def filter_prep(items):
+    for start in range(0, len(items), FILTER_MAX_ITEMS):
+        b = FilterBatch()
+        chunk = items[start:start + FILTER_MAX_ITEMS]
+        b.n = len(chunk)
+        for j, (wp, f) in enumerate(chunk):
+            _chk(wp, 'wp'); _chk(f.U, 'U')
+            it = b.items[j]
+            it.wp, it.U = wp.data_ptr(), f.U.data_ptr()
+            it.C, it.K, it.ldw, it.variant = f.C, f.K, wp.stride(0), f.variant
+        lib().call('contrad_conv2d_filter_prep', ctypes.byref(b), _stream())
+
+
+def conv2d_fwd(x, wp, bias, K, KH, KW, stride, pad, slope=1.0, gain=1.0, out=None, addend=None, filt=None):
     _chk(x, 'x'); _chk(wp, 'wp'); _chk(bias, 'bias'); _chk(addend, 'addend')
     N, H, W, C = x.shape
     Ho, Wo = out_size(H, KH, stride, pad), out_size(W, KW, stride, pad)
@@ -131,16 +171,20 @@
         out = torch.empty((N, Ho, Wo, K), device=x.device, dtype=torch.float32)
     _chk(out, 'out')
     d = make_desc(N, H, W, C, K, KH, KW, stride, pad, _ld(x), _ld(out), wp.stride(0))
+    if addend is not None and (tuple(addend.shape) != tuple(out.shape) or _ld(addend) != _ld(out)):
+        raise RuntimeError('contrad_hip: addend must match y in shape and leading dimension')
+    if filt is not None:
+        _conv_call(0, d, 'contrad_conv2d_fwd_add_pf', ctypes.byref(d), _p(x), _p(bias), _p(addend), _p(out), float(slope),
+                   float(gain), _p(filt.U), ctypes.c_longlong(filt.U.numel() * 4), int(filt.variant), _stream())
+        return out
     nbytes = lib().raw('contrad_conv2d_fwd_workspace_bytes')(ctypes.byref(d))
     ws = _workspace(nbytes, x.device) if nbytes > 0 else None
-    if addend is not None and (tuple(addend.shape) != tuple(out.shape) or _ld(addend) != _ld(out)):
-        raise RuntimeError('contrad_hip: addend must match y in shape and leading dimension')
     _conv_call(0, d, 'contrad_conv2d_fwd_add', ctypes.byref(d), _p(x), _p(wp), _p(bias), _p(addend), _p(out),
                float(slope), float(gain), _p(ws), nbytes, _stream())
     return out
 
 
-def conv2d_dgrad(gy, wp, x_shape, KH, KW, stride, pad, act_ref=None, slope=1.0, gain=1.0, out=None):
+def conv2d_dgrad(gy, wp, x_shape, KH, KW, stride, pad, act_ref=None, slope=1.0, gain=1.0, out=None, filt=None):
     _chk(gy, 'gy'); _chk(wp, 'wp'); _chk(act_ref, 'act_ref')
     N, H, W, C = x_shape
     K = gy.shape[3]
@@ -152,6 +196,10 @@
     d = make_desc(N, H, W, C, K, KH, KW, stride, pad, _ld(out), _ld(gy), wp.stride(0))
     if (d.Ho, d.Wo) != (gy.shape[1], gy.shape[2]):
         raise RuntimeError('contrad_hip: gy spatial size does not match the conv geometry')
+    if filt is not None:
+        _conv_call(1, d, 'contrad_conv2d_dgrad_pf', ctypes.byref(d), _p(gy), _p(out), _p(act_ref), float(slope),
+                   float(gain), _p(filt.U), ctypes.c_longlong(filt.U.numel() * 4), int(filt.variant), _stream())
+        return out
     nbytes = lib().raw('contrad_conv2d_dgrad_workspace_bytes')(ctypes.byref(d))
     ws = _workspace(nbytes, gy.device) if nbytes > 0 else None
     _conv_call(1, d, 'contrad_conv2d_dgrad_ws', ctypes.byref(d), _p(gy), _p(wp), _p(out), _p(act_ref),
@@ -309,6 +357,7 @@
 
 
 from ._lib import SnBatch, SnLayer, AdamBatch, SN_MAX_LAYERS, ADAM_MAX_TENSORS, AUG_NPARAM
+from ._lib import FilterBatch, FILTER_MAX_ITEMS
 
 
 class SnSpec(object):
@@ -357,10 +406,13 @@
         yield b, start
 
 
-def sn_weight_prep(specs, wps, ldws, training, scratch, offs, sigma, u_snaps=None, v_snaps=None, eps=1e-12):
+def sn_weight_prep(specs, wps, ldws, training, scratch, offs, sigma, u_snaps=None, v_snaps=None, eps=1e-12,
+                   filters=None):
     for b, start in _sn_batches(specs, wps, ldws, offs, u_snaps, v_snaps):
         lib().call('contrad_sn_weight_prep', ctypes.byref(b), int(bool(training)), float(eps), _p(scratch),
                    ctypes.c_void_p(sigma.data_ptr() + 4 * start), _stream())
+    if filters:
+        filter_prep([(wps[i], f) for i, f in filters])
 
 
 def sn_weight_grad(specs, wps, ldws, gwps, gws, scratch, offs, sigma, u_snaps=None, v_snaps=None):
diff --git a/include/contrad_hip.h b/include/contrad_hip.h
--- a/include/contrad_hip.h
+++ b/include/contrad_hip.h
@@ -47,6 +47,33 @@
 int contrad_conv2d_wino44(const contrad_conv_desc* d, int mode, const float* in, const float* wp, const float* bias,
                           const float* ref, float* out, float slope, float gain, float* workspace,
                           long long workspace_bytes, contrad_stream_t stream);
+
+#define CONTRAD_FILTER_NONE 0
+#define CONTRAD_FILTER_F44_FWD 1
+#define CONTRAD_FILTER_F44_DGRAD 2
+#define CONTRAD_FILTER_F22_FWD 3
+#define CONTRAD_FILTER_F22_DGRAD 4
+#define CONTRAD_FILTER_K4S2_FWD 5
+#define CONTRAD_FILTER_K4S2_DGRAD 6
+#define CONTRAD_FILTER_K3S2_FWD 7
+#define CONTRAD_FILTER_MAX_ITEMS 48
+typedef struct {
+  const float* wp;
+  float* U;
+  int C, K, ldw, variant;
+} contrad_filter_item;
+typedef struct {
+  int n;
+  contrad_filter_item items[CONTRAD_FILTER_MAX_ITEMS];
+} contrad_filter_batch;
+int contrad_conv2d_filter_variant(const contrad_conv_desc* d, int mode);
+long long contrad_conv2d_filter_bytes(int variant, int C, int K);
+int contrad_conv2d_filter_prep(const contrad_filter_batch* b, contrad_stream_t stream);
+int contrad_conv2d_fwd_add_pf(const contrad_conv_desc* d, const float* x, const float* bias, const float* addend, float* y,
+                              float slope, float gain, const float* U, long long U_bytes, int variant,
+                              contrad_stream_t stream);
+int contrad_conv2d_dgrad_pf(const contrad_conv_desc* d, const float* gy, float* dx, const float* act_ref, float slope,
+                            float gain, const float* U, long long U_bytes, int variant, contrad_stream_t stream);
 
 long long contrad_conv2d_wgrad_workspace_bytes(const contrad_conv_desc* d);
 int contrad_conv2d_tile(const contrad_conv_desc* d, int mode, int* bm, int* bn);
```
